# davxy/ark-vrf

Measured on AMD Instinct MI355X. Metric: thin_vrf_batch_verifications_per_sec, higher is better.
Workload: dtype u32x8 (256-bit prime-field Montgomery, integer)

## Files before the change

ark_vrf_amd/csrc/capi.hip:

```cpp
#include "capi_internal.h"
#include "host_sha512.h"
#include "host_shake128.h"
#include "host_sha256.h"
#include "host_sha512_mb.h"
#include <condition_variable>
#include <deque>
#include <mutex>
#include <thread>
#include "proto_dev.h"
#include "vrf_batch.h"
#include "suite_dispatch.h"
#include <chrono>
#include <optional>
#include <stdlib.h>
#include <string.h>

using namespace avrf;

namespace avrf {
double now_us() {
  return std::chrono::duration<double, std::micro>(std::chrono::steady_clock::now().time_since_epoch()).count();
}
}

static inline bool ctx_busy(const avrf_ctx *c) { return c->run_phase != 0; }

static int ensure_fixed(avrf_ctx *c) {
  if (c->fixed_ready) return AVRF_OK;
  if (c->d_fixed.ensure((size_t)2 * 32 * 256 * sizeof(te_pre_raw)) != hipSuccess) return AVRF_ERR_NO_DEVICE;
  AVRF_SINGLE(c->suite, fixed_table(c->d_fixed.as<te_pre_raw>(), c->stream));
  c->fixed_ready = true;
  return AVRF_OK;
}

static BatchDev batch_of(avrf_ctx *c) {
  BatchDev b;
  b.pks_xy = c->d_pks.as<uint8_t>(); b.ios_xy = c->d_ios.as<uint8_t>(); b.io_off = c->d_io_off.as<uint32_t>();
  b.ads = c->d_ads.as<uint8_t>(); b.ad_off = c->d_ad_off.as<uint32_t>(); b.proofs = c->d_proofs.as<uint8_t>();
  b.sks = c->d_sks.as<uint8_t>(); b.n = (uint32_t)c->n;
  b.fixed = (const te_pre *)c->d_fixed.p;
  b.tabs = (te_ext *)c->d_tabs.p; b.first = 0;
  b.weights = nullptr; b.records = nullptr;
  return b;
}

static constexpr size_t ITEM_CHUNK = 131072;
template <class F> static int per_item_chunks(avrf_ctx *c, bool with_pks, F launch) {
  if (int fs = ensure_fixed(c)) return fs;
  const size_t chunk = c->n < ITEM_CHUNK ? c->n : ITEM_CHUNK;
  if (c->d_tabs.ensure(chunk * (size_t)ITEM_TAB_SLOTS * sizeof(te_ext_raw)) != hipSuccess) return AVRF_ERR_NO_DEVICE;
  BatchDev b = batch_of(c);
  if (!with_pks) b.pks_xy = nullptr;
  for (size_t i = 0; i < c->n; i += chunk) {
    b.first = (uint32_t)i; b.n = (uint32_t)(c->n - i < chunk ? c->n : i + chunk);
    launch(b);
  }
  return AVRF_OK;
}

static void validate_staged(avrf_ctx *c, int kind, int32_t *d_rec_status) {
  if (c->validate <= 0 || !c->n) return;
  uint32_t *fl = c->d_flags.as<uint32_t>();
  const uint32_t n = (uint32_t)c->n;
  const KindFacts &k = kind_facts(kind);
  if (k.pk && c->d_pks.p) AVRF_SINGLE(c->suite, validate_xy(c->d_pks.as<uint8_t>(), 64, 1, n, c->validate, fl, d_rec_status, c->stream));
  if (k.points) AVRF_SINGLE(c->suite, validate_xy(c->d_proofs.as<uint8_t>(), (uint32_t)k.xy_proof(), (uint32_t)k.points, n, c->validate, fl, d_rec_status, c->stream));
  if (c->tot_io) {
    if (!d_rec_status) AVRF_SINGLE(c->suite, validate_xy(c->d_ios.as<uint8_t>(), 128, 2, (uint32_t)c->tot_io, c->validate, fl, nullptr, c->stream));
    else {
      const uint32_t *io_off = c->h_io.as<uint32_t>();
      bool uniform = c->tot_io == c->n;
      for (size_t j = 0; uniform && j < c->n; j++) uniform = io_off[j] == j;
      if (uniform) AVRF_SINGLE(c->suite, validate_xy(c->d_ios.as<uint8_t>(), 128, 2, n, c->validate, fl, d_rec_status, c->stream));
      else AVRF_SINGLE(c->suite, validate_xy(c->d_ios.as<uint8_t>(), 128, 2, (uint32_t)c->tot_io, c->validate, fl, d_rec_status, c->stream,
                                             c->d_io_off.as<uint32_t>(), n));
    }
  }
}

namespace avrf {
int ctx_create(int suite, int device, bool lane_owner, avrf_ctx **out) {
  if (!out || suite < 0 || suite >= AVRF_N_SUITES) return AVRF_ERR_BAD_ARG;
  *out = nullptr;
  int n = 0;
  if (hipGetDeviceCount(&n) != hipSuccess || n <= 0 || device < 0 || device >= n) return AVRF_ERR_NO_DEVICE;
  HIP_TRY(hipSetDevice(device));
  avrf_ctx *c = new avrf_ctx();
  c->suite = suite; c->device = device; c->lane_owner = lane_owner;
  if (lane_owner) {
    if (hipStreamCreateWithFlags(&c->own.stream, hipStreamNonBlocking) != hipSuccess) { delete c; return AVRF_ERR_NO_DEVICE; }
    c->stream = c->own.stream;
  }
  if (c->d_flags.ensure(64) != hipSuccess || c->h_flags.ensure(64) != hipSuccess) { avrf_ctx_destroy(c); return AVRF_ERR_NO_DEVICE; }
  *out = c;
  return AVRF_OK;
}
}

extern "C" {

int avrf_ctx_set_validation(avrf_ctx *c, int level) {
  if (!c || level < 0 || level > 2) return AVRF_ERR_BAD_ARG;
  c->validate = level;
  return AVRF_OK;
}

hipStream_t avrf_ctx_stream_(avrf_ctx *c) { return c->stream; }
int avrf_ctx_suite_(avrf_ctx *c) { return c->suite; }
int avrf_ctx_device_(avrf_ctx *c) { return c->device; }
int avrf_ctx_busy_(avrf_ctx *c) { return c && ctx_busy(c); }

const char *avrf_version(void) { return "avrf 0.3 (gfx950; tiny/thin/pedersen/ring VRF over Bandersnatch, Baby-JubJub, JubJub; device pairing)"; }

int avrf_device_count(void) {
  int n = 0;
  if (hipGetDeviceCount(&n) != hipSuccess) return 0;
  return n;
}

int avrf_device_set_blocking_sync(int device, int on) {
  int prev = 0;
  if (hipGetDevice(&prev) != hipSuccess || hipSetDevice(device) != hipSuccess) { (void)hipGetLastError(); return AVRF_ERR_NO_DEVICE; }
  const hipError_t e = hipSetDeviceFlags(on ? hipDeviceScheduleBlockingSync : hipDeviceScheduleAuto);
  (void)hipSetDevice(prev);
  if (e != hipSuccess) (void)hipGetLastError();
  return e == hipSuccess ? AVRF_OK : AVRF_ERR_NO_DEVICE;
}

int avrf_ctx_create(int suite, int device, avrf_ctx **out) { return ctx_create(suite, device, true, out); }

void avrf_ctx_destroy(avrf_ctx *c) {
  if (!c) return;
  delete c;
}

static int lane_msm(avrf_ctx *c, size_t n, HostExt *r) {
  return guarded([&] { return msm_te_device(c->suite, c->L->d_pre.as<te_pre_raw>(), c->L->d_scalars.as<uint32_t>(), n, c->L->ws, c->stream, r) ? (int)AVRF_ERR_BAD_ARG : 0; });
}
static int lane_msm_vectors(avrf_ctx *c, size_t n, size_t nv, HostExt *r) {
  return guarded([&] { return msm_te_small_vectors(c->suite, c->L->d_pre.as<te_pre_raw>(), c->L->d_scalars.as<uint32_t>(), n, nv, c->L->ws, c->stream, r) ? (int)AVRF_ERR_BAD_ARG : 0; });
}

static int finish_point(avrf_ctx *c, const HostExt &r, uint8_t out_xy[64]) {
  with_suite(c->suite, [&](auto tag) { using S = typename decltype(tag)::type; HostTe<S>::to_affine_bytes(r, out_xy); });
  return AVRF_OK;
}
static bool point_is_identity(avrf_ctx *c, const HostExt &r) {
  return with_suite(c->suite, [&](auto tag) { using S = typename decltype(tag)::type; return HostTe<S>::is_identity(r); });
}
static bool scalar_in_range(int suite, const uint8_t *s) {
  H256 v; memcpy(v.l, s, 32);
  return with_suite(suite, [&](auto tag) { using S = typename decltype(tag)::type; return !HostField<typename S::Fr>::geq_p(v); });
}

static int upload_bases_and_scalars(avrf_ctx *c, size_t n, const uint8_t *bases_xy, const uint8_t *scalars, size_t scalar_bytes) {
  HIP_TRY(c->d_misc.ensure(n * 64)); HIP_TRY(c->L->d_scalars.ensure(scalar_bytes)); HIP_TRY(c->L->d_pre.ensure(n * sizeof(te_pre_raw)));
  HIP_TRY(hipMemcpyAsync(c->d_misc.p, bases_xy, n * 64, hipMemcpyHostToDevice, c->stream));
  HIP_TRY(hipMemcpyAsync(c->L->d_scalars.p, scalars, scalar_bytes, hipMemcpyHostToDevice, c->stream));
  HIP_TRY(hipMemsetAsync(c->d_flags.p, 0, 4, c->stream));
  return AVRF_OK;
}

static int msm_te_call(avrf_ctx *c, size_t n, const uint8_t *bases_xy, const uint8_t *scalars, uint8_t out_xy[64], bool mont) {
  if (!c || !out_xy || (n && (!bases_xy || !scalars))) return AVRF_ERR_BAD_ARG;
  if (ctx_busy(c)) return AVRF_ERR_BAD_ARG;
  HIP_TRY(hipSetDevice(c->device));
  for (size_t i = 0; !mont && i < n; i++) if (!scalar_in_range(c->suite, scalars + 32 * i)) return AVRF_INVALID_DATA;
  HostExt r;
  if (n) {
    if (int e = upload_bases_and_scalars(c, n, bases_xy, scalars, n * 32)) return e;
    launch_pre_from_affine(c->suite, c->d_misc.as<uint8_t>(), n, c->L->d_pre.as<te_pre_raw>(), c->d_flags.as<uint32_t>(), 0, c->stream, mont);
    if (mont) launch_scalars_from_mont(c->suite, c->L->d_scalars.as<uint32_t>(), n, c->d_flags.as<uint32_t>(), c->stream);
    HIP_TRY(hipMemcpyAsync(c->h_flags.p, c->d_flags.p, 4, hipMemcpyDeviceToHost, c->stream));
  }
  c->staged_kind = 0;
  if (int e = lane_msm(c, n, &r)) return e;
  if (n && *c->h_flags.as<uint32_t>()) return AVRF_INVALID_DATA;
  finish_point(c, r, out_xy);
  if (mont) with_suite(c->suite, [&](auto tag) { using S = typename decltype(tag)::type; using Fq = HostField<typename S::Fq>;
    Fq::store_le(out_xy, Fq::to_mont(Fq::load_le(out_xy))); Fq::store_le(out_xy + 32, Fq::to_mont(Fq::load_le(out_xy + 32))); });
  return AVRF_OK;
}
int avrf_msm_te(avrf_ctx *c, size_t n, const uint8_t *bases_xy, const uint8_t *scalars, uint8_t out_xy[64]) { return msm_te_call(c, n, bases_xy, scalars, out_xy, false); }
int avrf_msm_te_mont(avrf_ctx *c, size_t n, const uint8_t *bases_mont_xy, const uint8_t *scalars_mont, uint8_t out_mont_xy[64]) { return msm_te_call(c, n, bases_mont_xy, scalars_mont, out_mont_xy, true); }

int avrf_g1_msm(avrf_ctx *c, size_t n, const uint8_t *bases_xy, const uint8_t *scalars, uint8_t *out_xy) {
  if (!c || !out_xy || (n && (!bases_xy || !scalars))) return AVRF_ERR_BAD_ARG;
  if (ctx_busy(c)) return AVRF_ERR_BAD_ARG;
  HIP_TRY(hipSetDevice(c->device));
  const int curve = pairing_curve_of(c->suite);
  const size_t fqb = curve == 0 ? 48 : 32;
  for (size_t i = 0; i < n; i++) {
    H256 v; memcpy(v.l, scalars + 32 * i, 32);
    bool ok = curve == 0 ? !HostField<FqBandersnatch>::geq_p(v) : !HostField<FqBabyJubJub>::geq_p(v);
    if (!ok) return AVRF_INVALID_DATA;
// ... 77 lines not shown
    for (size_t j = 0; j < n; j++) memcpy(&c->h_resp[rsz * j], resp + stride * j, rsz);
  }
  c->n_terms = n_terms(kind, n, c->tot_io);
  HIP_TRY(c->d_c.ensure(n * 16)); HIP_TRY(c->h_c.ensure(n * 16));
  HIP_TRY(c->d_z.ensure(z_bytes(kind, n, c->tot_io)));
  return c->lane_owner ? ensure_terms(c) : (int)AVRF_OK;
}

int ctx_stage(avrf_ctx *c, int kind, size_t n, const uint8_t *sks, const uint8_t *pks_xy, const uint8_t *ios_xy,
              const uint32_t *io_counts, const uint8_t *ads, const uint32_t *ad_lens, const uint8_t *proofs, bool wait) {
  if (int e = stage_open(c, kind, n, true, ios_xy, true, io_counts, ads, ad_lens)) return e;
  if (n == 0) return AVRF_OK;
  const size_t psz = kind_facts(kind).xy_proof();
  if (pks_xy) { HIP_TRY(c->d_pks.ensure(n * 64)); HIP_TRY(hipMemcpyAsync(c->d_pks.p, pks_xy, n * 64, hipMemcpyHostToDevice, c->stream)); }
  if (sks) { HIP_TRY(c->d_sks.ensure(n * 32)); HIP_TRY(hipMemcpyAsync(c->d_sks.p, sks, n * 32, hipMemcpyHostToDevice, c->stream)); }
  if (proofs) {
    HIP_TRY(c->d_proofs.ensure(n * psz)); HIP_TRY(hipMemcpyAsync(c->d_proofs.p, proofs, n * psz, hipMemcpyHostToDevice, c->stream));
    if (kind == Tiny) { HIP_TRY(hipStreamSynchronize(c->stream)); c->staged_kind = kind; return AVRF_OK; }
    if (int e = stage_verifier(c, kind, proofs + kind_facts(kind).resp_at_xy(), psz)) return e;
  }
  if (wait) HIP_TRY(hipStreamSynchronize(c->stream));
  c->staged_kind = kind;
  return AVRF_OK;
}
int ctx_stage_wire(avrf_ctx *c, int kind, size_t n, const uint8_t *pks, const uint8_t *ios, const uint32_t *io_counts, const uint8_t *ads,
                   const uint32_t *ad_lens, const uint8_t *proofs, int validate, bool wait) {
  const bool args_ok = (kind == Thin || kind == Pedersen) && (!n || (proofs && (kind != Thin || pks)));
  if (int e = stage_open(c, kind, n, args_ok, ios, false, io_counts, ads, ad_lens)) return e;
  if (n == 0) return AVRF_OK;
  const KindFacts &k = kind_facts(kind);
  const size_t L = (size_t)point_len_of(c->suite), a = c->tot_io, ppts = k.points, plen = k.wire_proof(L), psz = k.xy_proof();
  const size_t w_pks = k.pk ? n * L : 0, w_ios = 2 * a * L, w_pr = n * plen;
  HIP_TRY(c->d_proofs.ensure(n * psz));
  if (k.pk) HIP_TRY(c->d_pks.ensure(n * 64));
  HIP_TRY(c->d_misc.ensure(w_pks + w_ios + w_pr + 64)); HIP_TRY(c->d_status.ensure(64));
  uint8_t *dw = c->d_misc.as<uint8_t>();
  if (w_pks) HIP_TRY(hipMemcpyAsync(dw, pks, w_pks, hipMemcpyHostToDevice, c->stream));
  if (w_ios) HIP_TRY(hipMemcpyAsync(dw + w_pks, ios, w_ios, hipMemcpyHostToDevice, c->stream));
  HIP_TRY(hipMemcpyAsync(dw + w_pks + w_ios, proofs, w_pr, hipMemcpyHostToDevice, c->stream));
  uint32_t *d_flag = c->d_status.as<uint32_t>(), *h_flag = c->h_flags.as<uint32_t>() + 2;
  HIP_TRY(hipMemsetAsync(d_flag, 0, 4, c->stream));
  if (k.pk) AVRF_SINGLE(c->suite, decompress_strided(dw, (uint32_t)L, (uint32_t)n, c->d_pks.as<uint8_t>(), 64, validate, d_flag, c->stream));
  AVRF_SINGLE(c->suite, decompress_strided(dw + w_pks, (uint32_t)L, (uint32_t)(2 * a), c->d_ios.as<uint8_t>(), 64, validate, d_flag, c->stream));
  const uint8_t *dpr = dw + w_pks + w_ios;
  for (size_t p = 0; p < ppts; p++)
    AVRF_SINGLE(c->suite, decompress_strided(dpr + L * p, (uint32_t)plen, (uint32_t)n, c->d_proofs.as<uint8_t>() + 64 * p, (uint32_t)psz, validate, d_flag, c->stream));
  HIP_TRY(hipMemcpy2DAsync(c->d_proofs.as<uint8_t>() + 64 * ppts, psz, dpr + L * ppts, plen, k.tail, n, hipMemcpyDeviceToDevice, c->stream));
  HIP_TRY(hipMemcpyAsync(h_flag, d_flag, 4, hipMemcpyDeviceToHost, c->stream));
  if (int e = stage_verifier(c, kind, proofs + k.resp_at_wire(L), plen)) return e;
  if (!wait) { c->wire_pending = true; c->staged_kind = kind; return AVRF_OK; }
  HIP_TRY(hipStreamSynchronize(c->stream)); HIP_TRY(hipGetLastError());
  if (*h_flag) return AVRF_INVALID_DATA;
  c->staged_kind = kind;
  return AVRF_OK;
}
}
extern "C" {
int avrf_thin_batch_stage_wire(avrf_ctx *c, size_t n, const uint8_t *pks, const uint8_t *ios, const uint32_t *io_counts, const uint8_t *ads,
                               const uint32_t *ad_lens, const uint8_t *proofs, int validate) {
  if (!c || ctx_busy(c)) return AVRF_ERR_BAD_ARG;
  return avrf::ctx_stage_wire(c, Thin, n, pks, ios, io_counts, ads, ad_lens, proofs, validate, true);
}
int avrf_pedersen_batch_stage_wire(avrf_ctx *c, size_t n, const uint8_t *ios, const uint32_t *io_counts, const uint8_t *ads,
                                   const uint32_t *ad_lens, const uint8_t *proofs, int validate) {
  if (!c || ctx_busy(c)) return AVRF_ERR_BAD_ARG;
  return avrf::ctx_stage_wire(c, Pedersen, n, nullptr, ios, io_counts, ads, ad_lens, proofs, validate, true);
}

int avrf_thin_batch_stage(avrf_ctx *c, size_t n, const uint8_t *pks_xy, const uint8_t *ios_xy, const uint32_t *io_counts,
                          const uint8_t *ads, const uint32_t *ad_lens, const uint8_t *proofs) {
  if (n && (!pks_xy || !proofs)) return AVRF_ERR_BAD_ARG;
  return ctx_stage(c, Thin, n, nullptr, pks_xy, ios_xy, io_counts, ads, ad_lens, proofs, true);
}
int avrf_pedersen_batch_stage(avrf_ctx *c, size_t n, const uint8_t *ios_xy, const uint32_t *io_counts,
                              const uint8_t *ads, const uint32_t *ad_lens, const uint8_t *proofs) {
  if (n && !proofs) return AVRF_ERR_BAD_ARG;
  return ctx_stage(c, Pedersen, n, nullptr, nullptr, ios_xy, io_counts, ads, ad_lens, proofs, true);
}

namespace {
class WeightHashService {
 public:
  static WeightHashService &get() { static WeightHashService s; return s; }
  bool enabled() const { return !workers_.empty(); }
  void run(WeightJob &job) {
    Item it{&job, false};
    std::unique_lock<std::mutex> lk(m_);
    q_.push_back(&it);
    cv_work_.notify_one();
    cv_done_.wait(lk, [&] { return it.done; });
  }
 private:
  struct Item { WeightJob *job; bool done; };
  WeightHashService() {
    int n = 0;
    if (const char *e = getenv("AVRF_HASH_THREADS")) n = atoi(e);
    if (n < 0) n = 0; if (n > 16) n = 16;
    if (!sha512_mb_available()) n = 0;
    for (int i = 0; i < n; i++) workers_.emplace_back([this] { loop(); });
  }
  ~WeightHashService() {
    { std::lock_guard<std::mutex> lk(m_); stop_ = true; }
    cv_work_.notify_all();
    for (auto &t : workers_) t.join();
  }
  void loop() {
    for (;;) {
      Item *take[8]; int cnt = 0;
      {
        std::unique_lock<std::mutex> lk(m_);
        cv_work_.wait(lk, [&] { return stop_ || !q_.empty(); });
        if (stop_) return;
        if (q_.size() == 1) cv_work_.wait_for(lk, std::chrono::microseconds(40), [&] { return stop_ || q_.size() >= 2; });
        if (stop_) return;
        while (cnt < 8 && !q_.empty()) { take[cnt++] = q_.front(); q_.pop_front(); }
      }
      WeightJob *jobs[8];
      for (int i = 0; i < cnt; i++) jobs[i] = take[i]->job;
      sha512_many(jobs, cnt);
      { std::lock_guard<std::mutex> lk(m_); for (int i = 0; i < cnt; i++) take[i]->done = true; }
      cv_done_.notify_all();
    }
  }
  std::mutex m_; std::condition_variable cv_work_, cv_done_; std::deque<Item *> q_; std::vector<std::thread> workers_; bool stop_ = false;
};
}

}
namespace avrf {
static Seed64 seed_of(const uint8_t digest[64]) {
  Seed64 seed;
  for (int i = 0; i < 8; i++) { uint64_t v; memcpy(&v, digest + 8 * i, 8); seed.w[i] = __builtin_bswap64(v); }
  return seed;
}
static void launch_prepare(avrf_ctx *c, int kind, const BatchDev &b) {
  if (kind == Thin) AVRF_BATCH(c->suite, thin_prepare(b, c->d_c.as<uint32_t>(), c->d_z.as<uint32_t>(), c->d_flags.as<uint32_t>(), c->stream));
  else AVRF_BATCH(c->suite, ped_prepare(b, c->d_c.as<uint32_t>(), c->d_z.as<uint8_t>(), c->d_flags.as<uint32_t>(), c->stream));
}
static void launch_terms(avrf_ctx *c, int kind, const BatchDev &b, const Seed64 &seed, uint64_t first, uint32_t *d_scalars) {
  if (kind == Thin) AVRF_BATCH(c->suite, thin_terms(b, seed, first, c->d_c.as<uint32_t>(), c->d_z.as<uint32_t>(), d_scalars,
                                                    c->L->d_pre.as<te_pre_raw>(), c->L->d_gpart.as<uint32_t>(), (uint32_t)c->n_terms, c->stream));
  else AVRF_BATCH(c->suite, ped_terms(b, seed, first, c->d_c.as<uint32_t>(), c->d_z.as<uint8_t>(), d_scalars,
                                      c->L->d_pre.as<te_pre_raw>(), c->L->d_gpart.as<uint32_t>(), (uint32_t)c->n_terms, c->stream));
}

int batch_begin(avrf_ctx *c, int kind) {
  if (!c || c->staged_kind != kind || c->run_phase != 0) return AVRF_ERR_BAD_ARG;
  if (c->n == 0) { c->run_phase = 1; return AVRF_OK; }
  if (!c->n_terms) return AVRF_ERR_BAD_ARG;
  HIP_TRY(hipSetDevice(c->device));
  c->run_t0 = now_us();
  const size_t n = c->n;
  BatchDev b = batch_of(c);
  HIP_TRY(hipMemsetAsync(c->d_flags.p, 0, 4, c->stream));
  validate_staged(c, kind, nullptr);
  const bool host_weights = suite_host_weights(c->suite);
  const size_t recsz = kind_facts(kind).record();
  uint8_t prefix[64]; const size_t pl = batch_prefix(c->suite, prefix);
  if (!host_weights) {
    HIP_TRY(c->d_rec.ensure(n * recsz)); HIP_TRY(c->h_msg.ensure(pl + n * recsz));
    b.records = c->d_rec.as<uint8_t>();
  }
  launch_prepare(c, kind, b);
  if (!host_weights) {
    memcpy(c->h_msg.p, prefix, pl);
    HIP_TRY(hipMemcpyAsync(c->h_msg.as<uint8_t>() + pl, c->d_rec.p, n * recsz, hipMemcpyDeviceToHost, c->stream));
    c->h_msg_len = pl + n * recsz;
  } else HIP_TRY(hipMemcpyAsync(c->h_c.p, c->d_c.p, n * 16, hipMemcpyDeviceToHost, c->stream));
  HIP_TRY(hipMemcpyAsync(c->h_flags.p, c->d_flags.p, 4, hipMemcpyDeviceToHost, c->stream));
  c->run_begin_us = now_us() - c->run_t0;
  c->run_phase = 1;
  return AVRF_OK;
}

int batch_collect(avrf_ctx *c, int kind) {
  if (!c || c->staged_kind != kind || c->run_phase != 1) return AVRF_ERR_BAD_ARG;
  if (c->n && *c->h_flags.as<uint32_t>()) { c->run_phase = 0; return AVRF_INVALID_DATA; }
  if (c->wire_pending) {
    c->wire_pending = false;
    if (c->n && c->h_flags.as<uint32_t>()[2]) { c->run_phase = 0; c->staged_kind = 0; return AVRF_INVALID_DATA; }
  }
  return AVRF_OK;
}

int batch_seed(avrf_ctx *c, int kind, uint8_t digest[64]) {
  const size_t n = c->n;
  memset(digest, 0, 64);
  if (!n) return AVRF_OK;
  if (suite_host_weights(c->suite)) {
    const KindFacts &k = kind_facts(kind);
    uint8_t prefix[64]; const size_t pl = batch_prefix(c->suite, prefix);
    c->h_weights.resize(n * k.weight);
    with_suite(c->suite, [&](auto tag_) {
      using S = typename decltype(tag_)::type;
      std::conditional_t<S::XOF_SHAKE, HostShake128, HostSha256> h;
      absorb_weight_message(h, prefix, pl, n, c->h_c.as<uint8_t>(), c->h_resp.data(), k.resp);
      h.squeeze_copy(c->h_weights.data(), n * k.weight);
    });
    return AVRF_OK;
  }
  WeightJob job = WeightJob::whole(c->h_msg.as<uint8_t>(), c->h_msg_len);
  WeightHashService &svc = WeightHashService::get();
  if (svc.enabled()) svc.run(job); else weight_digest_scalar(job);
  memcpy(digest, job.digest, 64);
  return AVRF_OK;
}

int batch_launch(avrf_ctx *c, int kind, const uint8_t digest[64]) {
  if (!c || c->staged_kind != kind || c->run_phase != 1) return AVRF_ERR_BAD_ARG;
  if (c->n == 0) { c->run_phase = 2; return AVRF_OK; }
  c->run_phase = 0;
  HIP_TRY(hipSetDevice(c->device));
  const size_t n = c->n;
  BatchDev b = batch_of(c);
  if (c->unit_weights) {
    c->h_weights.assign(n * 16, 0);
    for (size_t j = 0; j < n; j++) c->h_weights[16 * j] = 1;
  }
  if (c->unit_weights || suite_host_weights(c->suite)) {
    const size_t wbytes = n * kind_facts(kind).weight;
    HIP_TRY(c->d_weights.ensure(wbytes));
    HIP_TRY(hipMemcpyAsync(c->d_weights.p, c->h_weights.data(), wbytes, hipMemcpyHostToDevice, c->stream));
    b.weights = c->d_weights.as<uint8_t>();
  } else b.records = c->d_rec.as<uint8_t>();
  if (int e = ensure_terms(c)) return e;
  const double t2 = now_us();
  launch_terms(c, kind, b, seed_of(digest), 0, c->L->d_scalars.as<uint32_t>());
  const double t3 = now_us();
  if (int e = guarded([&] { return msm_te_enqueue(c->suite, c->L->d_pre.as<te_pre_raw>(), c->L->d_scalars.as<uint32_t>(), c->n_terms, c->L->ws, c->chain(), c->stream) ? (int)AVRF_ERR_BAD_ARG : 0; })) return e;
  c->timing[3] = t3 - t2;
  c->run_msm_us = now_us() - t3;
  c->run_phase = 2;
  return AVRF_OK;
}

int batch_end(avrf_ctx *c, int kind) {
  if (!c || c->staged_kind != kind || c->run_phase != 2) return AVRF_ERR_BAD_ARG;
  c->run_phase = 0;
  if (c->n == 0) return AVRF_OK;
  HIP_TRY(hipSetDevice(c->device));
  const double t3 = now_us();
  HostExt r;
  if (int e = guarded([&] { return msm_te_finish(c->suite, c->L->ws, c->chain(), c->stream, &r) ? (int)AVRF_ERR_BAD_ARG : 0; })) return e;
  double t4 = now_us();
  int st = point_is_identity(c, r) ? AVRF_OK : AVRF_VERIFICATION_FAILURE;
  double t5 = now_us();
  c->timing[4] = c->run_msm_us + (t4 - t3); c->timing[5] = t5 - t4;
  c->timing[0] = c->timing[1] + c->timing[2] + c->timing[3] + c->timing[4] + c->timing[5];
  return st;
}
}
extern "C" {

static int batch_hash(avrf_ctx *c, int kind) {
  if (!c || c->staged_kind != kind || c->run_phase != 1) return AVRF_ERR_BAD_ARG;
  if (c->n == 0) { c->run_phase = 2; return AVRF_OK; }
  HIP_TRY(hipSetDevice(c->device));
  const double tw = now_us();
  if (hipStreamSynchronize(c->stream) != hipSuccess) { c->run_phase = 0; (void)hipGetLastError(); return AVRF_ERR_NO_DEVICE; }
  const double t1 = now_us();
  if (int e = batch_collect(c, kind)) return e;
  uint8_t digest[64];
  if (int e = batch_seed(c, kind, digest)) { c->run_phase = 0; return e; }
  const double t2 = now_us();
  c->timing[1] = c->run_begin_us + (t1 - tw); c->timing[2] = t2 - t1;
  return batch_launch(c, kind, digest);
}

static int batch_run(avrf_ctx *c, int kind) {
  if (int e = batch_begin(c, kind)) return e;
  if (int e = batch_hash(c, kind)) return e;
  return batch_end(c, kind);
}

int avrf_thin_batch_run(avrf_ctx *c) { return batch_run(c, Thin); }
int avrf_pedersen_batch_run(avrf_ctx *c) { return batch_run(c, Pedersen); }
static int run_call(avrf_ctx *c, int (*phase)(avrf_ctx *, int)) {
  if (!c) return AVRF_ERR_BAD_ARG;
  if (!c->staged_kind) {
    if (c->run_phase) { (void)hipSetDevice(c->device); (void)hipStreamSynchronize(c->stream); c->run_phase = 0; c->chain().disarm(); }
    return AVRF_ERR_BAD_ARG;
  }
  return phase(c, c->staged_kind);
}
int avrf_batch_run_begin(avrf_ctx *c) { return run_call(c, batch_begin); }
int avrf_batch_run_hash(avrf_ctx *c) { return run_call(c, batch_hash); }
int avrf_batch_run_end(avrf_ctx *c) { return run_call(c, batch_end); }

int avrf_thin_batch_verify(avrf_ctx *c, size_t n, const uint8_t *pks_xy, const uint8_t *ios_xy, const uint32_t *io_counts,
                           const uint8_t *ads, const uint32_t *ad_lens, const uint8_t *proofs) {
  int st = avrf_thin_batch_stage(c, n, pks_xy, ios_xy, io_counts, ads, ad_lens, proofs);
  return st ? st : avrf_thin_batch_run(c);
}
int avrf_pedersen_batch_verify(avrf_ctx *c, size_t n, const uint8_t *ios_xy, const uint32_t *io_counts,
                               const uint8_t *ads, const uint32_t *ad_lens, const uint8_t *proofs) {
  int st = avrf_pedersen_batch_stage(c, n, ios_xy, io_counts, ads, ad_lens, proofs);
  return st ? st : avrf_pedersen_batch_run(c);
}


int avrf_batch_weight_seed(int suite, int pedersen, size_t n, const uint8_t *c16, const uint8_t *resp, uint8_t seed_out[64]) {
  if (suite < 0 || suite >= AVRF_N_SUITES || !seed_out || (n && (!c16 || !resp))) return AVRF_ERR_BAD_ARG;
  if (suite_host_weights(suite)) return AVRF_ERR_BAD_ARG;
  uint8_t prefix[64]; const size_t pl = batch_prefix(suite, prefix);
  HostSha512 h;
  absorb_weight_message(h, prefix, pl, n, c16, resp, kind_facts(pedersen ? Pedersen : Thin).resp);
  h.final(seed_out);
  return AVRF_OK;
}

int avrf_batch_weight_seeds_x8(int suite, int pedersen, int count, const size_t *n, const uint8_t *const *c16, const uint8_t *const *resp, uint8_t *seeds_out) {
  if (suite < 0 || suite >= AVRF_N_SUITES || count < 1 || count > 8 || !n || !c16 || !resp || !seeds_out) return AVRF_ERR_BAD_ARG;
  if (suite_host_weights(suite)) return AVRF_ERR_BAD_ARG;
  if (!sha512_mb_available()) return AVRF_ERR_NO_DEVICE;
  uint8_t prefix[64]; const size_t pl = batch_prefix(suite, prefix);
  WeightJob jobs[8]; WeightJob *pj[8];
  for (int i = 0; i < count; i++) {
    if (n[i] && (!c16[i] || !resp[i])) return AVRF_ERR_BAD_ARG;
    jobs[i].prefix = prefix; jobs[i].prefix_len = pl; jobs[i].c16 = c16[i]; jobs[i].resp = resp[i]; jobs[i].n = n[i]; jobs[i].rsz = kind_facts(pedersen ? Pedersen : Thin).resp; pj[i] = &jobs[i];
  }
  sha512_weights_x8(pj, count);
  for (int i = 0; i < count; i++) memcpy(seeds_out + 64 * i, jobs[i].digest, 64);
  return AVRF_OK;
}

static int sha512_messages(int count, int lanes, bool available, void (*many)(WeightJob *const *, int), const uint8_t *const *msgs, const size_t *lens, uint8_t *digests_out) {
  if (count < 1 || count > lanes || !msgs || !lens || !digests_out) return AVRF_ERR_BAD_ARG;
  if (!available) return AVRF_ERR_NO_DEVICE;
  static const uint8_t empty = 0;
  WeightJob jobs[16]; WeightJob *pj[16];
// ... 18 lines not shown
  if (c->n == 0) return AVRF_OK;
  HIP_TRY(hipSetDevice(c->device));
  HIP_TRY(hipMemsetAsync(c->d_flags.p, 0, 4, c->stream));
  validate_staged(c, kind, nullptr);
  launch_prepare(c, kind, batch_of(c));
  HIP_TRY(hipMemcpyAsync(c_out, c->d_c.p, c->n * 16, hipMemcpyDeviceToHost, c->stream));
  HIP_TRY(hipMemcpyAsync(c->h_flags.p, c->d_flags.p, 4, hipMemcpyDeviceToHost, c->stream));
  HIP_TRY(hipStreamSynchronize(c->stream));
  if (*c->h_flags.as<uint32_t>()) return AVRF_INVALID_DATA;
  c->chal_gen = c->stage_gen;
  return AVRF_OK;
}
static int batch_partial(avrf_ctx *c, int kind, const uint8_t seed64[64], uint64_t first_index, uint8_t out_xy[64]) {
  if (!c || c->staged_kind != kind || !seed64 || !out_xy) return AVRF_ERR_BAD_ARG;
  if (ctx_busy(c)) return AVRF_ERR_BAD_ARG;
  if (suite_host_weights(c->suite)) return AVRF_ERR_BAD_ARG;
  if (c->n && c->chal_gen != c->stage_gen) return AVRF_ERR_BAD_ARG;
  HIP_TRY(hipSetDevice(c->device));
  HostExt r;
  if (c->n == 0) { r = with_suite(c->suite, [&](auto tag) { using S = typename decltype(tag)::type; return HostTe<S>::identity(); }); return finish_point(c, r, out_xy); }
  launch_terms(c, kind, batch_of(c), seed_of(seed64), first_index, c->L->d_scalars.as<uint32_t>());
  if (int e = lane_msm(c, c->n_terms, &r)) return e;
  return finish_point(c, r, out_xy);
}
int avrf_thin_batch_challenges(avrf_ctx *c, uint8_t *c_out) { return batch_challenges(c, Thin, c_out); }
int avrf_thin_batch_partial(avrf_ctx *c, const uint8_t seed64[64], uint64_t first_index, uint8_t out_xy[64]) { return batch_partial(c, Thin, seed64, first_index, out_xy); }
int avrf_pedersen_batch_challenges(avrf_ctx *c, uint8_t *c_out) { return batch_challenges(c, Pedersen, c_out); }
int avrf_pedersen_batch_partial(avrf_ctx *c, const uint8_t seed64[64], uint64_t first_index, uint8_t out_xy[64]) { return batch_partial(c, Pedersen, seed64, first_index, out_xy); }

int avrf_points_sum(int suite, size_t k, const uint8_t *points_xy, uint8_t out_xy[64]) {
  if (suite < 0 || suite >= AVRF_N_SUITES || !out_xy || (k && !points_xy)) return AVRF_ERR_BAD_ARG;
  bool bad = false;
  with_suite(suite, [&](auto tag) { using S = typename decltype(tag)::type; using T = HostTe<S>;
    HostExt acc = T::identity(), p;
    for (size_t i = 0; i < k && !bad; i++) { if (!T::from_affine_bytes(points_xy + 64 * i, &p)) bad = true; else acc = T::add(acc, p); }
    if (!bad) T::to_affine_bytes(acc, out_xy); });
  if (bad) return AVRF_INVALID_DATA;
  return AVRF_OK;
}

size_t avrf_batch_last_terms(avrf_ctx *c, uint8_t *bases_xy, uint8_t *scalars) {
  if (!c || !c->staged_kind || !c->n_terms || ctx_busy(c)) return 0;
  if (hipSetDevice(c->device) != hipSuccess) return 0;
  size_t k = c->n_terms;
  if (scalars) { if (hipMemcpy(scalars, c->L->d_scalars.p, k * 32, hipMemcpyDeviceToHost) != hipSuccess) return 0; }
  if (bases_xy) {
    std::vector<te_pre_raw> pre(k);
    if (hipMemcpy(pre.data(), c->L->d_pre.p, k * sizeof(te_pre_raw), hipMemcpyDeviceToHost) != hipSuccess) return 0;
    for (size_t i = 0; i < k; i++) {
      H256 x, y; memcpy(x.l, pre[i].w, 32); memcpy(y.l, pre[i].w + 8, 32);
      with_suite(c->suite, [&](auto tag) { using S = typename decltype(tag)::type; x = HostField<typename S::Fq>::from_mont(x); y = HostField<typename S::Fq>::from_mont(y); });
      memcpy(bases_xy + 64 * i, x.l, 32); memcpy(bases_xy + 64 * i + 32, y.l, 32);
    }
  }
  return k;
}

void avrf_last_timing(avrf_ctx *c, double out[8]) {
  if (!c || !out) return;
  for (int i = 0; i < 8; i++) out[i] = c->timing[i];
}

int avrf_kernel_stats(avrf_ctx *c, int reset, double *accum_ms_total, uint64_t *accum_launches, int32_t plan[4]) {
  if (!c) return AVRF_ERR_BAD_ARG;
  if (accum_ms_total) *accum_ms_total = c->L->ws.accum_ms_total;
  if (accum_launches) *accum_launches = c->L->ws.accum_launches;
  if (plan) { plan[0] = c->L->ws.last_plan.c; plan[1] = c->L->ws.last_plan.nwin; plan[2] = c->L->ws.last_plan.nb; plan[3] = c->L->ws.last_plan.lpb; }
  if (reset) { c->L->ws.accum_ms_total = 0; c->L->ws.accum_launches = 0; }
  return AVRF_OK;
}

}

static int read_flags(avrf_ctx *c) {
  if (hipMemcpyAsync(c->h_flags.p, c->d_flags.p, 4, hipMemcpyDeviceToHost, c->stream) != hipSuccess) return AVRF_ERR_NO_DEVICE;
  if (hipStreamSynchronize(c->stream) != hipSuccess || hipGetLastError() != hipSuccess) return AVRF_ERR_NO_DEVICE;
  static const bool trace = getenv("AVRF_TRACE_FLAGS") != nullptr;
  if (trace && *c->h_flags.as<uint32_t>()) fprintf(stderr, "avrf: input flags 0x%x (suite %d)\n", *c->h_flags.as<uint32_t>(), c->suite);
  return *c->h_flags.as<uint32_t>() ? AVRF_INVALID_DATA : AVRF_OK;
}

static int sync_stream(avrf_ctx *c) {
  HIP_TRY(hipStreamSynchronize(c->stream)); HIP_TRY(hipGetLastError());
  return AVRF_OK;
}

static bool wave_shape(const avrf_ctx *c, size_t n, const uint32_t *io_counts) {
  if (!n || n > (size_t)AVRF_WAVE_ITEMS_MAX || c->tot_io != n) return false;
  static const bool off = getenv("AVRF_NO_WAVE_ITEMS") != nullptr;
  if (off) return false;
  for (size_t j = 0; j < n; j++) if (io_counts[j] != 1) return false;
  return true;
}

using Route = std::optional<int>;
static bool one_as_msm() { static const bool on = getenv("AVRF_NO_ONE_AS_MSM") == nullptr; return on; }

static Route prove_one_as_msm(avrf_ctx *c, bool have_pk, bool tiny, uint8_t *proofs_out) {
  if (c->tot_io >= 1000) return {};
  const size_t nt = 1 + c->tot_io, plen = kind_facts(tiny ? Tiny : Thin).xy_proof(), sb = AVRF_SINGLE(c->suite, prove_state_bytes());
  HIP_TRY(c->h_c.ensure(64));
  if (!have_pk) { if (int fs = ensure_fixed(c)) return fs; }
  HIP_TRY(c->L->d_scalars.ensure(nt * 32)); HIP_TRY(c->L->d_pre.ensure(nt * sizeof(te_pre_raw))); HIP_TRY(c->d_misc.ensure(sb + 64)); HIP_TRY(c->d_out.ensure(plen));
  BatchDev b = batch_of(c);
  if (!have_pk) b.pks_xy = nullptr;
  uint8_t *d_state = c->d_misc.as<uint8_t>();
  AVRF_SINGLE(c->suite, thin_prove_begin(b, c->L->d_scalars.as<uint32_t>(), c->L->d_pre.as<te_pre_raw>(), d_state, c->stream, tiny));
  HostExt r;
  if (int e = lane_msm(c, nt, &r)) return e;
  uint8_t *rxy = c->h_c.as<uint8_t>();
  finish_point(c, r, rxy);
  HIP_TRY(hipMemcpyAsync(d_state + sb, rxy, 64, hipMemcpyHostToDevice, c->stream));
  AVRF_SINGLE(c->suite, thin_prove_end(b, d_state, d_state + sb, c->d_out.as<uint8_t>(), c->d_flags.as<uint32_t>(), c->stream, tiny));
  HIP_TRY(hipMemcpyAsync(proofs_out, c->d_out.p, plen, hipMemcpyDeviceToHost, c->stream));
  return read_flags(c);
}

static Route prove_ped_one_as_msm(avrf_ctx *c, bool have_pk, uint8_t *proofs_out, uint8_t *blindings_out) {
  if (c->tot_io > 1000) return {};
  if (!have_pk) { if (int fs = ensure_fixed(c)) return fs; }
  const size_t m = c->tot_io, nt = 2 + m, sb = AVRF_SINGLE(c->suite, ped_state_bytes()), wb = (m * 32 + 63) / 64 * 64 + 64;
  HIP_TRY(c->L->d_scalars.ensure(2 * nt * 32)); HIP_TRY(c->L->d_pre.ensure(nt * sizeof(te_pre_raw)));
  HIP_TRY(c->d_misc.ensure(sb + wb + 192 + 32)); HIP_TRY(c->d_out.ensure(kind_facts(Pedersen).xy_proof())); HIP_TRY(c->h_c.ensure(192));
  BatchDev b = batch_of(c);
  if (!have_pk) b.pks_xy = nullptr;
  uint8_t *d_state = c->d_misc.as<uint8_t>(), *d_pts = d_state + sb + wb, *d_blind = d_pts + 192;
  uint32_t *d_wts = reinterpret_cast<uint32_t *>(d_state + sb);
  uint32_t *d_sc = c->L->d_scalars.as<uint32_t>(); te_pre_raw *d_pre = c->L->d_pre.as<te_pre_raw>();
  AVRF_SINGLE(c->suite, ped_prove_begin(b, d_sc, d_pre, d_state, d_wts, c->stream));
  HostExt r[2];
  if (int e = lane_msm(c, 2, &r[0])) return e;
  uint8_t *pts = c->h_c.as<uint8_t>();
  finish_point(c, r[0], pts);
  HIP_TRY(hipMemcpyAsync(d_pts, pts, 64, hipMemcpyHostToDevice, c->stream));
  AVRF_SINGLE(c->suite, ped_prove_mid(b, d_sc, d_pre, d_state, d_wts, d_pts, c->stream));
  if (int e = lane_msm_vectors(c, nt, 2, r)) return e;
  finish_point(c, r[0], pts + 64); finish_point(c, r[1], pts + 128);
  HIP_TRY(hipMemcpyAsync(d_pts + 64, pts + 64, 128, hipMemcpyHostToDevice, c->stream));
  AVRF_SINGLE(c->suite, ped_prove_end(b, d_state, d_pts, c->d_out.as<uint8_t>(), blindings_out ? d_blind : nullptr, c->d_flags.as<uint32_t>(), c->stream));
  HIP_TRY(hipMemcpyAsync(proofs_out, c->d_out.p, kind_facts(Pedersen).xy_proof(), hipMemcpyDeviceToHost, c->stream));
  if (blindings_out) HIP_TRY(hipMemcpyAsync(blindings_out, d_blind, 32, hipMemcpyDeviceToHost, c->stream));
  return read_flags(c);
}

static Route verify_one_as_msm(avrf_ctx *c, int32_t *status_out) {
  if (!c->n_terms || c->n_terms > 2048) return {};
  uint8_t zero[64] = {0};
  c->unit_weights = true;
  int st = batch_begin(c, Thin);
  if (st == AVRF_OK) st = batch_launch(c, Thin, zero);
  if (st == AVRF_OK) st = batch_end(c, Thin);
  c->unit_weights = false;
  if (st != AVRF_OK && st != AVRF_VERIFICATION_FAILURE) { c->run_phase = 0; return st; }
  status_out[0] = *c->h_flags.as<uint32_t>() ? AVRF_INVALID_DATA : st;
  return AVRF_OK;
}

static Route verify_ped_one_as_msm(avrf_ctx *c, int32_t *status_out) {
  if (!c->n_terms || c->n_terms > 2048) return {};
  int st = batch_begin(c, Pedersen);
  c->run_phase = 0;
  if (st != AVRF_OK) return st;
  const size_t nt = c->n_terms;
  HIP_TRY(c->L->d_scalars.ensure(2 * nt * 32)); HIP_TRY(c->L->d_pre.ensure(nt * sizeof(te_pre_raw))); HIP_TRY(c->L->d_gpart.ensure(2 * 64 + 64));
  c->h_weights.assign(64, 0); c->h_weights[0] = 1; c->h_weights[32 + 16] = 1;
  HIP_TRY(c->d_weights.ensure(64));
  HIP_TRY(hipMemcpyAsync(c->d_weights.p, c->h_weights.data(), 64, hipMemcpyHostToDevice, c->stream));
  BatchDev b = batch_of(c);
  const uint8_t zero[64] = {0};
  for (int v = 0; v < 2; v++) {
    b.weights = c->d_weights.as<uint8_t>() + 32 * v;
    launch_terms(c, Pedersen, b, seed_of(zero), 0, c->L->d_scalars.as<uint32_t>() + (size_t)v * nt * 8);
  }
  HostExt r[2];
  if (int e = lane_msm_vectors(c, nt, 2, r)) return e;
  status_out[0] = *c->h_flags.as<uint32_t>() ? AVRF_INVALID_DATA : (point_is_identity(c, r[0]) && point_is_identity(c, r[1])) ? AVRF_OK : AVRF_VERIFICATION_FAILURE;
  return AVRF_OK;
}

struct ItemCall {
  int kind;
  bool prover;
  uint8_t *proofs_out;
  uint8_t *blindings_out;
  int32_t *status_out;
};

template <class One, class Wave, class Lane>
static int item_call(avrf_ctx *c, const ItemCall &k, size_t n, const uint8_t *sks, const uint8_t *pks_xy, const uint8_t *ios_xy,
                     const uint32_t *io_counts, const uint8_t *ads, const uint32_t *ad_lens, const uint8_t *proofs, One one, Wave wave, Lane lane) {
  int st = ctx_stage(c, k.kind, n, sks, pks_xy, ios_xy, io_counts, ads, ad_lens, proofs, k.kind == Tiny);
  if (st || !n) return st;
  const size_t psz = kind_facts(k.kind).xy_proof();
  if (k.prover) {
    c->staged_kind = 0;
    HIP_TRY(c->d_out.ensure(n * psz));
    if (k.kind == Pedersen) HIP_TRY(c->d_misc.ensure(n * 32));
  } else HIP_TRY(c->d_status.ensure(n * 4));
  if (k.prover || k.kind == Tiny) HIP_TRY(hipMemsetAsync(c->d_flags.p, 0, 4, c->stream));
  auto finish = [&](bool wave_statuses) -> int {
    if (!k.prover) {
      validate_staged(c, k.kind, c->d_status.as<int32_t>());
      HIP_TRY(hipMemcpyAsync(k.status_out, c->d_status.p, n * 4, hipMemcpyDeviceToHost, c->stream));
      return sync_stream(c);
    }
    HIP_TRY(hipMemcpyAsync(k.proofs_out, c->d_out.p, n * psz, hipMemcpyDeviceToHost, c->stream));
    if (k.blindings_out) HIP_TRY(hipMemcpyAsync(k.blindings_out, c->d_misc.p, n * 32, hipMemcpyDeviceToHost, c->stream));
    if (wave_statuses) HIP_TRY(hipMemcpyAsync(c->h_c.p, c->d_status.p, n * 4, hipMemcpyDeviceToHost, c->stream));
    return read_flags(c);
  };
  auto routes = [&]() -> int {
    if (n == 1 && one_as_msm()) { if (Route r = one()) return *r; }
    if ((!k.prover || pks_xy) && wave_shape(c, n, io_counts)) {
      if (k.prover && k.kind == Pedersen) { if (int fs = ensure_fixed(c)) return fs; }
      if (k.prover) { HIP_TRY(c->d_status.ensure(n * 4)); HIP_TRY(c->h_c.ensure(n * 4)); }
      if (wave(batch_of(c))) {
        const int ws = finish(true);
        if (ws < 0) return ws;
        const int32_t *h_status = k.prover ? c->h_c.as<int32_t>() : k.status_out;
        bool fallback = false;
        for (size_t j = 0; j < n; j++) fallback |= h_status[j] == AVRF_WAVE_FALLBACK;
        if (!fallback) return ws;
        if (k.prover) HIP_TRY(hipMemsetAsync(c->d_flags.p, 0, 4, c->stream));
      }
    }
    if (int e = per_item_chunks(c, !k.prover || pks_xy, lane)) return e;
    return finish(false);
  };
  const double t0 = now_us();
  st = routes();
  c->timing[0] = now_us() - t0;
  if (k.kind == Tiny && st == AVRF_OK) c->staged_kind = 0;
  return st;
}

template <class F> static int pointwise(avrf_ctx *c, size_t n, bool args_ok, F body) {
  if (!c || (n && !args_ok) || ctx_busy(c)) return AVRF_ERR_BAD_ARG;
  if (!n) return AVRF_OK;
  if (n > 0x7fffffffULL) return AVRF_ERR_BAD_ARG;
  HIP_TRY(hipSetDevice(c->device));
  c->staged_kind = 0;
  return body();
}
extern "C" {

static int thin_or_tiny_prove(avrf_ctx *c, bool tiny, size_t n, const uint8_t *sks, const uint8_t *pks_xy, const uint8_t *ios_xy,
                              const uint32_t *io_counts, const uint8_t *ads, const uint32_t *ad_lens, uint8_t *proofs_out) {
  if (n && (!sks || !proofs_out)) return AVRF_ERR_BAD_ARG;
  return item_call(c, {tiny ? Tiny : Thin, true, proofs_out, nullptr, nullptr}, n, sks, pks_xy, ios_xy, io_counts, ads, ad_lens, nullptr,
      [&] { return prove_one_as_msm(c, pks_xy != nullptr, tiny, proofs_out); },
      [&](const BatchDev &b) { return AVRF_SINGLE(c->suite, thin_prove_wave(b, c->d_out.as<uint8_t>(), c->d_flags.as<uint32_t>(), c->d_status.as<int32_t>(), c->stream, tiny)); },
      [&](const BatchDev &b) { AVRF_SINGLE(c->suite, thin_prove(b, c->d_out.as<uint8_t>(), c->d_flags.as<uint32_t>(), c->stream, tiny)); });
}

int avrf_thin_prove(avrf_ctx *c, size_t n, const uint8_t *sks, const uint8_t *pks_xy, const uint8_t *ios_xy, const uint32_t *io_counts,
                    const uint8_t *ads, const uint32_t *ad_lens, uint8_t *proofs_out) {
  return thin_or_tiny_prove(c, false, n, sks, pks_xy, ios_xy, io_counts, ads, ad_lens, proofs_out);
}

int avrf_thin_verify(avrf_ctx *c, size_t n, const uint8_t *pks_xy, const uint8_t *ios_xy, const uint32_t *io_counts,
                     const uint8_t *ads, const uint32_t *ad_lens, const uint8_t *proofs, int32_t *status_out) {
  if (n && (!pks_xy || !proofs || !status_out)) return AVRF_ERR_BAD_ARG;
  return item_call(c, {Thin, false, nullptr, nullptr, status_out}, n, nullptr, pks_xy, ios_xy, io_counts, ads, ad_lens, proofs,
      [&] { return verify_one_as_msm(c, status_out); },
      [&](const BatchDev &b) { return AVRF_SINGLE(c->suite, thin_verify_wave(b, c->d_status.as<int32_t>(), c->stream)); },
      [&](const BatchDev &b) { AVRF_SINGLE(c->suite, thin_verify(b, c->d_status.as<int32_t>(), c->stream)); });
}

int avrf_tiny_prove(avrf_ctx *c, size_t n, const uint8_t *sks, const uint8_t *pks_xy, const uint8_t *ios_xy, const uint32_t *io_counts,
                    const uint8_t *ads, const uint32_t *ad_lens, uint8_t *proofs_out) {
  return thin_or_tiny_prove(c, true, n, sks, pks_xy, ios_xy, io_counts, ads, ad_lens, proofs_out);
}
int avrf_tiny_verify(avrf_ctx *c, size_t n, const uint8_t *pks_xy, const uint8_t *ios_xy, const uint32_t *io_counts,
                     const uint8_t *ads, const uint32_t *ad_lens, const uint8_t *proofs, int32_t *status_out) {
  if (n && (!pks_xy || !proofs || !status_out)) return AVRF_ERR_BAD_ARG;
  return item_call(c, {Tiny, false, nullptr, nullptr, status_out}, n, nullptr, pks_xy, ios_xy, io_counts, ads, ad_lens, proofs,
      [] { return Route(); },
      [&](const BatchDev &b) { return AVRF_SINGLE(c->suite, tiny_verify_wave(b, c->d_status.as<int32_t>(), c->stream)); },
      [&](const BatchDev &b) { AVRF_SINGLE(c->suite, tiny_verify(b, c->d_status.as<int32_t>(), c->stream)); });
}

int avrf_pedersen_prove(avrf_ctx *c, size_t n, const uint8_t *sks, const uint8_t *pks_xy, const uint8_t *ios_xy, const uint32_t *io_counts,
                        const uint8_t *ads, const uint32_t *ad_lens, uint8_t *proofs_out, uint8_t *blindings_out) {
  if (n && (!sks || !proofs_out)) return AVRF_ERR_BAD_ARG;
  return item_call(c, {Pedersen, true, proofs_out, blindings_out, nullptr}, n, sks, pks_xy, ios_xy, io_counts, ads, ad_lens, nullptr,
      [&] { return prove_ped_one_as_msm(c, pks_xy != nullptr, proofs_out, blindings_out); },
      [&](const BatchDev &b) { return AVRF_SINGLE(c->suite, ped_prove_wave(b, c->d_out.as<uint8_t>(), c->d_misc.as<uint8_t>(), c->d_flags.as<uint32_t>(), c->d_status.as<int32_t>(), c->stream)); },
      [&](const BatchDev &b) { AVRF_SINGLE(c->suite, ped_prove(b, c->d_out.as<uint8_t>(), c->d_misc.as<uint8_t>(), c->d_flags.as<uint32_t>(), c->stream)); });
}

int avrf_pedersen_verify(avrf_ctx *c, size_t n, const uint8_t *ios_xy, const uint32_t *io_counts,
                         const uint8_t *ads, const uint32_t *ad_lens, const uint8_t *proofs, int32_t *status_out) {
  if (n && (!proofs || !status_out)) return AVRF_ERR_BAD_ARG;
  return item_call(c, {Pedersen, false, nullptr, nullptr, status_out}, n, nullptr, nullptr, ios_xy, io_counts, ads, ad_lens, proofs,
      [&] { return verify_ped_one_as_msm(c, status_out); },
      [&](const BatchDev &b) { return AVRF_SINGLE(c->suite, ped_verify_wave(b, c->d_status.as<int32_t>(), c->stream)); },
      [&](const BatchDev &b) { AVRF_SINGLE(c->suite, ped_verify(b, c->d_status.as<int32_t>(), c->stream)); });
}

static int smul_common(avrf_ctx *c, size_t n, const uint8_t *scalars, const uint8_t *points_xy, uint8_t *out_xy) {
  return pointwise(c, n, scalars && out_xy, [&]() -> int {
    if (points_xy && n <= 32 && one_as_msm()) {
      for (size_t i = 0; i < n; i++) if (!scalar_in_range(c->suite, scalars + 32 * i)) return AVRF_INVALID_DATA;
      std::vector<uint8_t> diag(n * n * 32, 0);
      for (size_t i = 0; i < n; i++) memcpy(&diag[(i * n + i) * 32], scalars + 32 * i, 32);
      if (int e = upload_bases_and_scalars(c, n, points_xy, diag.data(), diag.size())) return e;
      launch_pre_from_affine(c->suite, c->d_misc.as<uint8_t>(), n, c->L->d_pre.as<te_pre_raw>(), c->d_flags.as<uint32_t>(), 0, c->stream);
      HIP_TRY(hipMemcpyAsync(c->h_flags.p, c->d_flags.p, 4, hipMemcpyDeviceToHost, c->stream));
      HostExt r[32];
      if (int e = lane_msm_vectors(c, n, n, r)) return e;
      if (*c->h_flags.as<uint32_t>()) return AVRF_INVALID_DATA;
      for (size_t i = 0; i < n; i++) finish_point(c, r[i], out_xy + 64 * i);
      return AVRF_OK;
    }
    HIP_TRY(c->d_sks.ensure(n * 32)); HIP_TRY(c->d_out.ensure(n * 64));
    HIP_TRY(hipMemcpyAsync(c->d_sks.p, scalars, n * 32, hipMemcpyHostToDevice, c->stream));
    if (points_xy) { HIP_TRY(c->d_misc.ensure(n * 64)); HIP_TRY(hipMemcpyAsync(c->d_misc.p, points_xy, n * 64, hipMemcpyHostToDevice, c->stream)); }
    HIP_TRY(hipMemsetAsync(c->d_flags.p, 0, 4, c->stream));
    if (!points_xy) { if (int fs = ensure_fixed(c)) return fs; }
    AVRF_SINGLE(c->suite, smul(c->d_sks.as<uint8_t>(), points_xy ? c->d_misc.as<uint8_t>() : nullptr, (uint32_t)n, c->d_out.as<uint8_t>(),
                               c->d_flags.as<uint32_t>(), c->d_fixed.as<te_pre_raw>(), c->stream));
    HIP_TRY(hipMemcpyAsync(out_xy, c->d_out.p, n * 64, hipMemcpyDeviceToHost, c->stream));
    return read_flags(c);
  });
}
int avrf_scalar_mul_base(avrf_ctx *c, size_t n, const uint8_t *sks, uint8_t *out_xy) { return smul_common(c, n, sks, nullptr, out_xy); }
int avrf_scalar_mul(avrf_ctx *c, size_t n, const uint8_t *scalars, const uint8_t *points_xy, uint8_t *out_xy) {
  if (n && !points_xy) return AVRF_ERR_BAD_ARG;
  return smul_common(c, n, scalars, points_xy, out_xy);
// ... 70 lines not shown
```

ark_vrf_amd/csrc/capi_internal.h:

```cpp
#pragma once
#include "../../include/avrf.h"
#include "host_te.h"
#include "msm.h"
#include "proof_kind.h"
#include <hip/hip_runtime.h>
#include <stdio.h>
#include <new>
#include <vector>

#define HIP_TRY(x) do { hipError_t e_ = (x); if (e_ != hipSuccess) { fprintf(stderr, "avrf: HIP error %s at %s:%d\n", hipGetErrorString(e_), __FILE__, __LINE__); return AVRF_ERR_NO_DEVICE; } } while (0)

namespace avrf {

template <bool PINNED> struct StageBuf : OwnedMem<PINNED> {
  hipError_t ensure(size_t bytes) {
    if (bytes <= this->cap && this->p) return hipSuccess;
    return this->reset(PINNED ? bytes + 256 : bytes + bytes / 8 + 256);
  }
};
using DevBuf = StageBuf<false>;
using PinBuf = StageBuf<true>;

template <class F> int guarded(F f) {
  try { return f(); }
  catch (const avrf::HipFailure &e) { fprintf(stderr, "avrf: HIP error %s at %s:%d\n", hipGetErrorString(e.err), e.file, e.line); return AVRF_ERR_NO_DEVICE; }
  catch (const std::bad_alloc &) { return AVRF_ERR_NO_DEVICE; }
}

struct LaneStream {
  hipStream_t stream = nullptr;
  LaneStream() = default;
  LaneStream(const LaneStream &) = delete;
  LaneStream &operator=(const LaneStream &) = delete;
  ~LaneStream() { if (stream) (void)hipStreamDestroy(stream); }
};
struct Lane : LaneStream {
  int queued = 0;
  MsmWorkspace ws;
  DevBuf d_scalars, d_pre, d_gpart;
};

}

struct avrf_ctx {
  int suite = 0, device = 0;
  hipStream_t stream = nullptr;
  avrf::Lane own; avrf::Lane *L = &own;
  avrf::MsmChain *pend = nullptr;
  avrf::MsmChain &chain() const { return pend ? *pend : L->ws.own; }
  bool lane_owner = true;
  int validate = 0;
  bool wire_pending = false;
  uint64_t stage_gen = 0, chal_gen = 0;
  int staged_kind = 0;
  size_t n = 0, tot_io = 0, n_terms = 0;
  avrf::DevBuf d_pks, d_ios, d_io_off, d_ads, d_ad_off, d_proofs, d_sks;
  std::vector<uint8_t> h_resp;
  avrf::DevBuf d_rec; avrf::PinBuf h_msg;
  size_t h_msg_len = 0;
  std::vector<uint8_t> h_weights; avrf::DevBuf d_weights;
  avrf::DevBuf d_c, d_z, d_flags, d_misc, d_out, d_status;
  avrf::DevBuf d_tabs;
  avrf::DevBuf d_fixed; bool fixed_ready = false;
  avrf::PinBuf h_c, h_flags, h_io;
  double timing[8] = {0, 0, 0, 0, 0, 0, 0, 0};
  int run_phase = 0;
  bool unit_weights = false;
  double run_t0 = 0, run_begin_us = 0, run_msm_us = 0;
  ~avrf_ctx() { (void)hipSetDevice(device); if (own.stream) (void)hipStreamSynchronize(own.stream); }
};

namespace avrf {
struct WeightJob;
int ctx_create(int suite, int device, bool lane_owner, avrf_ctx **out);
int ctx_stage(avrf_ctx *c, int kind, size_t n, const uint8_t *sks, const uint8_t *pks_xy, const uint8_t *ios_xy, const uint32_t *io_counts,
              const uint8_t *ads, const uint32_t *ad_lens, const uint8_t *proofs, bool wait);
int ctx_stage_wire(avrf_ctx *c, int kind, size_t n, const uint8_t *pks, const uint8_t *ios, const uint32_t *io_counts, const uint8_t *ads,
                   const uint32_t *ad_lens, const uint8_t *proofs, int validate, bool wait);
int batch_begin(avrf_ctx *c, int kind);
int batch_collect(avrf_ctx *c, int kind);
bool suite_host_weights(int suite);
int batch_seed(avrf_ctx *c, int kind, uint8_t digest[64]);
void sha512_many(WeightJob *const *jobs, int k);
int batch_launch(avrf_ctx *c, int kind, const uint8_t digest[64]);
int batch_end(avrf_ctx *c, int kind);
double now_us();
}
```

ark_vrf_amd/csrc/msm.h:

```cpp
#pragma once
#include <hip/hip_runtime.h>
#include <stddef.h>
#include <stdint.h>
#include "host_te.h"

namespace avrf {

struct te_pre_raw { uint32_t w[24]; };
struct te_ext_raw { uint32_t w[32]; };

struct HipFailure { hipError_t err; const char *file; int line; };

template <bool PINNED> struct OwnedMem {
  void *p = nullptr; size_t cap = 0;
  OwnedMem() = default;
  explicit OwnedMem(size_t bytes) { ensure(bytes); }
  OwnedMem(const OwnedMem &) = delete;
  OwnedMem &operator=(const OwnedMem &) = delete;
  OwnedMem(OwnedMem &&o) noexcept : p(o.p), cap(o.cap) { o.p = nullptr; o.cap = 0; }
  OwnedMem &operator=(OwnedMem &&o) noexcept { if (this != &o) { (void)release(); p = o.p; cap = o.cap; o.p = nullptr; o.cap = 0; } return *this; }
  ~OwnedMem() { (void)release(); }
  hipError_t reset(size_t bytes) {
    if (hipError_t e = release()) return e;
    if (hipError_t e = PINNED ? hipHostMalloc(&p, bytes) : hipMalloc(&p, bytes)) { p = nullptr; return e; }
    cap = bytes;
    return hipSuccess;
  }
  void ensure(size_t bytes) { if (bytes > cap) if (hipError_t e = reset(bytes)) throw HipFailure{e, __FILE__, __LINE__}; }
  hipError_t release() { hipError_t e = !p ? hipSuccess : PINNED ? hipHostFree(p) : hipFree(p); p = nullptr; cap = 0; return e; }
  template <class T = uint32_t> T *as() const { return (T *)p; }
  explicit operator bool() const { return p != nullptr; }
};
using DevMem = OwnedMem<false>;
using PinMem = OwnedMem<true>;
struct DevEvent {
  hipEvent_t e = nullptr;
  DevEvent() = default;
  DevEvent(const DevEvent &) = delete;
  DevEvent &operator=(const DevEvent &) = delete;
  DevEvent(DevEvent &&o) noexcept : e(o.e) { o.e = nullptr; }
  DevEvent &operator=(DevEvent &&o) noexcept { if (this != &o) { destroy(); e = o.e; o.e = nullptr; } return *this; }
  ~DevEvent() { destroy(); }
  hipError_t create(unsigned flags = hipEventDefault) { destroy(); return hipEventCreateWithFlags(&e, flags); }
  void destroy() { if (e) (void)hipEventDestroy(e); e = nullptr; }
  operator hipEvent_t() const { return e; }
};

struct MsmPlan {
  int c;
  int nwin;
  int nb;
  int lpb;
};
MsmPlan msm_plan(size_t n, int scalar_bits);

struct MsmChain {
  PinMem bits_host, plan_host;
  DevEvent ev0, ev1;
  MsmPlan plan = {0, 0, 0, 0}; int ret = 0;
  int wsum_lg = 4;
  size_t n = 0;
  bool armed = false;
  void ensure(size_t bytes);
  void disarm() { armed = false; }
  void release() { *this = MsmChain(); }
};

struct MsmWorkspace {
  DevMem keys;
  DevMem sorted;
  DevMem hist;
  DevMem cnts;
  DevMem offsets;
  DevMem win_tot;
  DevMem lane_base;
  DevMem heavy;
  DevMem plan_dev;
  DevMem buckets;
  DevMem rc;
  DevMem part;
  DevMem bits;
  MsmChain own;
  bool owns(const MsmChain &rec) const { return &rec == &own; }
  double accum_ms_total = 0; uint64_t accum_launches = 0; float accum_ms_last = 0;
  MsmPlan last_plan = {0, 0, 0, 0};
  void ensure(size_t n, const MsmPlan &p, size_t acc_bytes, size_t batch, size_t lanes_max, size_t part_bytes = 0);
  void release() { *this = MsmWorkspace(); }
};

int msm_te_device(int suite, const te_pre_raw *d_pre, const uint32_t *d_scalars, size_t n,
                  MsmWorkspace &ws, hipStream_t stream, HostExt *out);
int msm_te_enqueue(int suite, const te_pre_raw *d_pre, const uint32_t *d_scalars, size_t n, MsmWorkspace &ws, MsmChain &rec, hipStream_t stream);
int msm_te_finish(int suite, MsmWorkspace &ws, MsmChain &rec, hipStream_t stream, HostExt *out);
int msm_te_small_vectors(int suite, const te_pre_raw *d_pre, const uint32_t *d_scalars, size_t n, size_t n_vectors, MsmWorkspace &ws, hipStream_t stream,
                         HostExt *out);
bool msm_te_pending_supported(int suite);

int msm_g1_device(int curve, const uint32_t *d_bases, const uint32_t *d_scalars, size_t n, MsmWorkspace &ws, hipStream_t stream, uint8_t *out_xy,
                  size_t batch = 1, size_t scalar_stride = 0);
void build_g1_table(int curve, const uint32_t *d_bases, size_t n, int c, int nwin, uint32_t *d_table, hipStream_t stream);
int msm_g1_fixed_device(int curve, const uint32_t *d_table, int table_c, size_t table_stride, const uint32_t *d_scalars, size_t n,
                        size_t scalar_stride, MsmWorkspace &ws, hipStream_t stream, uint8_t *out_xy, size_t batch,
                        const uint32_t *d_base_idx = nullptr, int scalars_mont = 0);
struct G1DirectTable {
  uint32_t *d = nullptr;
  int curve = 0, c = 0, rows = 0;
  size_t n = 0;
  uint64_t off[32] = {};
  uint32_t mult[32] = {};
  uint64_t points = 0, bytes = 0;
};
size_t g1_direct_table_shape(int curve, size_t n, int c, G1DirectTable *t);
void build_g1_direct_table(int curve, const uint32_t *d_bases, size_t n, int c, G1DirectTable *t, hipStream_t stream);
void free_g1_direct_table(G1DirectTable *t);
int msm_g1_direct_device(const G1DirectTable &t, const uint32_t *d_scalars, size_t n, size_t scalar_stride, MsmWorkspace &ws, hipStream_t stream,
                         uint8_t *out_xy, size_t batch, int scalars_mont = 0, const uint32_t *d_base_idx = nullptr);
void launch_g1_decompress(int curve, const uint8_t *d_comp, size_t n, uint8_t *d_out_xy, uint8_t *d_ok, hipStream_t stream);
void launch_g1_bases(int curve, const uint8_t *d_xy, size_t n, uint32_t *d_out, uint32_t *d_flag, hipStream_t stream);
void launch_g1_subgroup_check(int curve, const uint32_t *d_bases, size_t n, uint32_t *d_flag, hipStream_t stream, int32_t *d_rec_status = nullptr,
                              uint32_t ppr = 1);
void launch_g1_lincomb(int curve, const uint32_t *d_bases, const uint32_t *d_scalars, size_t n_items, uint32_t tpi, uint32_t split, uint32_t *d_out,
                       hipStream_t stream, bool glv_split_scalars = false);
void g1_glv_split_bls(uint64_t k[4]);

void launch_pre_from_affine(int suite, const uint8_t *d_xy, size_t n, te_pre_raw *d_pre, uint32_t *d_flag,
                            int check_curve, hipStream_t stream, int mont_in = 0);
void launch_scalars_from_mont(int suite, uint32_t *d_scalars, size_t n, uint32_t *d_flag, hipStream_t stream);

}
```

ark_vrf_amd/csrc/msm.hip:

```cpp
#include "msm.h"
#include "host_pool.h"
#include "curves.h"
#include "suite_dispatch.h"
#include "te_quad.h"
#include "host_g1.h"
#include <stdio.h>
#include <stdlib.h>
#include <string.h>
#include <mutex>
#include <vector>

namespace avrf {

#define HIP_CHECK(x) do { hipError_t e_ = (x); if (e_ != hipSuccess) throw HipFailure{e_, __FILE__, __LINE__}; } while (0)


template <class S>
__global__ void __launch_bounds__(256) k_pre_from_affine(const uint8_t *__restrict__ xy, uint32_t n, te_pre *__restrict__ out,
                                  uint32_t *__restrict__ flag, int check_curve, int mont_in) {
  using Fq = typename S::Fq;
  uint32_t i = blockIdx.x * blockDim.x + threadIdx.x;
  if (i >= n) return;
  fp x = fp_load_le(xy + 64 * (size_t)i), y = fp_load_le(xy + 64 * (size_t)i + 32);
  uint32_t f = 0;
// ... 5 lines not shown
}

void launch_pre_from_affine(int suite, const uint8_t *d_xy, size_t n, te_pre_raw *d_pre, uint32_t *d_flag,
                            int check_curve, hipStream_t stream, int mont_in) {
  if (!n) return;
  dim3 g((unsigned)((n + 255) / 256)), b(256);
  with_suite(suite, [&](auto tag) { using S = typename decltype(tag)::type;
    hipLaunchKernelGGL(k_pre_from_affine<S>, g, b, 0, stream, d_xy, (uint32_t)n, (te_pre *)d_pre, d_flag, check_curve, mont_in); });
}
template <class S>
__global__ void __launch_bounds__(256) k_scalars_from_mont(uint32_t *__restrict__ sc, uint32_t n, uint32_t *__restrict__ flag) {
  using Fr = typename S::Fr;
  uint32_t i = blockIdx.x * blockDim.x + threadIdx.x;
  if (i >= n) return;
  fp k = fp_load(sc + 8 * (size_t)i);
  if (ge_p<Fr>(k)) atomicOr(flag, 4u);
  fp_store(sc + 8 * (size_t)i, fp_from_mont<Fr>(k));
}
void launch_scalars_from_mont(int suite, uint32_t *d_scalars, size_t n, uint32_t *d_flag, hipStream_t stream) {
  if (!n) return;
  with_suite(suite, [&](auto tag) { using S = typename decltype(tag)::type;
    hipLaunchKernelGGL(k_scalars_from_mont<S>, dim3((unsigned)((n + 255) / 256)), dim3(256), 0, stream, d_scalars, (uint32_t)n, d_flag); });
}


__global__ void __launch_bounds__(256) k_digits(const uint32_t *__restrict__ scalars, uint32_t n, uint32_t stride, int c, int nwin, uint16_t *__restrict__ keys, int mont) {
  uint32_t i = blockIdx.x * blockDim.x + threadIdx.x;
  if (i >= n) return;
  const uint32_t bat = blockIdx.y;
  keys += (size_t)bat * nwin * n;
  uint32_t s[9];
  const uint4 *p = reinterpret_cast<const uint4 *>(scalars + 8 * ((size_t)bat * stride + i));
  uint4 a = p[0], b = p[1];
  s[0] = a.x; s[1] = a.y; s[2] = a.z; s[3] = a.w; s[4] = b.x; s[5] = b.y; s[6] = b.z; s[7] = b.w; s[8] = 0;
  if (mont) {
    fp v;
#pragma unroll
    for (int k = 0; k < 8; k++) v.v[k] = s[k];
    v = mont == 1 ? fp_from_mont<FqBandersnatch>(v) : fp_from_mont<FqBabyJubJub>(v);
#pragma unroll
    for (int k = 0; k < 8; k++) s[k] = v.v[k];
  }
  const uint32_t nb = 1u << (c - 1), mask = (1u << c) - 1;
  uint32_t carry = 0;
  for (int w = 0; w < nwin; w++) {
    int bit = w * c;
    uint32_t v = 0;
    if (bit < 256) {
      int li = bit >> 5, sh = bit & 31;
      uint64_t two = (uint64_t)s[li] | ((uint64_t)s[li + 1] << 32);
      v = (uint32_t)(two >> sh) & mask;
    }
    v += carry;
    uint32_t key;
    if (v > nb) { key = ((1u << c) - v) | 0x8000u; carry = 1; }
    else { key = v; carry = 0; }
    keys[(size_t)w * n + i] = (uint16_t)key;
  }
}


__global__ void __launch_bounds__(256)
k_hist(const uint16_t *__restrict__ keys, uint32_t n, uint32_t tile_len, int c, uint32_t *__restrict__ H) {
  extern __shared__ uint32_t lds[];
  const uint32_t nb = 1u << (c - 1), tile = blockIdx.x, w = blockIdx.y, ntiles = gridDim.x;
  for (uint32_t b = threadIdx.x; b < nb; b += blockDim.x) lds[b] = 0;
  __syncthreads();
  uint32_t lo = tile * tile_len, hi = lo + tile_len; if (hi > n) hi = n;
  const uint16_t *kw = keys + (size_t)w * n;
  for (uint32_t i = lo + threadIdx.x; i < hi; i += blockDim.x) {
    uint32_t b = kw[i] & 0x7fffu;
    if (b) atomicAdd(&lds[b - 1], 1u);
  }
  __syncthreads();
  uint32_t *out = H + ((size_t)w * ntiles + tile) * nb;
  for (uint32_t b = threadIdx.x; b < nb; b += blockDim.x) out[b] = lds[b];
}

__global__ void __launch_bounds__(256)
k_scan_tiles(uint32_t *__restrict__ H, uint32_t ntiles, int c, uint32_t *__restrict__ cnts) {
  const uint32_t nb = 1u << (c - 1), w = blockIdx.y, b = blockIdx.x * 256 + threadIdx.x;
  if (b >= nb) return;
  uint32_t *Hb = H + (size_t)w * ntiles * nb + b;
  uint32_t run = 0, k = 0;
  for (; k + 8 <= ntiles; k += 8) {
    uint32_t v[8];
#pragma unroll
    for (int j = 0; j < 8; j++) v[j] = Hb[(size_t)(k + j) * nb];
#pragma unroll
    for (int j = 0; j < 8; j++) { Hb[(size_t)(k + j) * nb] = run; run += v[j]; }
  }
  for (; k < ntiles; k++) { const uint32_t v = Hb[(size_t)k * nb]; Hb[(size_t)k * nb] = run; run += v; }
  cnts[(size_t)w * nb + b] = run;
}
__global__ void __launch_bounds__(1024)
k_scan_offs(const uint32_t *__restrict__ cnts, uint32_t n, int c, uint32_t *__restrict__ offs, uint32_t *__restrict__ win_tot) {
  __shared__ uint32_t part[1024];
  const uint32_t nb = 1u << (c - 1), w = blockIdx.x, t = threadIdx.x;
  const uint32_t bpt = (nb + 1023) / 1024;
  uint32_t b0 = t * bpt, b1 = b0 + bpt; if (b1 > nb) b1 = nb; if (b0 > nb) b0 = nb;
  uint32_t sum = 0;
  for (uint32_t b = b0; b < b1; b++) sum += cnts[(size_t)w * nb + b];
  part[t] = sum;
  __syncthreads();
  for (uint32_t off = 1; off < 1024; off <<= 1) {
    uint32_t v = (t >= off) ? part[t - off] : 0;
    __syncthreads();
    part[t] += v;
    __syncthreads();
  }
  if (t == 1023) win_tot[w] = part[1023];
  uint32_t run = part[t] - sum + w * n;
  for (uint32_t b = b0; b < b1; b++) { offs[(size_t)w * nb + b] = run; run += cnts[(size_t)w * nb + b]; }
}

__global__ void __launch_bounds__(1024)
k_plan(const uint32_t *__restrict__ win_tot, uint32_t vwin, uint32_t lanes_target, uint32_t per_min, uint32_t *__restrict__ lane_base,
       uint32_t *__restrict__ plan) {
  __shared__ uint64_t red[1024];
  __shared__ uint32_t sc[1024];
  __shared__ uint32_t carry_s;
  const uint32_t t = threadIdx.x;
  uint64_t s = 0;
  for (uint32_t v = t; v < vwin; v += 1024) s += win_tot[v];
  red[t] = s;
  __syncthreads();
  for (uint32_t off = 512; off >= 1; off >>= 1) { if (t < off) red[t] += red[t + off]; __syncthreads(); }
  const uint64_t total = red[0];
  if (lanes_target > 8 * vwin) lanes_target -= vwin;
  uint64_t per64 = (total + lanes_target - 1) / lanes_target;
  if (per64 < per_min) per64 = per_min;
  const uint32_t per = (uint32_t)per64;
  if (t == 0) carry_s = 0;
  __syncthreads();
  for (uint32_t base = 0; base < vwin; base += 1024) {
    const uint32_t v = base + t;
    const uint32_t mine = v < vwin ? (win_tot[v] + per - 1) / per : 0;
    sc[t] = mine;
    __syncthreads();
    for (uint32_t off = 1; off < 1024; off <<= 1) {
      uint32_t x = (t >= off) ? sc[t - off] : 0;
      __syncthreads();
      sc[t] += x;
      __syncthreads();
    }
    if (v < vwin) lane_base[v] = carry_s + sc[t] - mine;
    __syncthreads();
    if (t == 1023) carry_s += sc[1023];
    __syncthreads();
  }
  if (t == 0) { lane_base[vwin] = carry_s; plan[0] = per; plan[1] = carry_s; plan[2] = 0; }
}

__global__ void __launch_bounds__(256)
k_scatter(const uint16_t *__restrict__ keys, uint32_t n, uint32_t tile_len, int c, const uint32_t *__restrict__ H,
          const uint32_t *__restrict__ offs, uint32_t *__restrict__ sorted, uint32_t remap_n, uint32_t remap_stride,
          const uint32_t *__restrict__ bidx, uint32_t ntiles, uint32_t vwin) {
  extern __shared__ uint32_t lds[];
  const uint32_t nb = 1u << (c - 1);
  const uint32_t xcd = blockIdx.x & 7u, k = blockIdx.x >> 3, tile = k % ntiles, w = xcd + 8u * (k / ntiles);
  if (w >= vwin) return;
  const uint32_t *Hin = H + ((size_t)w * ntiles + tile) * nb;
  for (uint32_t b = threadIdx.x; b < nb; b += blockDim.x) lds[b] = offs[(size_t)w * nb + b] + Hin[b];
  __syncthreads();
  uint32_t lo = tile * tile_len, hi = lo + tile_len; if (hi > n) hi = n;
  const uint16_t *kw = keys + (size_t)w * n;
  for (uint32_t i = lo + threadIdx.x; i < hi; i += blockDim.x) {
    uint32_t key = kw[i], b = key & 0x7fffu;
    if (b) {
      uint32_t pos = atomicAdd(&lds[b - 1], 1u);
      uint32_t idx = i;
      if (remap_n) {
        uint32_t j = i % remap_n;
        idx = (i / remap_n) * remap_stride + (bidx ? bidx[(size_t)w * remap_n + j] : j);
      }
      sorted[pos] = idx | ((key & 0x8000u) << 16);
    }
  }
}

template <class CV> __device__ __noinline__ void cv_add_nf(typename CV::acc_t *r, const typename CV::acc_t *a, const typename CV::acc_t *b) { *r = CV::add(*a, *b); }
template <class CV> __device__ __noinline__ void cv_dbl_nf(typename CV::acc_t *r, const typename CV::acc_t *a) { *r = CV::dbl(*a); }
template <class CV> AVRF_DI typename CV::acc_t cv_add(const typename CV::acc_t &a, const typename CV::acc_t &b) {
  if constexpr (CV::INLINE_REDUCE_OPS) return CV::add(a, b);
  else { typename CV::acc_t r; cv_add_nf<CV>(&r, &a, &b); return r; }
}
template <class CV> AVRF_DI typename CV::acc_t cv_dbl(const typename CV::acc_t &a) {
  if constexpr (CV::INLINE_REDUCE_OPS) return CV::dbl(a);
  else { typename CV::acc_t r; cv_dbl_nf<CV>(&r, &a); return r; }
}



template <class CV>
__global__ void __launch_bounds__(256, CV::MIN_WAVES)
k_accumulate(const uint32_t *__restrict__ bases, const uint32_t *__restrict__ sorted,
             const uint32_t *__restrict__ offs, const uint32_t *__restrict__ win_tot, const uint32_t *__restrict__ lane_base,
             const uint32_t *__restrict__ plan, uint32_t vwin, uint32_t nb, uint32_t n, uint32_t *__restrict__ part) {
  using AC = typename CV::accum;
  using acc_t = typename AC::acc_t; using base_t = typename CV::base_t;
  const uint32_t t = blockIdx.x * blockDim.x + threadIdx.x;
  const uint32_t per = plan[0];
  if (t >= plan[1]) return;
  uint32_t lo = 0, hi = vwin;
  while (hi - lo > 1) { uint32_t mid = (lo + hi) >> 1; if (lane_base[mid] <= t) lo = mid; else hi = mid; }
  const uint32_t v = lo;
  const uint32_t wbeg = v * n, wend = wbeg + win_tot[v];
  const uint32_t e0 = wbeg + (t - lane_base[v]) * per;
  uint32_t e1 = e0 + per; if (e1 > wend) e1 = wend;
  const uint32_t *ow = offs + (size_t)v * nb;
  lo = 0; hi = nb;
  while (hi - lo > 1) { uint32_t mid = (lo + hi) >> 1; if (ow[mid] <= e0) lo = mid; else hi = mid; }
  uint32_t b = lo;
  uint32_t nxt = (b + 1 < nb) ? ow[b + 1] : 0xffffffffu;
  const size_t slot0 = (size_t)t + (size_t)v * nb;
  acc_t acc;
  {
    extern __shared__ uint32_t acc_lds[];
    constexpr int BW = CV::BASE_WORDS, CH = BW / 4;
    uint32_t *wbuf = acc_lds + (threadIdx.x >> 6) * (2 * BW * 64);
    const uint32_t lane = threadIdx.x & 63;
    auto issue = [&](uint32_t ix, uint32_t slot) {
      const uint32_t *src = bases + (size_t)(ix & 0x7fffffffu) * BW;
#pragma unroll
      for (int c = 0; c < CH; c++)
        __builtin_amdgcn_global_load_lds((const __attribute__((address_space(1))) void *)(src + 4 * c),
                                         (__attribute__((address_space(3))) void *)(wbuf + slot * (BW * 64) + c * 256), 16, 0, 0);
    };
    auto fetch = [&](uint32_t slot) {
      uint32_t w[BW];
#pragma unroll
      for (int c = 0; c < CH; c++) {
        const uint4 v = *reinterpret_cast<const uint4 *>(wbuf + slot * (BW * 64) + c * 256 + lane * 4);
        w[4 * c] = v.x; w[4 * c + 1] = v.y; w[4 * c + 2] = v.z; w[4 * c + 3] = v.w;
      }
      return CV::base_from_words(w);
    };
    const uint32_t cnt = e1 - e0;
    if constexpr (!CV::PREFETCH) acc = AC::identity();
    uint32_t idx = cnt ? sorted[e0] : 0u;
    uint32_t idx1 = cnt > 1 ? sorted[e0 + 1] : 0u;
    if (cnt) issue(idx, 0);
    for (uint32_t k = 0; k < cnt; k++) {
      const uint32_t i = e0 + k, cidx = idx;
      asm volatile("s_waitcnt vmcnt(0) lgkmcnt(0)" ::: "memory");
      const base_t cur = fetch(k & 1);
      idx = idx1;
      if (k + 1 < cnt) issue(idx, (k + 1) & 1);
      if (k + 2 < cnt) idx1 = sorted[i + 2];
      if constexpr (CV::PREFETCH) {
        if (k == 0) { acc = AC::from_base(cur, (cidx & 0x80000000u) != 0); continue; }
      }
      if (i >= nxt) {
        AC::store_part(part + (slot0 + b) * AC::PART_WORDS, acc);
        acc = AC::identity();
        do { b++; nxt = (b + 1 < nb) ? ow[b + 1] : 0xffffffffu; } while (i >= nxt);
      }
      acc = AC::madd(acc, cur, (cidx & 0x80000000u) != 0);
    }
  }
  AC::store_part(part + (slot0 + b) * AC::PART_WORDS, acc);
}

template <class T> struct type_tag { using type = T; };
template <class CV> AVRF_DI typename CV::acc_t wave_sum(typename CV::acc_t acc);

constexpr uint32_t HEAVY_PARTIALS = 12;
template <class CV>
__global__ void __launch_bounds__(256, CV::RED_WAVES)
k_bucket_sum(const uint32_t *__restrict__ offs, const uint32_t *__restrict__ cnts, const uint32_t *__restrict__ lane_base,
             uint32_t *__restrict__ plan, uint32_t nslots, uint32_t nb, uint32_t n, const uint32_t *__restrict__ part,
             uint32_t *__restrict__ buckets, uint32_t *__restrict__ heavy) {
  using acc_t = typename CV::acc_t;
  const uint32_t slot = blockIdx.x * blockDim.x + threadIdx.x;
  if (slot >= nslots) return;
  const uint32_t per = plan[0];
  const uint32_t cnt = cnts[slot];
  if (!cnt) { if (!CV::ZERO_IS_IDENTITY) CV::store_acc(buckets + (size_t)slot * CV::ACC_WORDS, CV::identity()); return; }
  const uint32_t v = slot / nb, rel = offs[slot] - v * n;
  const uint32_t lf = rel / per, ll = (rel + cnt - 1) / per, np = ll - lf + 1;
  if (np > HEAVY_PARTIALS) { heavy[atomicAdd(&plan[2], 1u)] = slot; return; }
  const size_t p0 = (size_t)lane_base[v] + lf + slot;
  using AC = typename CV::accum;
  acc_t acc = AC::load_part(part + p0 * AC::PART_WORDS);
#pragma unroll 1
  for (uint32_t k = 1; k < np; k++) acc = cv_add<CV>(acc, AC::load_part(part + (p0 + k) * AC::PART_WORDS));
  CV::store_acc(buckets + (size_t)slot * CV::ACC_WORDS, acc);
}

template <class CV>
__global__ void __launch_bounds__(256, CV::RED_WAVES)
k_heavy_sum(const uint32_t *__restrict__ offs, const uint32_t *__restrict__ cnts, const uint32_t *__restrict__ lane_base,
            const uint32_t *__restrict__ plan, uint32_t nb, uint32_t n, const uint32_t *__restrict__ part,
            uint32_t *__restrict__ buckets, const uint32_t *__restrict__ heavy) {
  using acc_t = typename CV::acc_t;
  extern __shared__ uint32_t lds[];
  const uint32_t per = plan[0], nheavy = plan[2], t = threadIdx.x, lane = t & 63, wv = t >> 6;
  for (uint32_t h = blockIdx.x; h < nheavy; h += gridDim.x) {
    const uint32_t slot = heavy[h], cnt = cnts[slot];
    const uint32_t v = slot / nb, rel = offs[slot] - v * n;
    const uint32_t lf = rel / per, ll = (rel + cnt - 1) / per, np = ll - lf + 1;
    const size_t p0 = (size_t)lane_base[v] + lf + slot;
    if constexpr (CV::QUAD) { q_heavy_sum<typename CV::suite>(part, p0, np, buckets + (size_t)slot * CV::ACC_WORDS, lds); continue; }
    acc_t a = CV::identity();
#pragma unroll 1
    for (uint32_t k = t; k < np; k += 256) a = cv_add<CV>(a, CV::accum::load_part(part + (p0 + k) * CV::accum::PART_WORDS));
    a = wave_sum<CV>(a);
    if (lane == 0) CV::store_acc(lds + wv * CV::ACC_WORDS, a);
    __syncthreads();
    if (t == 0) {
#pragma unroll 1
      for (uint32_t w = 1; w < 4; w++) a = cv_add<CV>(a, CV::load_acc(lds + w * CV::ACC_WORDS));
      CV::store_acc(buckets + (size_t)slot * CV::ACC_WORDS, a);
    }
    __syncthreads();
  }
}


template <class CV> AVRF_DI typename CV::acc_t wave_sum(typename CV::acc_t acc) {
#pragma unroll 1
  for (int off = 32; off >= 1; off >>= 1) acc = cv_add<CV>(acc, CV::shfl_down(acc, off));
  return acc;
}

template <class CV>
__global__ void __launch_bounds__(256)
k_rowcol(const uint32_t *__restrict__ buckets, int c, int h, uint32_t total_waves, uint32_t *__restrict__ rc) {
  const uint32_t nb = 1u << (c - 1), NC = 1u << h, NR = nb >> h;
  const uint32_t gw = (blockIdx.x * blockDim.x + threadIdx.x) >> 6, lane = threadIdx.x & 63;
  if (gw >= total_waves) return;
  const uint32_t tasks = NR + NC, w = gw / tasks, task = gw - w * tasks;
  const uint32_t *B = buckets + (size_t)w * nb * CV::ACC_WORDS;
  typename CV::acc_t acc = CV::identity();
  if (task < NR) {
    for (uint32_t lo = lane; lo < NC; lo += 64) { uint32_t b = task * NC + lo; if (b >= 1) acc = CV::add(acc, CV::load_acc(B + (size_t)(b - 1) * CV::ACC_WORDS)); }
  } else {
    uint32_t lo = task - NR;
    for (uint32_t hi = lane; hi < NR; hi += 64) { uint32_t b = hi * NC + lo; if (b >= 1) acc = CV::add(acc, CV::load_acc(B + (size_t)(b - 1) * CV::ACC_WORDS)); }
  }
  acc = wave_sum<CV>(acc);
  if (lane == 0) CV::store_acc(rc + (size_t)gw * CV::ACC_WORDS, acc);
}

template <class CV>
__global__ void __launch_bounds__(256)
k_bits(const uint32_t *__restrict__ buckets, const uint32_t *__restrict__ rc, int c, int h, uint32_t total_waves, uint32_t *__restrict__ out) {
  const uint32_t nb = 1u << (c - 1), NC = 1u << h, NR = nb >> h;
  const uint32_t gw = (blockIdx.x * blockDim.x + threadIdx.x) >> 6, lane = threadIdx.x & 63;
  if (gw >= total_waves) return;
  const uint32_t w = gw / c, k = gw - w * c;
  const uint32_t *RC = rc + (size_t)w * (NR + NC) * CV::ACC_WORDS;
  typename CV::acc_t acc = CV::identity();
  if ((int)k == c - 1) { if (lane == 0) acc = CV::load_acc(buckets + ((size_t)w * nb + (nb - 1)) * CV::ACC_WORDS); }
  else if ((int)k < h) { for (uint32_t lo = lane; lo < NC; lo += 64) if ((lo >> k) & 1) acc = CV::add(acc, CV::load_acc(RC + (size_t)(NR + lo) * CV::ACC_WORDS)); }
  else { uint32_t kk = k - h; for (uint32_t hi = lane; hi < NR; hi += 64) if ((hi >> kk) & 1) acc = CV::add(acc, CV::load_acc(RC + (size_t)hi * CV::ACC_WORDS)); }
  acc = wave_sum<CV>(acc);
  if (lane == 0) CV::store_acc(out + (size_t)gw * CV::ACC_WORDS, acc);
}

template <class CV>
__global__ void __launch_bounds__(128)
k_bits_direct(const uint32_t *__restrict__ buckets, int c, uint32_t total, uint32_t *__restrict__ out) {
  const uint32_t t = blockIdx.x * blockDim.x + threadIdx.x;
  if (t >= total) return;
  const uint32_t nb = 1u << (c - 1), w = t / c, k = t - w * c;
  const uint32_t *B = buckets + (size_t)w * nb * CV::ACC_WORDS;
  typename CV::acc_t acc = CV::identity();
  if ((int)k == c - 1) acc = CV::load_acc(B + (size_t)(nb - 1) * CV::ACC_WORDS);
  else for (uint32_t m = 0; m < (nb >> 1); m++) {
    uint32_t b = ((m >> k) << (k + 1)) | (1u << k) | (m & ((1u << k) - 1));
    acc = CV::add(acc, CV::load_acc(B + (size_t)(b - 1) * CV::ACC_WORDS));
  }
  CV::store_acc(out + (size_t)t * CV::ACC_WORDS, acc);
}

template <class CV>
__global__ void __launch_bounds__(64)
k_horner(const uint32_t *__restrict__ bits, uint32_t nbits, uint32_t batch, uint32_t *__restrict__ out) {
  uint32_t b = blockIdx.x * blockDim.x + threadIdx.x;
  if (b >= batch) return;
  const uint32_t *T = bits + (size_t)b * nbits * CV::ACC_WORDS;
  typename CV::acc_t acc = CV::identity();
  for (int i = (int)nbits - 1; i >= 0; i--) {
    acc = CV::dbl(acc);
    acc = CV::add(acc, CV::load_acc(T + (size_t)i * CV::ACC_WORDS));
  }
  CV::store_acc(out + (size_t)b * CV::ACC_WORDS, acc);
}

template <class CV>
__global__ void __launch_bounds__(256, CV::RED_WAVES)
k_wsum(const uint32_t *__restrict__ buckets, uint32_t nb, uint32_t nsets, uint32_t lps_log, uint32_t *__restrict__ out) {
  using acc_t = typename CV::acc_t;
  const uint32_t t = blockIdx.x * blockDim.x + threadIdx.x;
  const uint32_t lps = 1u << lps_log, set = t >> lps_log, g = t & (lps - 1), m = nb >> lps_log;
  const bool live = set < nsets;
  acc_t S = CV::identity(), W = CV::identity();
  if (live) {
    const uint32_t *B = buckets + (size_t)set * nb * CV::ACC_WORDS;
    const uint32_t lo = g * m + 1;
#pragma unroll 1
    for (uint32_t b = lo + m - 1; b >= lo; b--) {
      S = CV::add(S, CV::load_acc(B + (size_t)(b - 1) * CV::ACC_WORDS));
      W = CV::add(W, S);
    }
  }
  acc_t A = S;
#pragma unroll 1
  for (uint32_t off = 1; off < lps; off <<= 1) {
    acc_t o = CV::shfl_down(A, off);
    if (g + off < lps) A = cv_add<CV>(A, o);
  }
  acc_t Z = g ? A : CV::identity();
#pragma unroll 1
  for (uint32_t k = m; k > 1; k >>= 1) Z = cv_dbl<CV>(Z);
  acc_t V = cv_add<CV>(W, Z);
#pragma unroll 1
  for (uint32_t off = lps >> 1; off >= 1; off >>= 1) {
    acc_t o = CV::shfl_down(V, off);
    if (g + off < lps) V = cv_add<CV>(V, o);
  }
  if (live && g == 0) CV::store_out(out + (size_t)set * CV::OUT_WORDS, V);
}

template <class CV>
__global__ void __launch_bounds__(256, CV::RED_WAVES)
k_wsum_blk(const uint32_t *__restrict__ buckets, uint32_t nb, uint32_t *__restrict__ out) {
  using acc_t = typename CV::acc_t;
  extern __shared__ uint32_t lds[];
  const uint32_t set = blockIdx.x, t = threadIdx.x, lane = t & 63, wv = t >> 6, wps = blockDim.x >> 6;
  const uint32_t m = nb / blockDim.x;
  const uint32_t *B = buckets + (size_t)set * nb * CV::ACC_WORDS;
  acc_t S = CV::identity(), W = CV::identity();
  {
    const uint32_t lo = t * m + 1;
#pragma unroll 1
    for (uint32_t b = lo + m - 1; b >= lo; b--) {
      S = CV::add(S, CV::load_acc(B + (size_t)(b - 1) * CV::ACC_WORDS));
      W = CV::add(W, S);
    }
  }
  acc_t A = S;
#pragma unroll 1
  for (uint32_t off = 1; off < 64; off <<= 1) {
    acc_t o = CV::shfl_down(A, off);
    if (lane + off < 64) A = cv_add<CV>(A, o);
  }
  acc_t Z = lane ? A : CV::identity();
#pragma unroll 1
  for (uint32_t k = m; k > 1; k >>= 1) Z = cv_dbl<CV>(Z);
  acc_t V = cv_add<CV>(W, Z);
#pragma unroll 1
  for (uint32_t off = 32; off >= 1; off >>= 1) {
    acc_t o = CV::shfl_down(V, off);
    if (lane + off < 64) V = cv_add<CV>(V, o);
  }
  if (lane == 0) { CV::store_acc(lds + (2 * wv) * CV::ACC_WORDS, V); CV::store_acc(lds + (2 * wv + 1) * CV::ACC_WORDS, A); }
  __syncthreads();
  if (t == 0) {
    acc_t r = V, suf = CV::identity(), q = CV::identity();
#pragma unroll 1
    for (uint32_t w = wps - 1; w >= 1; w--) {
      suf = cv_add<CV>(suf, CV::load_acc(lds + (2 * w + 1) * CV::ACC_WORDS));
      q = cv_add<CV>(q, suf);
      r = cv_add<CV>(r, CV::load_acc(lds + (2 * w) * CV::ACC_WORDS));
    }
#pragma unroll 1
    for (uint32_t k = 64 * m; k > 1; k >>= 1) q = cv_dbl<CV>(q);
    CV::store_out(out + (size_t)set * CV::OUT_WORDS, cv_add<CV>(r, q));
  }
}


struct MsmEnv {
  int c = 0, per_min = 8, wsum_wps = 0, occ = 0, tile = 0; bool window_sums = true, tiny = true;
  size_t wsum_blk_max = 64;
  MsmEnv() {
    if (const char *e = getenv("AVRF_MSM_C")) { int v = atoi(e); if (v >= 3 && v <= 15) c = v; }
    if (const char *e = getenv("AVRF_MSM_OCC")) { int v = atoi(e); if (v >= 1 && v <= 8) occ = v; }
    if (const char *e = getenv("AVRF_MSM_TILE")) { int v = atoi(e); if (v >= 1024 && v <= (1 << 22)) tile = v; }
    if (const char *e = getenv("AVRF_MSM_PER_MIN")) { int v = atoi(e); if (v >= 1 && v <= 4096) per_min = v; }
    if (const char *e = getenv("AVRF_TE_WSUM_WPS")) { int v = atoi(e); if (v == 1 || v == 2 || v == 4 || v == 8 || v == 16) wsum_wps = v; }
    if (const char *e = getenv("AVRF_TE_WINDOW_SUMS")) window_sums = atoi(e) != 0;
    if (const char *e = getenv("AVRF_G1_WSUM_BLK_MAX")) { int v = atoi(e); if (v >= 0 && v <= 65536) wsum_blk_max = (size_t)v; }
    if (const char *e = getenv("AVRF_MSM_TINY")) tiny = atoi(e) != 0;
  }
};
static const MsmEnv &msm_env() { static const MsmEnv e; return e; }
static uint32_t tile_len_for(size_t n, size_t vwin) { return vwin >= 64 && msm_env().tile ? (uint32_t)msm_env().tile : 8192u; }

MsmPlan msm_plan(size_t n, int scalar_bits) {
  MsmPlan p;
  int lg = 0; while (((size_t)1 << (lg + 1)) <= n) lg++;
  int c = lg >= 16 ? lg - 5 : lg - 3;
  if (c < 4) c = 4; if (c > 15) c = 15;
  p.c = msm_env().c ? msm_env().c : c; p.lpb = 0;
  p.nb = 1 << (p.c - 1);
  p.nwin = (scalar_bits + 1 + p.c - 1) / p.c;
  return p;
}


struct AccShape { size_t lanes; unsigned lds; };
template <class CV> static AccShape accumulate_shape() {
  static AccShape cache[64] = {};
  static std::mutex mu;
  int dev = 0; HIP_CHECK(hipGetDevice(&dev));
  if (dev < 0 || dev >= 64) dev = 0;
  std::lock_guard<std::mutex> lk(mu);
  if (!cache[dev].lanes) {
    int cus = 0, blocks = 0, lds_cu = 0, lds_blk = 0;
    HIP_CHECK(hipDeviceGetAttribute(&cus, hipDeviceAttributeMultiprocessorCount, dev));
    HIP_CHECK(hipOccupancyMaxActiveBlocksPerMultiprocessor(&blocks, k_accumulate<CV>, 256, 0));
    if (blocks < 1) blocks = 1;
    if (hipDeviceGetAttribute(&lds_cu, hipDeviceAttributeMaxSharedMemoryPerMultiprocessor, dev) != hipSuccess || lds_cu <= 0) { (void)hipGetLastError(); lds_cu = 0; }
    if (hipDeviceGetAttribute(&lds_blk, hipDeviceAttributeMaxSharedMemoryPerBlock, dev) != hipSuccess || lds_blk <= 0) { (void)hipGetLastError(); lds_blk = 64 * 1024; }
    {
      hipDeviceProp_t prop;
      if (hipGetDeviceProperties(&prop, dev) == hipSuccess && !strncmp(prop.gcnArchName, "gfx950", 6)) {
        if (lds_cu < 160 * 1024) lds_cu = 160 * 1024;
        if (lds_blk < 160 * 1024) lds_blk = 160 * 1024;
      } else (void)hipGetLastError();
    }
    int cap = CV::MAX_WAVES;
    if (msm_env().occ) cap = msm_env().occ;
    unsigned lds = 0;
    if (cap >= 1 && cap < blocks && lds_cu > 0) {
      const unsigned slice = (unsigned)(lds_cu / (cap + 1) + 1024);
      if ((size_t)slice * cap <= (size_t)lds_cu && slice <= (unsigned)lds_blk) {
        blocks = cap; lds = slice;
        if (lds > 48 * 1024) HIP_CHECK(hipFuncSetAttribute((const void *)k_accumulate<CV>, hipFuncAttributeMaxDynamicSharedMemorySize, (int)lds));
      }
    }
    {
      const unsigned need = 4u * 2u * CV::BASE_WORDS * 64u * 4u;
      if (lds < need) lds = need;
      if (lds > 48 * 1024) HIP_CHECK(hipFuncSetAttribute((const void *)k_accumulate<CV>, hipFuncAttributeMaxDynamicSharedMemorySize, (int)lds));
      int blk2 = 0;
      HIP_CHECK(hipOccupancyMaxActiveBlocksPerMultiprocessor(&blk2, k_accumulate<CV>, 256, lds));
      if (blk2 >= 1 && blk2 < blocks) blocks = blk2;
    }
    cache[dev] = AccShape{(size_t)cus * blocks * 256, lds};
  }
  return cache[dev];
}
template <class CV> static size_t accumulate_lanes() { return accumulate_shape<CV>().lanes; }

static bool msm_poison() { static const bool on = getenv("AVRF_MSM_POISON") != nullptr; return on; }
static void poison(void *p, size_t bytes, int which) {
  if (!msm_poison() || !p) return;
  if (const char *e = getenv("AVRF_MSM_POISON_SKIP")) { if (atoi(e) == which) return; }
  HIP_CHECK(hipMemset(p, 0xA5, bytes)); if (!getenv("AVRF_MSM_POISON_NOSYNC")) HIP_CHECK(hipDeviceSynchronize());
}
static void ws_buf(DevMem &m, size_t bytes, int which) {
  if (bytes <= m.cap) return;
  m.ensure(bytes);
  poison(m.p, bytes, which);
}

void MsmWorkspace::ensure(size_t n, const MsmPlan &p, size_t acc_bytes, size_t batch, size_t lanes_max, size_t part_bytes) {
  const size_t vwin = (size_t)p.nwin * batch;
  const size_t nbk = vwin * p.nb, nbits = vwin * p.c;
  const size_t need_n = vwin * n;
  const size_t ntiles = (n + tile_len_for(n, vwin) - 1) / tile_len_for(n, vwin);
  ws_buf(keys, need_n * 2 + 16, 1); ws_buf(sorted, need_n * 4 + 16, 2);
  ws_buf(hist, nbk * ntiles * 4 + 64, 3);
  ws_buf(cnts, nbk * 4, 4); ws_buf(offsets, nbk * 4, 5); ws_buf(heavy, nbk * 4, 6);
  ws_buf(win_tot, (vwin + 64) * 4, 7); ws_buf(lane_base, (vwin + 64) * 4, 8);
  plan_dev.ensure(64);
  ws_buf(buckets, nbk * acc_bytes, 9); ws_buf(rc, nbk * acc_bytes, 10);
  ws_buf(part, (lanes_max + nbk + 64) * (part_bytes ? part_bytes : acc_bytes) + 64, 11);
  ws_buf(bits, nbits * acc_bytes, 12); own.ensure(nbits * acc_bytes);
}

void MsmChain::ensure(size_t bytes) {
  if (!plan_host) { plan_host.ensure(64); plan_host.as()[0] = plan_host.as()[1] = 0; }
  if (!ev0) { HIP_CHECK(ev0.create()); HIP_CHECK(ev1.create()); }
  bits_host.ensure(bytes);
}

static void msm_collect(MsmWorkspace &ws, MsmChain &rec, hipStream_t stream) {
  if (ws.owns(rec)) { HIP_CHECK(hipStreamSynchronize(stream)); HIP_CHECK(hipGetLastError()); }
  HIP_CHECK(hipEventElapsedTime(&ws.accum_ms_last, rec.ev0, rec.ev1));
  rec.plan.lpb = (int)rec.plan_host.as()[0];
  ws.accum_ms_total += ws.accum_ms_last; ws.accum_launches++; ws.last_plan = rec.plan;
}

constexpr size_t MSM_TINY_TERMS = 2048, MSM_TINY_VECTORS = 32;
template <class CV>
__global__ void __launch_bounds__(256)
k_msm_tiny_bits(const uint32_t *__restrict__ bases, const uint32_t *__restrict__ scalars, uint32_t n, uint32_t stride, uint32_t *__restrict__ out) {
  extern __shared__ uint32_t lds[];
  const uint32_t p = blockIdx.x, v = blockIdx.y, t = threadIdx.x, T = blockDim.x, lane = t & 63, wv = t >> 6, nw = T >> 6;
  typename CV::acc_t acc = CV::identity();
  bool first = true;
#pragma unroll 1
  for (uint32_t k = t; k < n; k += T) {
    if (!((scalars[8 * ((size_t)v * stride + k) + (p >> 5)] >> (p & 31)) & 1u)) continue;
    const typename CV::base_t q = CV::load_base(bases + (size_t)k * CV::BASE_WORDS);
    acc = first ? CV::from_base(q, false) : CV::madd(acc, q, false);
    first = false;
  }
  uint32_t span = 1; while (span < n && span < 64) span <<= 1;
#pragma unroll 1
  for (uint32_t off = span >> 1; off >= 1; off >>= 1) acc = cv_add<CV>(acc, CV::shfl_down(acc, (int)off));
  if (nw > 1) {
    if (lane == 0) CV::store_acc(lds + wv * CV::ACC_WORDS, acc);
    __syncthreads();
    if (wv == 0) {
      acc = lane < nw ? CV::load_acc(lds + lane * CV::ACC_WORDS) : CV::identity();
#pragma unroll 1
      for (uint32_t off = nw >> 1; off >= 1; off >>= 1) acc = cv_add<CV>(acc, CV::shfl_down(acc, (int)off));
    }
  }
  if (t == 0) CV::store_acc(out + ((size_t)v * gridDim.x + p) * CV::ACC_WORDS, acc);
}

struct MsmLaunch {
  size_t batch = 1;
  int table_c = 0; size_t table_stride = 0;
  size_t scalar_stride = 0;
  const uint32_t *d_base_idx = nullptr;
  bool defer = false;
  int scalars_mont = 0;
};

template <class CV>
static int msm_device(const uint32_t *d_bases, const uint32_t *d_scalars, size_t n_in, int scalar_bits, MsmWorkspace &ws, MsmChain &rec, hipStream_t stream,
                      const MsmLaunch &o = MsmLaunch()) {
  const size_t batch = o.batch, scalar_stride = o.scalar_stride ? o.scalar_stride : n_in;
  const int table_c = o.table_c, scalars_mont = o.scalars_mont;
  const uint32_t *const d_base_idx = o.d_base_idx;
  MsmPlan p = msm_plan(n_in, scalar_bits);
  auto finish = [&]() { if (!o.defer) msm_collect(ws, rec, stream); };
  if (n_in <= MSM_TINY_TERMS && batch <= (CV::FIXED_TABLE ? (size_t)7 : MSM_TINY_VECTORS) && !table_c && !d_base_idx && !scalars_mont && msm_env().tiny) {
    p.c = 1; p.nwin = scalar_bits; p.nb = 1; p.lpb = 0;
    const size_t acc_b = (size_t)CV::ACC_WORDS * 4, nbits = (size_t)scalar_bits;
    ws.ensure(n_in, p, acc_b, batch, 256);
    rec.ensure(batch * nbits * acc_b); rec.plan_host.as()[0] = 0; rec.plan = p;
    HIP_CHECK(hipEventRecord(rec.ev0, stream));
    unsigned threads = 64; while (threads < n_in && threads < 256) threads <<= 1;
    hipLaunchKernelGGL(k_msm_tiny_bits<CV>, dim3((unsigned)nbits, (unsigned)batch), dim3(threads), (threads / 64) * acc_b, stream, d_bases, d_scalars, (uint32_t)n_in,
                       (uint32_t)scalar_stride, ws.bits.as());
    HIP_CHECK(hipEventRecord(rec.ev1, stream));
    HIP_CHECK(hipMemcpyAsync(rec.bits_host.p, ws.bits.p, batch * nbits * acc_b, hipMemcpyDeviceToHost, stream));
    finish();
    return (int)nbits;
  }
  const size_t lanes_target = accumulate_lanes<CV>();
  size_t n = n_in;
  uint32_t remap_n = 0, remap_stride = 0;
  dim3 b256(256);
  int dig_nwin = p.nwin;
  if (table_c) {
    dig_nwin = (scalar_bits + 1 + table_c - 1) / table_c;
    p.c = table_c; p.nb = 1 << (table_c - 1); p.nwin = 1;
    n = n_in * (size_t)dig_nwin;
    remap_n = (uint32_t)n_in; remap_stride = (uint32_t)o.table_stride;
  }
  using RV = typename CV::red;
  const bool red = CV::FIXED_TABLE && table_c != 0;
  const size_t acc_bytes = (size_t)(red ? (int)RV::ACC_WORDS : (int)CV::ACC_WORDS) * 4;
  const uint32_t vwin = (uint32_t)(p.nwin * batch);
  const size_t lanes_max = lanes_target + vwin + 256;
  if ((size_t)vwin * n >= 0xffff0000ull) throw HipFailure{hipErrorInvalidValue, __FILE__, __LINE__};
  ws.ensure(n, p, acc_bytes, batch, lanes_max, (size_t)CV::accum::PART_WORDS * 4);
  const uint32_t nbk = vwin * p.nb;
  const uint32_t tile_len = tile_len_for(n, vwin), ntiles = (uint32_t)((n + tile_len - 1) / tile_len);
  const size_t lds_bytes = (size_t)p.nb * 4;
  hipLaunchKernelGGL(k_digits, dim3((unsigned)((n_in + 255) / 256), (unsigned)batch), b256, 0, stream, d_scalars, (uint32_t)n_in, (uint32_t)scalar_stride,
                     p.c, dig_nwin, ws.keys.as<uint16_t>(), scalars_mont);
  hipLaunchKernelGGL(k_hist, dim3(ntiles, vwin), b256, lds_bytes, stream, ws.keys.as<uint16_t>(), (uint32_t)n, tile_len, p.c, ws.hist.as());
  hipLaunchKernelGGL(k_scan_tiles, dim3((unsigned)((p.nb + 255) / 256), vwin), b256, 0, stream, ws.hist.as(), ntiles, p.c, ws.cnts.as());
  hipLaunchKernelGGL(k_scan_offs, dim3(vwin), dim3(1024), 0, stream, ws.cnts.as(), (uint32_t)n, p.c, ws.offsets.as(), ws.win_tot.as());
  hipLaunchKernelGGL(k_plan, dim3(1), dim3(1024), 0, stream, ws.win_tot.as(), vwin, (uint32_t)lanes_target, (uint32_t)msm_env().per_min,
                     ws.lane_base.as(), ws.plan_dev.as());
  hipLaunchKernelGGL(k_scatter, dim3(8u * ((vwin + 7u) / 8u) * ntiles), b256, lds_bytes, stream, ws.keys.as<uint16_t>(), (uint32_t)n, tile_len, p.c, ws.hist.as(),
                     ws.offsets.as(), ws.sorted.as(), remap_n, remap_stride, d_base_idx, ntiles, vwin);
  rec.ensure((size_t)vwin * 3 * acc_bytes);
  if (CV::ZERO_IS_IDENTITY) HIP_CHECK(hipMemsetAsync(ws.buckets.p, 0, (size_t)nbk * acc_bytes, stream));
  HIP_CHECK(hipEventRecord(rec.ev0, stream));
  hipLaunchKernelGGL(k_accumulate<CV>, dim3((unsigned)((lanes_max + 255) / 256)), b256, accumulate_shape<CV>().lds, stream, d_bases, ws.sorted.as(),
                     ws.offsets.as(), ws.win_tot.as(), ws.lane_base.as(), ws.plan_dev.as(), vwin, (uint32_t)p.nb, (uint32_t)n, ws.part.as());
  HIP_CHECK(hipEventRecord(rec.ev1, stream));
  auto bucket_sums = [&](auto tag) {
    using BV = typename decltype(tag)::type;
    hipLaunchKernelGGL(k_bucket_sum<BV>, dim3((nbk + 255) / 256), b256, 0, stream, ws.offsets.as(), ws.cnts.as(), ws.lane_base.as(), ws.plan_dev.as(), nbk,
                       (uint32_t)p.nb, (uint32_t)n, ws.part.as(), ws.buckets.as(), ws.heavy.as());
    hipLaunchKernelGGL(k_heavy_sum<BV>, dim3(nbk < 1024 ? nbk : 1024), b256, 4 * acc_bytes, stream, ws.offsets.as(), ws.cnts.as(), ws.lane_base.as(),
                       ws.plan_dev.as(), (uint32_t)p.nb, (uint32_t)n, ws.part.as(), ws.buckets.as(), ws.heavy.as());
  };
  if (red) bucket_sums(type_tag<RV>{}); else bucket_sums(type_tag<CV>{});
  HIP_CHECK(hipMemcpyAsync(rec.plan_host.p, ws.plan_dev.p, 8, hipMemcpyDeviceToHost, stream));
  rec.plan = p;
  if constexpr (CV::WINDOW_SUMS) if (batch == 1 && msm_env().window_sums) {
    const uint32_t nb = (uint32_t)p.nb;
    const uint32_t wpw = nb >= 256 ? 16u : 1u, m = nb >= 256 ? nb / 256 : (nb >= 16 ? nb / 16 : 1u);
    const uint32_t nwaves = vwin * wpw;
    hipLaunchKernelGGL(k_wsum_q1<typename CV::suite>, dim3((nwaves + 3) / 4), b256, 0, stream, ws.buckets.as(), nb, m, wpw, nwaves, ws.rc.as());
    hipLaunchKernelGGL(k_wsum_q2<typename CV::suite>, dim3(vwin), dim3(64), 0, stream, ws.rc.as(), wpw, ws.bits.as());
    HIP_CHECK(hipMemcpyAsync(rec.bits_host.p, ws.bits.p, (size_t)vwin * 3 * acc_bytes, hipMemcpyDeviceToHost, stream));
    rec.wsum_lg = 4; while ((1u << rec.wsum_lg) < 16 * m) rec.wsum_lg++;
    finish();
    return -(int)vwin;
  }
  if (!ws.owns(rec)) throw HipFailure{hipErrorInvalidValue, __FILE__, __LINE__};
  const int h = (p.c - 1) / 2;
  const uint32_t tasks = (1u << h) + ((uint32_t)p.nb >> h);
  const int nbits = (int)vwin * p.c;
  if constexpr (CV::FIXED_TABLE) if (table_c) {
    uint32_t wps = 1;
    const uint32_t wps_max = batch <= msm_env().wsum_blk_max ? 4 : 1;
    while (wps < wps_max && (uint32_t)p.nb >= 64 * wps * 2) wps *= 2;
    if (wps > 1) {
      hipLaunchKernelGGL(k_wsum_blk<RV>, dim3((unsigned)batch), dim3(64 * wps), (size_t)wps * 2 * acc_bytes, stream, ws.buckets.as(),
                         (uint32_t)p.nb, ws.rc.as());
    } else {
      uint32_t lps_log = 6;
      while (lps_log > 2 && (batch << (lps_log - 1)) >= 2048 * 64) lps_log--;
      while ((1u << lps_log) > (uint32_t)p.nb) lps_log--;
      hipLaunchKernelGGL(k_wsum<RV>, dim3((unsigned)(((batch << lps_log) + 255) / 256)), b256, 0, stream, ws.buckets.as(), (uint32_t)p.nb,
                         (uint32_t)batch, lps_log, ws.rc.as());
    }
    HIP_CHECK(hipMemcpyAsync(rec.bits_host.p, ws.rc.p, batch * (size_t)RV::OUT_WORDS * 4, hipMemcpyDeviceToHost, stream));
    finish();
    return p.c;
  }
  if (p.nb <= 256 && batch >= 8) {
    hipLaunchKernelGGL(k_bits_direct<CV>, dim3(((unsigned)nbits + 127) / 128), dim3(128), 0, stream, ws.buckets.as(), p.c, (uint32_t)nbits, ws.bits.as());
  } else {
    hipLaunchKernelGGL(k_rowcol<CV>, dim3(((size_t)vwin * tasks * 64 + 255) / 256), b256, 0, stream, ws.buckets.as(), p.c, h,
                       vwin * tasks, ws.rc.as());
    hipLaunchKernelGGL(k_bits<CV>, dim3(((size_t)nbits * 64 + 255) / 256), b256, 0, stream, ws.buckets.as(), ws.rc.as(),
                       p.c, h, (uint32_t)nbits, ws.bits.as());
  }
  if (batch >= 8) {
    hipLaunchKernelGGL(k_horner<CV>, dim3(((unsigned)batch + 63) / 64), dim3(64), 0, stream, ws.bits.as(), (uint32_t)(p.nwin * p.c),
                       (uint32_t)batch, ws.rc.as());
    HIP_CHECK(hipMemcpyAsync(rec.bits_host.p, ws.rc.p, batch * acc_bytes, hipMemcpyDeviceToHost, stream));
  } else {
    HIP_CHECK(hipMemcpyAsync(rec.bits_host.p, ws.bits.p, (size_t)nbits * acc_bytes, hipMemcpyDeviceToHost, stream));
  }
  finish();
  return p.nwin * p.c;
}

template <class S>
static int msm_te_enqueue_impl(const te_pre_raw *d_pre, const uint32_t *d_scalars, size_t n, MsmWorkspace &ws, MsmChain &rec, hipStream_t stream) {
  rec.n = n; rec.ret = 0; rec.armed = true;
  MsmLaunch o; o.defer = true;
  if (n) rec.ret = msm_device<TeCurve<S>>((const uint32_t *)d_pre, d_scalars, n, S::Fr::BITS, ws, rec, stream, o);
  return 0;
}
template <class S>
static int msm_te_finish_impl(MsmWorkspace &ws, MsmChain &rec, hipStream_t stream, HostExt *out) {
  using HT = HostTe<S>;
  *out = HT::identity();
  if (!rec.armed) return -1;
  rec.disarm();
  if (rec.n == 0) return 0;
  msm_collect(ws, rec, stream);
  const int nbits = rec.ret, c = rec.plan.c, lg = rec.wsum_lg; const uint32_t *bh = rec.bits_host.as();
  HostExt acc = HT::identity();
  if (nbits < 0) {
    for (int w = -nbits - 1; w >= 0; w--) {
      for (int k = 0; k < c - lg; k++) acc = HT::dbl(acc);
      acc = HT::add(acc, HT::from_raw32(bh + ((size_t)w * 3 + 2) * 32));
      for (int k = 0; k < lg - 4; k++) acc = HT::dbl(acc);
      acc = HT::add(acc, HT::from_raw32(bh + ((size_t)w * 3 + 1) * 32));
      for (int k = 0; k < 4; k++) acc = HT::dbl(acc);
      acc = HT::add(acc, HT::from_raw32(bh + (size_t)w * 3 * 32));
    }
  } else for (int i = nbits - 1; i >= 0; i--) {
    acc = HT::dbl(acc);
    acc = HT::add(acc, HT::from_raw32(bh + (size_t)i * 32));
  }
  *out = acc;
  return 0;
}

int msm_te_enqueue(int suite, const te_pre_raw *d_pre, const uint32_t *d_scalars, size_t n, MsmWorkspace &ws, MsmChain &rec, hipStream_t stream) {
  if (suite < 0 || suite >= AVRF_N_SUITES) return -1;
  return with_suite(suite, [&](auto tag) { using S = typename decltype(tag)::type; return msm_te_enqueue_impl<S>(d_pre, d_scalars, n, ws, rec, stream); });
}
int msm_te_finish(int suite, MsmWorkspace &ws, MsmChain &rec, hipStream_t stream, HostExt *out) {
  if (suite < 0 || suite >= AVRF_N_SUITES) return -1;
  return with_suite(suite, [&](auto tag) { using S = typename decltype(tag)::type; return msm_te_finish_impl<S>(ws, rec, stream, out); });
}
template <class S>
static int msm_te_small_vectors_impl(const te_pre_raw *d_pre, const uint32_t *d_scalars, size_t n, size_t nv, MsmWorkspace &ws, hipStream_t stream, HostExt *out) {
  using HT = HostTe<S>;
  if (!n || n > MSM_TINY_TERMS || !nv || nv > MSM_TINY_VECTORS || !msm_env().tiny) return -1;
  MsmLaunch o; o.batch = nv; o.scalar_stride = n;
  const int nbits = msm_device<TeCurve<S>>((const uint32_t *)d_pre, d_scalars, n, S::Fr::BITS, ws, ws.own, stream, o);
  ws.own.disarm();
  const uint32_t *bh = ws.own.bits_host.as();
  parallel_for(nv, [&](size_t v) {
    HostExt acc = HT::identity();
    for (int i = nbits - 1; i >= 0; i--) { acc = HT::dbl(acc); acc = HT::add(acc, HT::from_raw32(bh + ((size_t)v * nbits + i) * 32)); }
    out[v] = acc;
  });
  return 0;
}
int msm_te_small_vectors(int suite, const te_pre_raw *d_pre, const uint32_t *d_scalars, size_t n, size_t n_vectors, MsmWorkspace &ws, hipStream_t stream,
                         HostExt *out) {
  if (suite < 0 || suite >= AVRF_N_SUITES) return -1;
  return with_suite(suite, [&](auto tag) { using S = typename decltype(tag)::type; return msm_te_small_vectors_impl<S>(d_pre, d_scalars, n, n_vectors, ws, stream, out); });
}
bool msm_te_pending_supported(int suite) {
  if (suite < 0 || suite >= AVRF_N_SUITES || !msm_env().window_sums) return false;
  return with_suite(suite, [&](auto tag) { using S = typename decltype(tag)::type; return (bool)TeCurve<S>::WINDOW_SUMS; });
}
int msm_te_device(int suite, const te_pre_raw *d_pre, const uint32_t *d_scalars, size_t n,
                  MsmWorkspace &ws, hipStream_t stream, HostExt *out) {
  if (int e = msm_te_enqueue(suite, d_pre, d_scalars, n, ws, ws.own, stream)) return e;
  return msm_te_finish(suite, ws, ws.own, stream, out);
}


template <class C>
__global__ void __launch_bounds__(256) k_g1_bases(const uint8_t *__restrict__ xy, uint32_t n, uint32_t *__restrict__ out, uint32_t *__restrict__ flag) {
  using Fq = typename C::Fq; constexpr int N = Fq::N;
  uint32_t i = blockIdx.x * blockDim.x + threadIdx.x;
  if (i >= n) return;
  const uint32_t *src = reinterpret_cast<const uint32_t *>(xy + (size_t)i * N * 8);
  fpn<N> x = fp_load<N>(src), y = fp_load<N>(src + N);
  if (ge_p<Fq>(x) || ge_p<Fq>(y)) atomicOr(flag, 1u);
  fp_store<N>(out + (size_t)i * 2 * N, fp_to_mont<Fq>(x)); fp_store<N>(out + (size_t)i * 2 * N + N, fp_to_mont<Fq>(y));
}

template <class C>
__global__ void __launch_bounds__(64) k_g1_decompress(const uint8_t *__restrict__ comp, uint32_t n, uint8_t *__restrict__ out_xy, uint8_t *__restrict__ ok) {
  using Fq = typename C::Fq; constexpr int N = Fq::N, FQB = 4 * N;
  const uint32_t i = blockIdx.x * blockDim.x + threadIdx.x;
  if (i >= n) return;
  const uint8_t *b = comp + (size_t)i * FQB;
  uint8_t le[FQB]; bool big, inf;
  if (FQB == 48) {
    inf = b[0] & 0x40; big = b[0] & 0x20;
    if (!(b[0] & 0x80)) { ok[i] = 0; return; }
    for (int k = 0; k < FQB; k++) le[k] = b[FQB - 1 - k];
    le[FQB - 1] &= 0x1f;
  } else {
    inf = b[FQB - 1] & 0x40; big = b[FQB - 1] & 0x80;
    for (int k = 0; k < FQB; k++) le[k] = b[k];
    le[FQB - 1] &= 0x3f;
  }
  fpn<N> x;
  for (int k = 0; k < N; k++) x.v[k] = (uint32_t)le[4 * k] | ((uint32_t)le[4 * k + 1] << 8) | ((uint32_t)le[4 * k + 2] << 16) | ((uint32_t)le[4 * k + 3] << 24);
  uint32_t *o = reinterpret_cast<uint32_t *>(out_xy + (size_t)i * 2 * FQB);
  if (inf) {
    const bool good = !big && fp_is_zero(x);
    fp_store<N>(o, fp_zero<N>()); fp_store<N>(o + N, fp_zero<N>());
    ok[i] = good ? 2 : 0; return;
// ... 275 lines not shown
    const uint32_t *q = tmp + ((size_t)(m - m0) * lanes + lane) * 3 * N;
    const fpn<N> zz = fp_load<N>(q), zzz = fp_load<N>(q + N);
    if (fp_is_zero(zz)) { fp_store<N>(o, fp_zero<N>()); fp_store<N>(o + N, fp_zero<N>()); continue; }
    const fpn<N> dinv = fp_mul<Fq>(inv, fp_load<N>(q + 2 * N));
    inv = fp_mul<Fq>(inv, fp_mul<Fq>(zz, zzz));
    fp_store<N>(o, fp_mul<Fq>(fp_load<N>(o), fp_mul<Fq>(dinv, zzz)));
    fp_store<N>(o + N, fp_mul<Fq>(fp_load<N>(o + N), fp_mul<Fq>(dinv, zz)));
  }
}
template <class C> static void build_direct_impl(const uint32_t *d_bases, G1DirectTable *t, hipStream_t stream) {
  constexpr int N = C::Fq::N;
  const size_t n = t->n; const uint32_t rows = (uint32_t)t->rows;
  if (t->points >= 0x7fffffffull) throw HipFailure{hipErrorInvalidValue, __FILE__, __LINE__};
  HIP_CHECK(hipMalloc(&t->d, t->bytes));
  DevMem rowbase((size_t)rows * n * 2 * N * 4);
  build_g1_table(t->curve, d_bases, n, t->c, (int)rows, rowbase.as(), stream);
  const uint32_t lanes = (uint32_t)(rows * n), K = 128;
  DevMem tmp((size_t)K * lanes * 3 * N * 4);
  uint32_t mmax = 0; for (uint32_t w = 0; w < rows; w++) mmax = t->mult[w] > mmax ? t->mult[w] : mmax;
  for (uint32_t m0 = 0; m0 < mmax; m0 += K)
    hipLaunchKernelGGL(k_g1_multiples<C>, dim3((lanes + 63) / 64), dim3(64), 0, stream, (const uint32_t *)rowbase.as(), (uint32_t)n, rows, *t, m0, K, t->d, tmp.as(), lanes);
  HIP_CHECK(hipStreamSynchronize(stream));
  HIP_CHECK(hipGetLastError());
  HIP_CHECK(tmp.release()); HIP_CHECK(rowbase.release());
}
void build_g1_direct_table(int curve, const uint32_t *d_bases, size_t n, int c, G1DirectTable *t, hipStream_t stream) {
  free_g1_direct_table(t);
  g1_direct_table_shape(curve, n, c, t);
  if (curve == 0) build_direct_impl<G1Bls12381>(d_bases, t, stream); else build_direct_impl<G1Bn254>(d_bases, t, stream);
}
void free_g1_direct_table(G1DirectTable *t) { if (t->d) (void)hipFree(t->d); t->d = nullptr; }

constexpr uint32_t DIRECT_ZERO = 0xffffffffu;
__global__ void __launch_bounds__(256) k_direct_index(const uint32_t *__restrict__ scalars, uint32_t n, uint32_t stride, G1DirectTable t, uint32_t *__restrict__ idx, int mont,
                                                      const uint32_t *__restrict__ base_idx) {
  const uint32_t i = blockIdx.x * blockDim.x + threadIdx.x;
  if (i >= n) return;
  const uint32_t bat = blockIdx.y, rows = (uint32_t)t.rows, tn = (uint32_t)t.n;
  const int c = t.c;
  uint32_t s[9];
  const uint4 *p = reinterpret_cast<const uint4 *>(scalars + 8 * ((size_t)bat * stride + i));
  const uint4 a = p[0], b = p[1];
  s[0] = a.x; s[1] = a.y; s[2] = a.z; s[3] = a.w; s[4] = b.x; s[5] = b.y; s[6] = b.z; s[7] = b.w; s[8] = 0;
  if (mont) {
    fp v;
#pragma unroll
    for (int k = 0; k < 8; k++) v.v[k] = s[k];
    v = mont == 1 ? fp_from_mont<FqBandersnatch>(v) : fp_from_mont<FqBabyJubJub>(v);
#pragma unroll
    for (int k = 0; k < 8; k++) s[k] = v.v[k];
  }
  uint32_t *o = idx + ((size_t)bat * n + i) * rows;
  const uint32_t ib = base_idx ? base_idx[(size_t)bat * n + i] : i;
  const uint32_t nb = 1u << (c - 1), mask = (1u << c) - 1;
  uint32_t carry = 0;
  for (uint32_t w = 0; w < rows; w++) {
    const int bit = (int)w * c;
    uint32_t v = 0;
    if (bit < 256) {
      const int li = bit >> 5, sh = bit & 31;
      const uint64_t two = (uint64_t)s[li] | ((uint64_t)(li + 1 < 9 ? s[li + 1] : 0u) << 32);
      v = (uint32_t)(two >> sh) & mask;
    }
    v += carry;
    uint32_t m, sign = 0;
    if (v > nb) { m = (1u << c) - v; sign = 0x80000000u; carry = 1; } else { m = v; carry = 0; }
    o[w] = (m == 0 || m > t.mult[w] || ib >= tn) ? DIRECT_ZERO : (uint32_t)(t.off[w] + (uint64_t)(m - 1) * tn + ib) | sign;
  }
}

template <class CV>
__global__ void __launch_bounds__(256, CV::MIN_WAVES)
k_accumulate_direct(const uint32_t *__restrict__ table, const uint32_t *__restrict__ idx, uint32_t E, uint32_t lpv, uint32_t per, uint32_t batch,
                    uint32_t *__restrict__ part) {
  using AC = typename CV::accum; using acc_t = typename AC::acc_t; using base_t = typename CV::base_t;
  const uint32_t t = blockIdx.x * blockDim.x + threadIdx.x;
  const uint32_t vec = t / lpv, r = t - vec * lpv;
  extern __shared__ uint32_t acc_lds[];
  constexpr int BW = CV::BASE_WORDS, CH = BW / 4;
  uint32_t *wbuf = acc_lds + (threadIdx.x >> 6) * (2 * BW * 64);
  const uint32_t lane = threadIdx.x & 63;
  const bool live = vec < batch;
  const size_t v0 = (size_t)(live ? vec : 0) * E;
  uint32_t cnt = 0; size_t e0 = v0;
  if (live && (uint64_t)r * per < E) { e0 = v0 + (size_t)r * per; cnt = (uint64_t)r * per + per <= E ? per : (uint32_t)(E - (uint64_t)r * per); }
  auto issue = [&](uint32_t ix, uint32_t slot) {
    const uint32_t *src = table + (size_t)(ix == DIRECT_ZERO ? 0u : (ix & 0x7fffffffu)) * BW;
#pragma unroll
    for (int c = 0; c < CH; c++)
      __builtin_amdgcn_global_load_lds((const __attribute__((address_space(1))) void *)(src + 4 * c),
                                       (__attribute__((address_space(3))) void *)(wbuf + slot * (BW * 64) + c * 256), 16, 0, 0);
  };
  auto fetch = [&](uint32_t slot) {
    uint32_t w[BW];
#pragma unroll
    for (int c = 0; c < CH; c++) {
      const uint4 v = *reinterpret_cast<const uint4 *>(wbuf + slot * (BW * 64) + c * 256 + lane * 4);
      w[4 * c] = v.x; w[4 * c + 1] = v.y; w[4 * c + 2] = v.z; w[4 * c + 3] = v.w;
    }
    return CV::base_from_words(w);
  };
  acc_t acc = AC::identity();
  uint32_t ix = cnt ? idx[e0] : DIRECT_ZERO;
  uint32_t ix1 = cnt > 1 ? idx[e0 + 1] : DIRECT_ZERO;
  if (cnt) issue(ix, 0);
  for (uint32_t k = 0; k < cnt; k++) {
    const uint32_t cix = ix;
    asm volatile("s_waitcnt vmcnt(0) lgkmcnt(0)" ::: "memory");
    const base_t cur = fetch(k & 1);
    ix = ix1;
    if (k + 1 < cnt) issue(ix, (k + 1) & 1);
    if (k + 2 < cnt) ix1 = idx[e0 + k + 2];
    if (cix != DIRECT_ZERO) acc = AC::madd(acc, cur, (cix & 0x80000000u) != 0);
  }
  if (t < batch * lpv) AC::store_part(part + (size_t)t * AC::PART_WORDS, acc);
}
template <class RV>
__global__ void __launch_bounds__(64, RV::RED_WAVES)
k_direct_reduce(const uint32_t *__restrict__ part, uint32_t lpv, uint32_t *__restrict__ out) {
  using acc_t = typename RV::acc_t;
  const uint32_t vec = blockIdx.x, t = threadIdx.x;
  acc_t a = RV::identity();
#pragma unroll 1
  for (uint32_t k = t; k < lpv; k += 64) a = cv_add<RV>(a, RV::accum::load_part(part + ((size_t)vec * lpv + k) * RV::accum::PART_WORDS));
  a = wave_sum<RV>(a);
  if (t == 0) RV::store_out(out + (size_t)vec * RV::OUT_WORDS, a);
}
template <class C>
static int msm_g1_direct_impl(const G1DirectTable &t, const uint32_t *d_scalars, size_t n, size_t scalar_stride, MsmWorkspace &ws, hipStream_t stream,
                              uint8_t *out_xy, size_t batch, int scalars_mont, const uint32_t *d_base_idx) {
  using CV = G1Curve<C>; using RV = typename CV::red; using HG = HostG1<C>;
  if (!n || !batch) return -1;
  const size_t rows = (size_t)t.rows, E = n * rows;
  if (E * batch >= 0xffff0000ull || (!d_base_idx && n > t.n)) throw HipFailure{hipErrorInvalidValue, __FILE__, __LINE__};
  const AccShape shape = accumulate_shape<CV>();
  size_t lpv = shape.lanes / batch; if (lpv > 1024) lpv = 1024; if (lpv < 1) lpv = 1;
  const size_t per = (E + lpv - 1) / lpv, lanes = batch * lpv;
  MsmChain &rec = ws.own;
  MsmPlan p; p.c = t.c; p.nwin = 1; p.nb = 1; p.lpb = (int)per;
  ws.ensure(E, p, (size_t)RV::OUT_WORDS * 4 > (size_t)RV::ACC_WORDS * 4 ? (size_t)RV::OUT_WORDS * 4 : (size_t)RV::ACC_WORDS * 4, batch, lanes + 256,
            (size_t)CV::accum::PART_WORDS * 4);
  static std::once_flag once[2];
  std::call_once(once[t.curve ? 1 : 0], [&]() {
    if (shape.lds > 48 * 1024) HIP_CHECK(hipFuncSetAttribute((const void *)k_accumulate_direct<CV>, hipFuncAttributeMaxDynamicSharedMemorySize, (int)shape.lds));
  });
  hipLaunchKernelGGL(k_direct_index, dim3((unsigned)((n + 255) / 256), (unsigned)batch), dim3(256), 0, stream, d_scalars, (uint32_t)n, (uint32_t)(scalar_stride ? scalar_stride : n),
                     t, ws.sorted.as(), scalars_mont, d_base_idx);
  HIP_CHECK(hipEventRecord(rec.ev0, stream));
  hipLaunchKernelGGL(k_accumulate_direct<CV>, dim3((unsigned)((lanes + 255) / 256)), dim3(256), shape.lds, stream, (const uint32_t *)t.d, ws.sorted.as(),
                     (uint32_t)E, (uint32_t)lpv, (uint32_t)per, (uint32_t)batch, ws.part.as());
  HIP_CHECK(hipEventRecord(rec.ev1, stream));
  hipLaunchKernelGGL(k_direct_reduce<RV>, dim3((unsigned)batch), dim3(64), 0, stream, ws.part.as(), (uint32_t)lpv, ws.rc.as());
  HIP_CHECK(hipMemcpyAsync(rec.bits_host.p, ws.rc.p, batch * (size_t)RV::OUT_WORDS * 4, hipMemcpyDeviceToHost, stream));
  rec.plan_host.as()[0] = (uint32_t)per;
  rec.plan = p;
  msm_collect(ws, rec, stream);
  std::vector<typename HG::Pt> res(batch);
  for (size_t b = 0; b < batch; b++) res[b] = HG::from_raw32(rec.bits_host.as() + b * 4 * C::Fq::N);
  HG::to_affine_bytes_batch(res.data(), batch, out_xy);
  return 0;
}
int msm_g1_direct_device(const G1DirectTable &t, const uint32_t *d_scalars, size_t n, size_t scalar_stride, MsmWorkspace &ws, hipStream_t stream,
                         uint8_t *out_xy, size_t batch, int scalars_mont, const uint32_t *d_base_idx) {
  if (t.curve == 0) return msm_g1_direct_impl<G1Bls12381>(t, d_scalars, n, scalar_stride, ws, stream, out_xy, batch, scalars_mont, d_base_idx);
  return msm_g1_direct_impl<G1Bn254>(t, d_scalars, n, scalar_stride, ws, stream, out_xy, batch, scalars_mont, d_base_idx);
}

int msm_g1_fixed_device(int curve, const uint32_t *d_table, int table_c, size_t table_stride, const uint32_t *d_scalars, size_t n,
                        size_t scalar_stride, MsmWorkspace &ws, hipStream_t stream, uint8_t *out_xy, size_t batch, const uint32_t *d_base_idx,
                        int scalars_mont) {
  MsmLaunch o; o.batch = batch; o.table_c = table_c; o.table_stride = table_stride; o.scalar_stride = scalar_stride; o.d_base_idx = d_base_idx; o.scalars_mont = scalars_mont;
  if (curve == 0) return msm_g1_impl<G1Bls12381>(d_table, d_scalars, n, ws, stream, out_xy, o);
  if (curve == 1) return msm_g1_impl<G1Bn254>(d_table, d_scalars, n, ws, stream, out_xy, o);
  return -1;
}

}
```

ark_vrf_amd/csrc/proto_dev.h:

```cpp
#pragma once
#include "sha512_dev.h"
#include "shake_dev.h"
#include "sha256_dev.h"
#include "te.h"
#include <type_traits>

#define fp_mul fp_mul_nf
#define fp_sqr fp_sqr_nf
#define fp_inv fp_inv_nf
#define fp_to_mont fp_to_mont_nf
#define fp_from_mont fp_from_mont_nf
#define fp_is_negative_mont fp_is_negative_mont_nf
#define fp_from_wide_mont fp_from_wide_mont_nf
#define te_to_aff te_to_aff_nf
#define te_make_pre te_make_pre_nf
#include "sw_map.h"
#include "fpu_te.h"

namespace avrf {

enum : uint8_t {
  DS_TINY = 0x00, DS_THIN = 0x01, DS_PEDERSEN = 0x02, DS_NONCE_EXPAND = 0x10, DS_NONCE = 0x11, DS_PEDERSEN_BLINDING = 0x12,
  DS_POINT_TO_HASH = 0x20, DS_DELINEARIZE = 0x30, DS_CHALLENGE = 0x40, DS_BATCH_VERIFY = 0x50
};
enum { FLAG_RANGE = 1, FLAG_IDENTITY = 2, FLAG_SCALAR = 4, FLAG_CURVE = 8 };

struct BatchDev {
  const uint8_t *pks_xy;
  const uint8_t *ios_xy;
  const uint32_t *io_off;
  const uint8_t *ads;
  const uint32_t *ad_off;
  const uint8_t *proofs;
  const uint8_t *sks;
  uint32_t n;
  const te_pre *fixed;
  uint8_t *records;
  const uint8_t *weights;
  te_ext *tabs;
  uint32_t first;
};
struct Seed64 { uint64_t w[8]; };
template <class S> using suite_tr = std::conditional_t<S::XOF_SHAKE, Shake128, std::conditional_t<S::TR_SHA256, Sha256, Sha512>>;

template <class S, class T> AVRF_DI void absorb_point_xy(T &h, const fp &x, const fp &y) {
  using Fq = typename S::Fq;
  if constexpr (S::SW_CODEC) {
    absorb_sw_enc(h, sw_encode_te<S>(fp_to_mont<Fq>(x), fp_to_mont<Fq>(y)));
    return;
  }
  uint32_t sign = fp_is_negative_plain<Fq>(x) ? 0x80000000u : 0u;
#pragma unroll
  for (int i = 0; i < 8; i++) tr_u32le(h, y.v[i] | (i == 7 ? sign : 0u));
}
template <class T> AVRF_DI void absorb_sw_enc(T &h, const sw_enc &e) {
#pragma unroll
  for (int i = 0; i < 8; i++) tr_u32le(h, e.x.v[i]);
  tr_byte(h, e.flag);
}
template <class S, class T> AVRF_DI void absorb_generator(T &h) {
  for (int i = 0; i < S::POINT_LEN; i++) tr_byte(h, S::G_ENC[i]);
}
template <class T> AVRF_DI void absorb_fp_le(T &h, const fp &a) {
#pragma unroll
  for (int i = 0; i < 8; i++) tr_u32le(h, a.v[i]);
}
template <class S> AVRF_DI uint32_t point_flags(const fp &x, const fp &y) {
  using Fq = typename S::Fq;
  uint32_t f = 0;
  if (ge_p<Fq>(x) || ge_p<Fq>(y)) f |= FLAG_RANGE;
  fp one = fp_zero(); one.v[0] = 1;
  if constexpr (S::SW_NATIVE) { if (fp_is_zero(x) && fp_is_zero(y)) f |= FLAG_IDENTITY; }
  else if (fp_is_zero(x) && fp_eq(y, one)) f |= FLAG_IDENTITY;
  return f;
}

template <class S, class T> AVRF_DI void tr_base(T &h, uint8_t scheme, bool schnorr, const fp &pkx, const fp &pky,
                                        const uint8_t *ios_xy, uint32_t m, const uint8_t *ad, uint32_t adl, uint32_t *flags) {
  tr_init(h);
  for (int i = 0; i < S::SUITE_ID_LEN; i++) tr_byte(h, S::SUITE_ID[i]);
  tr_byte(h, scheme);
  tr_u64le(h, (uint64_t)m + (schnorr ? 1 : 0));
  uint32_t f = 0;
  if constexpr (S::SW_CODEC) if (m == 1) {
    fp xs[3], ys[3]; sw_enc enc[3];
    xs[0] = fp_load_le(ios_xy); ys[0] = fp_load_le(ios_xy + 32); xs[1] = fp_load_le(ios_xy + 64); ys[1] = fp_load_le(ios_xy + 96);
    if (schnorr) { xs[2] = pkx; ys[2] = pky; } else { xs[2] = xs[0]; ys[2] = ys[0]; }
    sw_encode_te_many<S, 3>(xs, ys, enc);
    if (schnorr) { absorb_generator<S>(h); f |= point_flags<S>(xs[2], ys[2]); absorb_sw_enc(h, enc[2]); }
    f |= point_flags<S>(xs[0], ys[0]) | point_flags<S>(xs[1], ys[1]);
    absorb_sw_enc(h, enc[0]); absorb_sw_enc(h, enc[1]);
    tr_u64le(h, (uint64_t)adl);
    tr_bytes(h, ad, adl);
    *flags |= f;
    return;
  }
  if (schnorr) {
    absorb_generator<S>(h);
    f |= point_flags<S>(pkx, pky);
    absorb_point_xy<S>(h, pkx, pky);
  }
  for (uint32_t i = 0; i < m; i++) {
    const uint8_t *p = ios_xy + 128 * (size_t)i;
    fp x = fp_load_le(p), y = fp_load_le(p + 32);
    f |= point_flags<S>(x, y); absorb_point_xy<S>(h, x, y);
    x = fp_load_le(p + 64); y = fp_load_le(p + 96);
    f |= point_flags<S>(x, y); absorb_point_xy<S>(h, x, y);
  }
  tr_u64le(h, (uint64_t)adl);
  tr_bytes(h, ad, adl);
  *flags |= f;
}
template <class S, class T> AVRF_DI void tr_base(T &h, uint8_t scheme, bool schnorr, const uint8_t *pk_xy,
                                        const uint8_t *ios_xy, uint32_t m, const uint8_t *ad, uint32_t adl, uint32_t *flags) {
  fp x = fp_zero(), y = fp_zero();
  if (schnorr) { x = fp_load_le(pk_xy); y = fp_load_le(pk_xy + 32); }
  tr_base<S>(h, scheme, schnorr, x, y, ios_xy, m, ad, adl, flags);
}
template <class T> AVRF_DI auto delin_seed(const T &h) {
  T hd = h; tr_byte(hd, DS_DELINEARIZE); return tr_reader(hd);
}
template <class R> AVRF_DI fp xof128(R &rd, uint32_t i) {
  uint32_t w[4]; rd_chunk16(rd, i, w);
  fp a = fp_zero(); a.v[0] = w[0]; a.v[1] = w[1]; a.v[2] = w[2]; a.v[3] = w[3]; return a;
}
template <class T> AVRF_DI fp challenge_finish(const T &h) {
  auto rd = tr_reader(h); return xof128(rd, 0);
}
template <class T> AVRF_DI void squeeze64(const T &h, fp &lo, fp &hi) {
  auto rd = tr_reader(h);
#pragma unroll
  for (int k = 0; k < 4; k++) {
    uint32_t w[4]; rd_chunk16(rd, (uint32_t)k, w);
    fp &dst = k < 2 ? lo : hi;
#pragma unroll
    for (int i = 0; i < 4; i++) dst.v[4 * (k & 1) + i] = w[i];
  }
}
template <class S, class T> AVRF_DN fp nonce(fp sk_plain, T t) {
  using Fr = typename S::Fr;
  T te = t; tr_byte(te, DS_NONCE_EXPAND); absorb_fp_le(te, sk_plain);
  fp lo, hi;
  squeeze64(te, lo, hi);
  T tn = t; tr_byte(tn, DS_NONCE);
  absorb_fp_le(tn, lo); absorb_fp_le(tn, hi);
  squeeze64(tn, lo, hi);
  static_assert((Fr::BITS + 128 + 7) / 8 == 48, "nonce length");
#pragma unroll
  for (int i = 4; i < 8; i++) hi.v[i] = 0;
  return fp_from_wide_mont<Fr>(lo, hi);
}


template <class S> AVRF_DI te_pre pre_from_xy(const uint8_t *xy) {
  using Fq = typename S::Fq;
  return te_make_pre<S>(fp_to_mont<Fq>(fp_load_le(xy)), fp_to_mont<Fq>(fp_load_le(xy + 32)));
}
template <class S> struct Chain {
#ifndef AVRF_NO_UNSAT_CHAINS
  static constexpr bool U = !S::SW_NATIVE && FuAsm<typename S::Fq>::value;
#else
  static constexpr bool U = false;
#endif
  struct sat_t { te_ext p; };
  using acc_t = std::conditional_t<U, teu4<S>, te_ext>;
  static AVRF_DI acc_t identity() { if constexpr (U) return teu4_identity<S>(); else return te_identity<S>(); }
  static AVRF_DI acc_t dbl(const acc_t &a) { if constexpr (U) return teu4_dbl<S>(a); else return te_dbl<S>(a); }
  template <int N> static AVRF_DI acc_t dbln(acc_t a) {
#pragma unroll 1
    for (int t = 0; t < N; t++) a = dbl(a);
    return a;
  }
  static AVRF_DI acc_t add(const acc_t &a, const te_ext &e) { if constexpr (U) return teu4_add_sat<S>(a, e); else return te_add<S>(a, e); }
  static AVRF_DI acc_t madd(const acc_t &a, const te_pre &q) { if constexpr (U) return teu4_madd_pre<S>(a, q); else return te_madd<S>(a, q); }
  static AVRF_DI te_ext finish(const acc_t &a) { if constexpr (U) return teu4_to_ext<S>(a); else return a; }
};
template <class S> AVRF_DN te_ext te_smul(te_pre p, fp k, int nbits) {
  te_ext tab[16];
  tab[0] = te_identity<S>(); tab[1] = te_from_pre<S>(p);
  for (int i = 2; i < 16; i++) tab[i] = te_madd<S>(tab[i - 1], p);
  using CH = Chain<S>;
  typename CH::acc_t acc = CH::identity();
  for (int w = (nbits + 3) / 4 - 1; w >= 0; w--) {
    acc = CH::template dbln<4>(acc);
    uint32_t d = (k.v[w >> 3] >> (4 * (w & 7))) & 15u;
    if (d) acc = CH::add(acc, tab[d]);
  }
  return CH::finish(acc);
}
enum { ITEM_TAB_SLOTS = 40 };
template <class S> AVRF_DN te_ext te_smul_ws(te_ext *tab, te_pre p, fp k, int nbits) {
  te_ext cur = te_from_pre<S>(p);
  store_ext(tab + 1, cur);
// ... 74 lines not shown
```

ark_vrf_amd/csrc/te_quad.h:

```cpp
#pragma once
#include "te.h"
#include "curves.h"

namespace avrf {

template <int P0, int P1, int P2, int P3> AVRF_DI fp qperm(const fp &a) {
  fp r;
#pragma unroll
  for (int i = 0; i < 8; i++) r.v[i] = (uint32_t)__builtin_amdgcn_mov_dpp((int)a.v[i], P0 | (P1 << 2) | (P2 << 4) | (P3 << 6), 0xf, 0xf, true);
  return r;
}
AVRF_DI fp fp_sel(bool c, const fp &a, const fp &b) {
  fp r;
#pragma unroll
  for (int i = 0; i < 8; i++) r.v[i] = c ? a.v[i] : b.v[i];
  return r;
}
template <class S> AVRF_DI fp q_identity(uint32_t j) { return (j & 1) ? fp_one<typename S::Fq>() : fp_zero(); }

template <class S> __device__ __noinline__ static fp q_add(fp a, fp b, uint32_t j) {
  using Fq = typename S::Fq;
  const fp m1 = fp_mul<Fq>(a, b);
  const fp sa = fp_add<Fq>(a, qperm<1, 0, 3, 2>(a)), sb = fp_add<Fq>(b, qperm<1, 0, 3, 2>(b));
  const bool l2 = j == 2;
// ... 55 lines not shown
    if (w) { acc = q_dbl<S>(acc, j); acc = q_dbl<S>(acc, j); acc = q_dbl<S>(acc, j); }
    fp e = tab[0];
#pragma unroll
    for (uint32_t i = 1; i < 8; i++) e = fp_sel(d == i, tab[i], e);
    acc = q_add<S>(acc, e, j);
  }
  return acc;
}

AVRF_DI fp fp_shfl_down(const fp &a, int delta) {
  fp r;
#pragma unroll
  for (int i = 0; i < 8; i++) r.v[i] = __shfl_down(a.v[i], delta);
  return r;
}
AVRF_DI fp fp_shfl_xor(const fp &a, int mask) {
  fp r;
#pragma unroll
  for (int i = 0; i < 8; i++) r.v[i] = __shfl_xor(a.v[i], mask);
  return r;
}

template <int P0, int P1, int P2, int P3, int L> AVRF_DI fu<L> fu_qperm(const fu<L> &a) {
  fu<L> r;
#pragma unroll
  for (int i = 0; i < L; i++) r.v[i] = __builtin_amdgcn_mov_dpp(a.v[i], P0 | (P1 << 2) | (P2 << 4) | (P3 << 6), 0xf, 0xf, true);
  return r;
}
template <int L> AVRF_DI fu<L> fu_sel(bool c, const fu<L> &a, const fu<L> &b) {
  fu<L> r;
#pragma unroll
  for (int i = 0; i < L; i++) r.v[i] = c ? a.v[i] : b.v[i];
  return r;
}
template <class S> __device__ __noinline__ static fuF<typename S::Fq> qu_add(fuF<typename S::Fq> a, fuF<typename S::Fq> b, uint32_t j) {
  using Fq = typename S::Fq;
  constexpr int L = UL<Fq>::L, SH = UL<Fq>::SH;
  const fu<L> m1 = fu_mul<Fq>(a, b);
  const fu<L> sa = fu_add<L>(a, fu_qperm<1, 0, 3, 2>(a)), sb = fu_carry<Fq>(fu_add<L>(b, fu_qperm<1, 0, 3, 2>(b)));
  const bool l2 = j == 2;
  const fu<L> m2 = fu_mul<Fq>(fu_sel<L>(l2, m1, sa), fu_sel<L>(l2, fu_slice<Fq, SH>(S::D), sb));
  const fu<L> A = fu_qperm<0, 0, 0, 0>(m1), B = fu_qperm<1, 1, 1, 1>(m1), D = fu_qperm<3, 3, 3, 3>(m1);
  const fu<L> C = fu_qperm<2, 2, 2, 2>(m2), Ep = fu_qperm<0, 0, 0, 0>(m2);
  fu<L> X, Y;
#pragma unroll
  for (int i = 0; i < L; i++) {
    X.v[i] = j == 0 ? Ep.v[i] : (j == 1 ? B.v[i] : D.v[i]);
    const int32_t y1 = S::A_KIND == 0 ? A.v[i] : -A.v[i];
    Y.v[i] = j == 0 ? A.v[i] + B.v[i] : (j == 1 ? y1 : (l2 ? -C.v[i] : C.v[i]));
  }
  fu<L> U = fu_carry<Fq>(fu_sub<L>(X, Y));
  if (S::A_KIND == 1) {
    uint32_t h[L - 1];
#pragma unroll
    for (int i = 0; i < L - 1; i++) h[i] = (uint32_t)B.v[i] + 5u * (uint32_t)A.v[i];
    U = fu_sel<L>(j == 1, fu_carry_u<Fq>(h, B.v[L - 1] + 5 * A.v[L - 1]), U);
  }
  return fu_mul<Fq>(fu_qperm<0, 1, 0, 3>(U), fu_qperm<3, 2, 1, 2>(U));
}

template <class S> struct QuadSat {
  using el = fp;
  static AVRF_DI el identity(uint32_t j) { return q_identity<S>(j); }
  static AVRF_DI el add(const el &a, const el &b, uint32_t j) { return q_add<S>(a, b, j); }
  static AVRF_DI el sel(bool c, const el &a, const el &b) { return fp_sel(c, a, b); }
  static AVRF_DI el shfl_down(const el &a, int d) { return fp_shfl_down(a, d); }
  static AVRF_DI el shfl_xor(const el &a, int m) { return fp_shfl_xor(a, m); }
  static AVRF_DI el load(const uint32_t *p) { return fp_load(p); }
  static AVRF_DI void store(uint32_t *p, const el &v) { fp_store(p, v); }
  static AVRF_DI el load_part(const uint32_t *part, size_t k, int j) {
    if constexpr (TeCurve<S>::accum::PART_WORDS == 32) return fp_load(part + k * 32 + j * 8);
    else return teu_load_part_coord<S>(part + k * TEU_PART_WORDS, j);
  }
};
template <class S> struct QuadUns {
  using Fq = typename S::Fq;
  static constexpr int L = UL<Fq>::L;
  using el = fu<L>;
  static AVRF_DI el identity(uint32_t j) { return (j & 1) ? fu_const<Fq>(UL<Fq>::ONE) : fu_zero<L>(); }
  static AVRF_DI el add(const el &a, const el &b, uint32_t j) { return qu_add<S>(a, b, j); }
  static AVRF_DI el sel(bool c, const el &a, const el &b) { return fu_sel<L>(c, a, b); }
  static AVRF_DI el shfl_down(const el &a, int d) { el r;
#pragma unroll
    for (int i = 0; i < L; i++) r.v[i] = __shfl_down(a.v[i], d);
    return r; }
  static AVRF_DI el shfl_xor(const el &a, int m) { el r;
#pragma unroll
    for (int i = 0; i < L; i++) r.v[i] = __shfl_xor(a.v[i], m);
    return r; }
  static AVRF_DI el load(const uint32_t *p) { const fp v = fp_load(p); return fu_slice<Fq, 0>(v.v); }
  static AVRF_DI void store(uint32_t *p, const el &v) { fp r; fu_to_packed<Fq>(r.v, v); fp_store(p, r); }
  static AVRF_DI el load_part(const uint32_t *part, size_t k, int j) { return teu_load_part_coord_raw<S>(part + k * TEU_PART_WORDS, j); }
};
#if !defined(AVRF_NO_UNSAT) && !defined(AVRF_NO_UNSAT_QUAD)
template <class S> using Quad = std::conditional_t<FuAsm<typename S::Fq>::value && !S::SW_NATIVE, QuadUns<S>, QuadSat<S>>;
#else
template <class S> using Quad = QuadSat<S>;
#endif

template <class S> AVRF_DI typename Quad<S>::el q_wave_sum(typename Quad<S>::el v, uint32_t q, uint32_t j) {
  using Q = Quad<S>;
#pragma unroll 1
  for (int off = 8; off >= 1; off >>= 1) {
    const typename Q::el o = Q::shfl_down(v, 4 * off);
    if ((int)q < off) v = Q::add(v, o, j);
  }
  return v;
}
template <class S> AVRF_DI typename Quad<S>::el q_wave_sum2(const typename Quad<S>::el &a, const typename Quad<S>::el &b, uint32_t q, uint32_t j) {
  using Q = Quad<S>;
  const bool lowq = q < 8;
  const typename Q::el send = Q::sel(lowq, b, a);
  const typename Q::el got = Q::shfl_xor(send, 32);
  typename Q::el v = Q::add(Q::sel(lowq, a, b), got, j);
#pragma unroll 1
  for (int off = 4; off >= 1; off >>= 1) {
    const typename Q::el o = Q::shfl_down(v, 4 * off);
    if ((int)(q & 7) < off) v = Q::add(v, o, j);
  }
  return v;
}
template <class S> AVRF_DI typename Quad<S>::el q_wave_suffix(typename Quad<S>::el v, uint32_t q, uint32_t j) {
  using Q = Quad<S>;
#pragma unroll 1
  for (int off = 1; off < 16; off <<= 1) {
    const typename Q::el o = Q::shfl_down(v, 4 * off);
    if ((int)q + off < 16) v = Q::add(v, o, j);
  }
  return v;
}

template <class S>
__global__ void __launch_bounds__(256)
k_wsum_q1(const uint32_t *__restrict__ buckets, uint32_t nb, uint32_t m, uint32_t wpw, uint32_t nwaves, uint32_t *__restrict__ out) {
  const uint32_t gw = (blockIdx.x * blockDim.x + threadIdx.x) >> 6, lane = threadIdx.x & 63, q = lane >> 2, j = lane & 3;
  if (gw >= nwaves) return;
  const uint32_t v = gw / wpw, wi = gw - v * wpw;
  using Q = Quad<S>; using el = typename Q::el;
  const uint32_t *B = buckets + (size_t)v * nb * 32;
  el Sx = Q::identity(j), J = Q::identity(j);
#pragma unroll 1
  for (int k = (int)m - 1; k >= 0; k--) {
    const uint32_t b0 = wi * 16 * m + q + 16 * (uint32_t)k;
    if (b0 < nb) Sx = Q::add(Sx, Q::load(B + (size_t)b0 * 32 + j * 8), j);
    if (k > 0) J = Q::add(J, Sx, j);
  }
  const el A = q_wave_suffix<S>(Sx, q, j);
  const el V = q_wave_sum2<S>(A, J, q, j);
  uint32_t *o = out + (size_t)gw * 3 * 32 + j * 8;
  if (q == 0) { Q::store(o, V); Q::store(o + 64, A); }
  if (q == 8) Q::store(o + 32, V);
}

template <class S>
__global__ void __launch_bounds__(64)
k_wsum_q2(const uint32_t *__restrict__ trip, uint32_t wpw, uint32_t *__restrict__ out) {
  const uint32_t v = blockIdx.x, lane = threadIdx.x & 63, q = lane >> 2, j = lane & 3;
  using Q = Quad<S>; using el = typename Q::el;
  el v1 = Q::identity(j), v2 = v1, y = v1;
  if (q < wpw) {
    const uint32_t *t = trip + ((size_t)v * wpw + q) * 3 * 32 + j * 8;
    v1 = Q::load(t); v2 = Q::load(t + 32); y = Q::load(t + 64);
  }
  const el P12 = q_wave_sum2<S>(v1, v2, q, j);
  el A = q_wave_suffix<S>(y, q, j);
  if (q == 0) A = Q::identity(j);
  const el P3 = q_wave_sum<S>(A, q, j);
  uint32_t *o = out + (size_t)v * 3 * 32 + j * 8;
  if (q == 0) { Q::store(o, P12); Q::store(o + 64, P3); }
  if (q == 8) Q::store(o + 32, P12);
}

template <class S> AVRF_DI void q_heavy_sum(const uint32_t *__restrict__ part, size_t p0, uint32_t np, uint32_t *__restrict__ dst, uint32_t *lds) {
  const uint32_t t = threadIdx.x, lane = t & 63, q = lane >> 2, j = lane & 3, gq = t >> 2, wv = t >> 6;
  using Q = Quad<S>; using el = typename Q::el;
  el a = Q::identity(j);
#pragma unroll 1
  for (uint32_t k = gq; k < np; k += 64) a = Q::add(a, Q::load_part(part, p0 + k, (int)j), j);
  a = q_wave_sum<S>(a, q, j);
  if (q == 0) Q::store(lds + wv * 32 + j * 8, a);
  __syncthreads();
  if (t < 4) {
#pragma unroll 1
    for (uint32_t w = 1; w < 4; w++) a = Q::add(a, Q::load(lds + w * 32 + j * 8), j);
    Q::store(dst + j * 8, a);
  }
  __syncthreads();
}

}
```

ark_vrf_amd/csrc/vrf_batch.hip:

```cpp
#include "vrf_batch.h"
#include "proto_dev.h"
#include "suite_dispatch.h"

#ifndef AVRF_TU_SUITE
#error "vrf_batch.hip is built once per suite: -DAVRF_TU_SUITE=<id> (csrc/Makefile)"
#endif
namespace avrf {

template <class S>
__global__ void __launch_bounds__(128)
k_thin_prepare(BatchDev b, uint32_t *__restrict__ c_out, uint32_t *__restrict__ z_out, uint32_t *__restrict__ flags) {
  using Fr = typename S::Fr;
  uint32_t j = blockIdx.x * blockDim.x + threadIdx.x;
  if (j >= b.n) return;
  uint32_t io0 = b.io_off[j], io1 = b.io_off[j + 1], m = io1 - io0;
  uint32_t ad0 = b.ad_off[j], adl = b.ad_off[j + 1] - ad0;
  uint32_t f = 0;
  suite_tr<S> h; tr_init(h);
  for (int i = 0; i < S::SUITE_ID_LEN; i++) tr_byte(h, S::SUITE_ID[i]);
  tr_byte(h, DS_THIN);
  tr_u64le(h, (uint64_t)m + 1);
  absorb_generator<S>(h);
  sw_enc enc[4]; bool have_enc = false;
  if constexpr (S::SW_CODEC) if (m == 1) {
    const uint8_t *p = b.ios_xy + 128 * (size_t)io0, *pr = b.proofs + 96 * (size_t)j, *pk = b.pks_xy + 64 * (size_t)j;
    const fp xs[4] = {fp_load_le(pk), fp_load_le(p), fp_load_le(p + 64), fp_load_le(pr)};
    const fp ys[4] = {fp_load_le(pk + 32), fp_load_le(p + 32), fp_load_le(p + 96), fp_load_le(pr + 32)};
    sw_encode_te_many<S, 4>(xs, ys, enc); have_enc = true;
  }
  {
    fp x = fp_load_le(b.pks_xy + 64 * (size_t)j), y = fp_load_le(b.pks_xy + 64 * (size_t)j + 32);
    f |= point_flags<S>(x, y);
    if (have_enc) absorb_sw_enc(h, enc[0]); else absorb_point_xy<S>(h, x, y);
  }
  for (uint32_t i = 0; i < m; i++) {
    const uint8_t *p = b.ios_xy + 128 * (size_t)(io0 + i);
    fp x = fp_load_le(p), y = fp_load_le(p + 32);
    f |= point_flags<S>(x, y); if (have_enc) absorb_sw_enc(h, enc[1]); else absorb_point_xy<S>(h, x, y);
    x = fp_load_le(p + 64); y = fp_load_le(p + 96);
    f |= point_flags<S>(x, y); if (have_enc) absorb_sw_enc(h, enc[2]); else absorb_point_xy<S>(h, x, y);
  }
  tr_u64le(h, (uint64_t)adl);
  tr_bytes(h, b.ads + ad0, adl);
  if (m) {
    auto rd = delin_seed(h);
    for (uint32_t i = 0; i < m; i++) {
      uint32_t w[4]; rd_chunk16(rd, i, w);
      uint4 *o = reinterpret_cast<uint4 *>(z_out + 4 * (size_t)(io0 + i));
      *o = make_uint4(w[0], w[1], w[2], w[3]);
    }
  }
  {
    const uint8_t *pr = b.proofs + 96 * (size_t)j;
    fp x = fp_load_le(pr), y = fp_load_le(pr + 32), s = fp_load_le(pr + 64);
    if (point_flags<S>(x, y) & FLAG_RANGE) f |= FLAG_RANGE;
    if (ge_p<Fr>(s)) f |= FLAG_SCALAR;
    tr_byte(h, DS_CHALLENGE);
    if (have_enc) absorb_sw_enc(h, enc[3]); else absorb_point_xy<S>(h, x, y);
    auto rd = tr_reader(h);
    uint32_t w[4]; rd_chunk16(rd, 0, w);
    uint4 *o = reinterpret_cast<uint4 *>(c_out + 4 * (size_t)j);
    *o = make_uint4(w[0], w[1], w[2], w[3]);
    if (b.records) {
      uint4 *r = reinterpret_cast<uint4 *>(b.records + 64 * (size_t)j);
      const uint4 *sp = reinterpret_cast<const uint4 *>(pr + 64);
      r[0] = make_uint4(w[0], w[1], w[2], w[3]); r[1] = make_uint4(0, 0, 0, 0); r[2] = sp[0]; r[3] = sp[1];
    }
  }
  if (f) atomicOr(flags, f);
}

AVRF_DI fp fp_from_u128(const uint32_t *w) {
  fp a = fp_zero(); uint4 v = *reinterpret_cast<const uint4 *>(w);
  a.v[0] = v.x; a.v[1] = v.y; a.v[2] = v.z; a.v[3] = v.w; return a;
}
template <class S> AVRF_DI void emit_term(uint32_t *scalars, te_pre *pre, uint32_t t, const fp &scalar_plain, const uint8_t *xy) {
  using Fq = typename S::Fq;
  fp_store(scalars + 8 * (size_t)t, scalar_plain);
  fp x = fp_to_mont<Fq>(fp_load_le(xy)), y = fp_to_mont<Fq>(fp_load_le(xy + 32));
  store_pre(pre + t, te_make_pre<S>(x, y));
}

template <class S>
__global__ void __launch_bounds__(128)
k_thin_terms(BatchDev b, Seed64 seed, uint64_t j0, const uint32_t *__restrict__ c_in, const uint32_t *__restrict__ z_in,
             uint32_t *__restrict__ scalars, te_pre *__restrict__ pre, uint32_t *__restrict__ gpart) {
  using Fr = typename S::Fr;
  __shared__ fp red[128];
  uint32_t j = blockIdx.x * blockDim.x + threadIdx.x;
  fp ws = fp_zero();
  if (j < b.n) {
    uint32_t io0 = b.io_off[j], m = b.io_off[j + 1] - io0;
    uint64_t gj = j0 + j;
    uint32_t ww[4];
    if (b.weights) { const uint4 v = *reinterpret_cast<const uint4 *>(b.weights + 16 * (size_t)j); ww[0] = v.x; ww[1] = v.y; ww[2] = v.z; ww[3] = v.w; }
    else { uint64_t blk[8]; sha512_xof_block(seed.w, gj >> 2, blk); digest_le128(blk, (int)(gj & 3), ww); }
    fp w_plain = fp_zero(); w_plain.v[0] = ww[0]; w_plain.v[1] = ww[1]; w_plain.v[2] = ww[2]; w_plain.v[3] = ww[3];
    fp w = fp_to_mont<Fr>(w_plain);
    fp c = fp_to_mont<Fr>(fp_from_u128(c_in + 4 * (size_t)j));
    const uint8_t *pr = b.proofs + 96 * (size_t)j;
    fp s = fp_to_mont<Fr>(fp_load_le(pr + 64));
    fp wc = fp_mul<Fr>(w, c);
    ws = fp_mul<Fr>(w, s);
    uint32_t t = 2 * j + 2 * io0;
    emit_term<S>(scalars, pre, t, w_plain, pr);
    emit_term<S>(scalars, pre, t + 1, fp_from_mont<Fr>(wc), b.pks_xy + 64 * (size_t)j);
    for (uint32_t i = 0; i < m; i++) {
      fp z = fp_to_mont<Fr>(fp_from_u128(z_in + 4 * (size_t)(io0 + i)));
      const uint8_t *p = b.ios_xy + 128 * (size_t)(io0 + i);
      emit_term<S>(scalars, pre, t + 2 + 2 * i, fp_from_mont<Fr>(fp_mul<Fr>(wc, z)), p + 64);
      emit_term<S>(scalars, pre, t + 3 + 2 * i, fp_from_mont<Fr>(fp_neg<Fr>(fp_mul<Fr>(ws, z))), p);
    }
  }
  red[threadIdx.x] = ws;
  __syncthreads();
  for (int s2 = 64; s2 >= 1; s2 >>= 1) {
    if ((int)threadIdx.x < s2) red[threadIdx.x] = fp_add<Fr>(red[threadIdx.x], red[threadIdx.x + s2]);
    __syncthreads();
  }
  if (threadIdx.x == 0) fp_store(gpart + 8 * (size_t)blockIdx.x, red[0]);
}

template <class S>
__global__ void __launch_bounds__(256)
k_g_final(const uint32_t *__restrict__ gpart, uint32_t nparts, uint32_t *__restrict__ scalars, te_pre *__restrict__ pre,
          uint32_t t_last, int which_base) {
  using Fr = typename S::Fr; using Fq = typename S::Fq;
  __shared__ fp red[256];
  fp acc = fp_zero();
  for (uint32_t i = threadIdx.x; i < nparts; i += 256) acc = fp_add<Fr>(acc, fp_load(gpart + 8 * (size_t)i));
  red[threadIdx.x] = acc;
  __syncthreads();
  for (int s2 = 128; s2 >= 1; s2 >>= 1) {
    if ((int)threadIdx.x < s2) red[threadIdx.x] = fp_add<Fr>(red[threadIdx.x], red[threadIdx.x + s2]);
    __syncthreads();
  }
  if (threadIdx.x == 0) {
    fp_store(scalars + 8 * (size_t)t_last, fp_from_mont<Fr>(fp_neg<Fr>(red[0])));
    te_pre g;
    if (which_base == 0) { g.x = fp_const<Fq>(S::G_X); g.y = fp_const<Fq>(S::G_Y); g.k = fp_const<Fq>(S::G_K); }
    else { g.x = fp_const<Fq>(S::B_X); g.y = fp_const<Fq>(S::B_Y); g.k = fp_const<Fq>(S::B_K); }
    store_pre(pre + t_last, g);
  }
}



template <class S>
__global__ void __launch_bounds__(128)
k_ped_prepare(BatchDev b, uint32_t *__restrict__ c_out, uint8_t *__restrict__ merged_xy, uint32_t *__restrict__ flags) {
  using Fr = typename S::Fr;
  uint32_t j = blockIdx.x * blockDim.x + threadIdx.x;
  if (j >= b.n) return;
  uint32_t io0 = b.io_off[j], m = b.io_off[j + 1] - io0, ad0 = b.ad_off[j], adl = b.ad_off[j + 1] - ad0;
  const uint8_t *ios = b.ios_xy + 128 * (size_t)io0, *pr = b.proofs + 256 * (size_t)j;
  suite_tr<S> t; uint32_t f = 0;
  tr_base<S>(t, DS_PEDERSEN, false, nullptr, ios, m, b.ads + ad0, adl, &f);
  uint8_t *mo = merged_xy + 128 * (size_t)j;
  if (m == 1) {
    const uint4 *src = reinterpret_cast<const uint4 *>(ios); uint4 *dst = reinterpret_cast<uint4 *>(mo);
#pragma unroll
    for (int i = 0; i < 8; i++) dst[i] = src[i];
  } else if (m == 0) {
    fp zero = fp_zero(), one = fp_zero(); one.v[0] = S::SW_NATIVE ? 0 : 1;
    fp_store_le(mo, zero); fp_store_le(mo + 32, one); fp_store_le(mo + 64, zero); fp_store_le(mo + 96, one);
  } else {
    auto dseed = delin_seed(t);
    te_ext im = te_identity<S>(), om = te_identity<S>();
    for (uint32_t i = 0; i < m; i++) {
      te_pre pi = pre_from_xy<S>(ios + 128 * (size_t)i), po = pre_from_xy<S>(ios + 128 * (size_t)i + 64);
      if (i == 0) { im = te_madd<S>(im, pi); om = te_madd<S>(om, po); }
      else { fp z = xof128(dseed, i - 1); im = te_add<S>(im, te_smul<S>(pi, z, 128)); om = te_add<S>(om, te_smul<S>(po, z, 128)); }
    }
    te_aff ia = te_to_aff<S>(im), oa = te_to_aff<S>(om);
    store_xy<S>(mo, ia); store_xy<S>(mo + 64, oa);
  }
  fp ybx = fp_load_le(pr), yby = fp_load_le(pr + 32), rx = fp_load_le(pr + 64), ry = fp_load_le(pr + 96);
  fp okx = fp_load_le(pr + 128), oky = fp_load_le(pr + 160);
  f |= point_flags<S>(ybx, yby);
  f |= (point_flags<S>(rx, ry) | point_flags<S>(okx, oky)) & FLAG_RANGE;
  if (ge_p<Fr>(fp_load_le(pr + 192)) || ge_p<Fr>(fp_load_le(pr + 224))) f |= FLAG_SCALAR;
  if constexpr (S::SW_CODEC) {
    const fp xs[3] = {ybx, rx, okx}, ys[3] = {yby, ry, oky};
    sw_enc enc[3]; sw_encode_te_many<S, 3>(xs, ys, enc);
    absorb_sw_enc(t, enc[0]); tr_byte(t, DS_CHALLENGE); absorb_sw_enc(t, enc[1]); absorb_sw_enc(t, enc[2]);
  } else {
    absorb_point_xy<S>(t, ybx, yby);
    tr_byte(t, DS_CHALLENGE); absorb_point_xy<S>(t, rx, ry); absorb_point_xy<S>(t, okx, oky);
  }
  fp c = challenge_finish(t);
  *reinterpret_cast<uint4 *>(c_out + 4 * (size_t)j) = make_uint4(c.v[0], c.v[1], c.v[2], c.v[3]);
  if (b.records) {
    uint4 *r = reinterpret_cast<uint4 *>(b.records + 96 * (size_t)j);
    const uint4 *sp = reinterpret_cast<const uint4 *>(pr + 192);
    r[0] = make_uint4(c.v[0], c.v[1], c.v[2], c.v[3]); r[1] = make_uint4(0, 0, 0, 0); r[2] = sp[0]; r[3] = sp[1]; r[4] = sp[2]; r[5] = sp[3];
  }
  if (f) atomicOr(flags, f);
}

template <class S>
__global__ void __launch_bounds__(128)
k_ped_terms(BatchDev b, Seed64 seed, uint64_t j0, const uint32_t *__restrict__ c_in, const uint8_t *__restrict__ merged_xy,
            uint32_t *__restrict__ scalars, te_pre *__restrict__ pre, uint32_t *__restrict__ gpart, uint32_t *__restrict__ bpart) {
  using Fr = typename S::Fr;
  __shared__ fp red[128];
  uint32_t j = blockIdx.x * blockDim.x + threadIdx.x;
  fp us = fp_zero(), usb = fp_zero();
  if (j < b.n) {
    fp t_plain, u_plain;
    if (b.weights) { t_plain = fp_from_u128(reinterpret_cast<const uint32_t *>(b.weights + 32 * (size_t)j)); u_plain = fp_from_u128(reinterpret_cast<const uint32_t *>(b.weights + 32 * (size_t)j + 16)); }
    else {
      ShaReader rd; for (int i = 0; i < 8; i++) rd.seed[i] = seed.w[i]; rd.have = 0;
      t_plain = xof128(rd, (uint32_t)(2 * (j0 + j))); u_plain = xof128(rd, (uint32_t)(2 * (j0 + j) + 1));
    }
    fp tt = fp_to_mont<Fr>(t_plain), uu = fp_to_mont<Fr>(u_plain);
    fp c = fp_to_mont<Fr>(fp_from_u128(c_in + 4 * (size_t)j));
    const uint8_t *pr = b.proofs + 256 * (size_t)j, *mo = merged_xy + 128 * (size_t)j;
    fp s = fp_to_mont<Fr>(fp_load_le(pr + 192)), sb = fp_to_mont<Fr>(fp_load_le(pr + 224));
    uint32_t k = 5 * j;
    emit_term<S>(scalars, pre, k, fp_from_mont<Fr>(fp_mul<Fr>(tt, c)), mo + 64);
    emit_term<S>(scalars, pre, k + 1, t_plain, pr + 128);
    emit_term<S>(scalars, pre, k + 2, fp_from_mont<Fr>(fp_neg<Fr>(fp_mul<Fr>(tt, s))), mo);
    emit_term<S>(scalars, pre, k + 3, fp_from_mont<Fr>(fp_mul<Fr>(uu, c)), pr);
    emit_term<S>(scalars, pre, k + 4, u_plain, pr + 64);
    us = fp_mul<Fr>(uu, s); usb = fp_mul<Fr>(uu, sb);
  }
  red[threadIdx.x] = us;
  __syncthreads();
  for (int s2 = 64; s2 >= 1; s2 >>= 1) {
    if ((int)threadIdx.x < s2) red[threadIdx.x] = fp_add<Fr>(red[threadIdx.x], red[threadIdx.x + s2]);
    __syncthreads();
  }
  if (threadIdx.x == 0) fp_store(gpart + 8 * (size_t)blockIdx.x, red[0]);
  __syncthreads();
  red[threadIdx.x] = usb;
  __syncthreads();
  for (int s2 = 64; s2 >= 1; s2 >>= 1) {
    if ((int)threadIdx.x < s2) red[threadIdx.x] = fp_add<Fr>(red[threadIdx.x], red[threadIdx.x + s2]);
    __syncthreads();
  }
  if (threadIdx.x == 0) fp_store(bpart + 8 * (size_t)blockIdx.x, red[0]);
}

template <class S> void BatchOps<S>::ped_prepare(const BatchDev &b, uint32_t *d_c, uint8_t *d_merged, uint32_t *d_flags, hipStream_t st) {
  if (!b.n) return;
  dim3 g((b.n + 127) / 128), blk(128);
  hipLaunchKernelGGL(k_ped_prepare<S>, g, blk, 0, st, b, d_c, d_merged, d_flags);
}
template <class S> void BatchOps<S>::ped_terms(const BatchDev &b, const Seed64 &seed, uint64_t j0, const uint32_t *d_c, const uint8_t *d_merged,
                                               uint32_t *d_scalars, te_pre_raw *d_pre, uint32_t *d_gpart, uint32_t n_terms, hipStream_t st) {
  if (!b.n) return;
  dim3 g((b.n + 127) / 128), blk(128);
  uint32_t *bp = d_gpart + 8 * (size_t)g.x;
  hipLaunchKernelGGL(k_ped_terms<S>, g, blk, 0, st, b, seed, j0, d_c, d_merged, d_scalars, (te_pre *)d_pre, d_gpart, bp);
  hipLaunchKernelGGL(k_g_final<S>, dim3(1), dim3(256), 0, st, d_gpart, g.x, d_scalars, (te_pre *)d_pre, n_terms - 2, 0);
  hipLaunchKernelGGL(k_g_final<S>, dim3(1), dim3(256), 0, st, bp, g.x, d_scalars, (te_pre *)d_pre, n_terms - 1, 1);
}
template <class S> void BatchOps<S>::thin_prepare(const BatchDev &b, uint32_t *d_c, uint32_t *d_z, uint32_t *d_flags, hipStream_t st) {
  if (!b.n) return;
  dim3 g((b.n + 127) / 128), blk(128);
  hipLaunchKernelGGL(k_thin_prepare<S>, g, blk, 0, st, b, d_c, d_z, d_flags);
}
template <class S> void BatchOps<S>::thin_terms(const BatchDev &b, const Seed64 &seed, uint64_t j0, const uint32_t *d_c, const uint32_t *d_z,
                                                uint32_t *d_scalars, te_pre_raw *d_pre, uint32_t *d_gpart, uint32_t n_terms, hipStream_t st) {
  if (!b.n) return;
  dim3 g((b.n + 127) / 128), blk(128);
  hipLaunchKernelGGL(k_thin_terms<S>, g, blk, 0, st, b, seed, j0, d_c, d_z, d_scalars, (te_pre *)d_pre, d_gpart);
  hipLaunchKernelGGL(k_g_final<S>, dim3(1), dim3(256), 0, st, d_gpart, g.x, d_scalars, (te_pre *)d_pre, n_terms - 1, 0);
}
template struct BatchOps<suite_by_id<AVRF_TU_SUITE>::type>;

}
```

Measured before the change: 136.0 million.

## Fold MSM plan into waves and piggyback batch flags on record copy

When validation is off, the prepare kernels write one flags word per block into the tail of the record buffer. This removes the separate flags memset and the small device-to-host copy, since the flags now ride the record download and are OR-reduced on the host. For single-vector window-sum MSMs, the k_plan kernel is dropped: each wave recomputes the lane plan with shuffles inside the accumulate kernel. The bucket-sum and heavy-sum kernels are merged into one launch, and the lanes-per-bucket value is written into the window-sums output so the separate plan copy is skipped. The aim is fewer launches and copies per batch, at the cost of redundant per-wave plan computation and extra block-level synchronisation in prepare.

Result: slower. 133.9 million (-1.5%).

```diff
diff --git a/ark_vrf_amd/csrc/capi.hip b/ark_vrf_amd/csrc/capi.hip
--- a/ark_vrf_amd/csrc/capi.hip
+++ b/ark_vrf_amd/csrc/capi.hip
@@ -40,7 +40,7 @@
   b.sks = c->d_sks.as<uint8_t>(); b.n = (uint32_t)c->n;
   b.fixed = (const te_pre *)c->d_fixed.p;
   b.tabs = (te_ext *)c->d_tabs.p; b.first = 0;
-  b.weights = nullptr; b.records = nullptr;
+  b.weights = nullptr; b.records = nullptr; b.flag_blk = nullptr;
   return b;
 }
 
@@ -424,30 +424,42 @@
   c->run_t0 = now_us();
   const size_t n = c->n;
   BatchDev b = batch_of(c);
-  HIP_TRY(hipMemsetAsync(c->d_flags.p, 0, 4, c->stream));
+  const bool host_weights = suite_host_weights(c->suite);
+  const uint32_t flag_words = (c->validate <= 0 && !c->wire_pending && !host_weights) ? (uint32_t)((n + 127) / 128) : 0;
+  c->flag_words = flag_words;
+  if (!flag_words) HIP_TRY(hipMemsetAsync(c->d_flags.p, 0, 4, c->stream));
   validate_staged(c, kind, nullptr);
-  const bool host_weights = suite_host_weights(c->suite);
   const size_t recsz = kind_facts(kind).record();
   uint8_t prefix[64]; const size_t pl = batch_prefix(c->suite, prefix);
   if (!host_weights) {
-    HIP_TRY(c->d_rec.ensure(n * recsz)); HIP_TRY(c->h_msg.ensure(pl + n * recsz));
+    HIP_TRY(c->d_rec.ensure(n * recsz + 4 * (size_t)flag_words)); HIP_TRY(c->h_msg.ensure(pl + n * recsz + 4 * (size_t)flag_words));
     b.records = c->d_rec.as<uint8_t>();
+    if (flag_words) b.flag_blk = (uint32_t *)(c->d_rec.as<uint8_t>() + n * recsz);
   }
   launch_prepare(c, kind, b);
   if (!host_weights) {
     memcpy(c->h_msg.p, prefix, pl);
-    HIP_TRY(hipMemcpyAsync(c->h_msg.as<uint8_t>() + pl, c->d_rec.p, n * recsz, hipMemcpyDeviceToHost, c->stream));
+    HIP_TRY(hipMemcpyAsync(c->h_msg.as<uint8_t>() + pl, c->d_rec.p, n * recsz + 4 * (size_t)flag_words, hipMemcpyDeviceToHost, c->stream));
     c->h_msg_len = pl + n * recsz;
   } else HIP_TRY(hipMemcpyAsync(c->h_c.p, c->d_c.p, n * 16, hipMemcpyDeviceToHost, c->stream));
-  HIP_TRY(hipMemcpyAsync(c->h_flags.p, c->d_flags.p, 4, hipMemcpyDeviceToHost, c->stream));
+  if (!flag_words) HIP_TRY(hipMemcpyAsync(c->h_flags.p, c->d_flags.p, 4, hipMemcpyDeviceToHost, c->stream));
   c->run_begin_us = now_us() - c->run_t0;
   c->run_phase = 1;
   return AVRF_OK;
 }
 
+static uint32_t batch_flags(const avrf_ctx *c) {
+  if (!c->n) return 0;
+  if (!c->flag_words) return *c->h_flags.as<uint32_t>();
+  uint32_t flags = 0;
+  const uint8_t *fw = c->h_msg.as<uint8_t>() + c->h_msg_len;
+  for (uint32_t i = 0; i < c->flag_words; i++) { uint32_t w; memcpy(&w, fw + 4 * (size_t)i, 4); flags |= w; }
+  return flags;
+}
+
 int batch_collect(avrf_ctx *c, int kind) {
   if (!c || c->staged_kind != kind || c->run_phase != 1) return AVRF_ERR_BAD_ARG;
-  if (c->n && *c->h_flags.as<uint32_t>()) { c->run_phase = 0; return AVRF_INVALID_DATA; }
+  if (batch_flags(c)) { c->run_phase = 0; return AVRF_INVALID_DATA; }
   if (c->wire_pending) {
     c->wire_pending = false;
     if (c->n && c->h_flags.as<uint32_t>()[2]) { c->run_phase = 0; c->staged_kind = 0; return AVRF_INVALID_DATA; }
@@ -772,7 +784,7 @@
   if (st == AVRF_OK) st = batch_end(c, Thin);
   c->unit_weights = false;
   if (st != AVRF_OK && st != AVRF_VERIFICATION_FAILURE) { c->run_phase = 0; return st; }
-  status_out[0] = *c->h_flags.as<uint32_t>() ? AVRF_INVALID_DATA : st;
+  status_out[0] = batch_flags(c) ? AVRF_INVALID_DATA : st;
   return AVRF_OK;
 }
 
@@ -794,7 +806,7 @@
   }
   HostExt r[2];
   if (int e = lane_msm_vectors(c, nt, 2, r)) return e;
-  status_out[0] = *c->h_flags.as<uint32_t>() ? AVRF_INVALID_DATA : (point_is_identity(c, r[0]) && point_is_identity(c, r[1])) ? AVRF_OK : AVRF_VERIFICATION_FAILURE;
+  status_out[0] = batch_flags(c) ? AVRF_INVALID_DATA : (point_is_identity(c, r[0]) && point_is_identity(c, r[1])) ? AVRF_OK : AVRF_VERIFICATION_FAILURE;
   return AVRF_OK;
 }
 
diff --git a/ark_vrf_amd/csrc/capi_internal.h b/ark_vrf_amd/csrc/capi_internal.h
--- a/ark_vrf_amd/csrc/capi_internal.h
+++ b/ark_vrf_amd/csrc/capi_internal.h
@@ -58,6 +58,7 @@
   std::vector<uint8_t> h_resp;
   avrf::DevBuf d_rec; avrf::PinBuf h_msg;
   size_t h_msg_len = 0;
+  uint32_t flag_words = 0;
   std::vector<uint8_t> h_weights; avrf::DevBuf d_weights;
   avrf::DevBuf d_c, d_z, d_flags, d_misc, d_out, d_status;
   avrf::DevBuf d_tabs;
diff --git a/ark_vrf_amd/csrc/msm.h b/ark_vrf_amd/csrc/msm.h
--- a/ark_vrf_amd/csrc/msm.h
+++ b/ark_vrf_amd/csrc/msm.h
@@ -59,6 +59,7 @@
   DevEvent ev0, ev1;
   MsmPlan plan = {0, 0, 0, 0}; int ret = 0;
   int wsum_lg = 4;
+  size_t lpb_word = 0;
   size_t n = 0;
   bool armed = false;
   void ensure(size_t bytes);
diff --git a/ark_vrf_amd/csrc/msm.hip b/ark_vrf_amd/csrc/msm.hip
--- a/ark_vrf_amd/csrc/msm.hip
+++ b/ark_vrf_amd/csrc/msm.hip
@@ -181,6 +181,26 @@
   if (t == 0) { lane_base[vwin] = carry_s; plan[0] = per; plan[1] = carry_s; plan[2] = 0; }
 }
 
+constexpr uint32_t PLAN_WAVE_WINDOWS = 64;
+struct PlanArgs { const uint32_t *win_tot; uint32_t vwin, lanes_target, per_min; };
+struct WavePlan { uint32_t per, lanes, tot, base; };
+AVRF_DI WavePlan wave_plan(const PlanArgs &a) {
+  const uint32_t l = threadIdx.x & 63;
+  const uint32_t tot = l < a.vwin ? a.win_tot[l] : 0;
+  uint32_t total = tot;
+#pragma unroll
+  for (int off = 32; off >= 1; off >>= 1) total += __shfl_xor(total, off);
+  uint32_t lt = a.lanes_target;
+  if (lt > 8 * a.vwin) lt -= a.vwin;
+  uint32_t per = total / lt + (total % lt != 0);
+  if (per < a.per_min) per = a.per_min;
+  const uint32_t mine = tot / per + (tot % per != 0);
+  uint32_t inc = mine;
+#pragma unroll
+  for (int off = 1; off < 64; off <<= 1) { const uint32_t x = __shfl_up(inc, off); if ((int)l >= off) inc += x; }
+  return WavePlan{per, (uint32_t)__shfl(inc, 63), tot, inc - mine};
+}
+
 __global__ void __launch_bounds__(256)
 k_scatter(const uint16_t *__restrict__ keys, uint32_t n, uint32_t tile_len, int c, const uint32_t *__restrict__ H,
           const uint32_t *__restrict__ offs, uint32_t *__restrict__ sorted, uint32_t remap_n, uint32_t remap_stride,
@@ -221,21 +241,33 @@
 
 
 
-template <class CV>
+template <class CV, bool WAVE_PLAN = false>
 __global__ void __launch_bounds__(256, CV::MIN_WAVES)
 k_accumulate(const uint32_t *__restrict__ bases, const uint32_t *__restrict__ sorted,
              const uint32_t *__restrict__ offs, const uint32_t *__restrict__ win_tot, const uint32_t *__restrict__ lane_base,
-             const uint32_t *__restrict__ plan, uint32_t vwin, uint32_t nb, uint32_t n, uint32_t *__restrict__ part) {
+             const uint32_t *__restrict__ plan, uint32_t vwin, uint32_t nb, uint32_t n, uint32_t *__restrict__ part,
+             uint32_t lanes_target, uint32_t per_min) {
   using AC = typename CV::accum;
   using acc_t = typename AC::acc_t; using base_t = typename CV::base_t;
   const uint32_t t = blockIdx.x * blockDim.x + threadIdx.x;
-  const uint32_t per = plan[0];
-  if (t >= plan[1]) return;
-  uint32_t lo = 0, hi = vwin;
-  while (hi - lo > 1) { uint32_t mid = (lo + hi) >> 1; if (lane_base[mid] <= t) lo = mid; else hi = mid; }
-  const uint32_t v = lo;
-  const uint32_t wbeg = v * n, wend = wbeg + win_tot[v];
-  const uint32_t e0 = wbeg + (t - lane_base[v]) * per;
+  uint32_t per, v, vbase, vtot, lo, hi;
+  if constexpr (WAVE_PLAN) {
+    const WavePlan wp = wave_plan(PlanArgs{win_tot, vwin, lanes_target, per_min});
+    per = wp.per; v = 0; vbase = 0; vtot = 0;
+    for (uint32_t k = 0; k < vwin; k++) {
+      const uint32_t bk = __builtin_amdgcn_readlane(wp.base, k), tk = __builtin_amdgcn_readlane(wp.tot, k);
+      if (bk <= t) { v = k; vbase = bk; vtot = tk; }
+    }
+    if (t >= wp.lanes) return;
+  } else {
+    per = plan[0];
+    if (t >= plan[1]) return;
+    lo = 0; hi = vwin;
+    while (hi - lo > 1) { uint32_t mid = (lo + hi) >> 1; if (lane_base[mid] <= t) lo = mid; else hi = mid; }
+    v = lo; vbase = lane_base[v]; vtot = win_tot[v];
+  }
+  const uint32_t wbeg = v * n, wend = wbeg + vtot;
+  const uint32_t e0 = wbeg + (t - vbase) * per;
   uint32_t e1 = e0 + per; if (e1 > wend) e1 = wend;
   const uint32_t *ow = offs + (size_t)v * nb;
   lo = 0; hi = nb;
@@ -346,6 +378,66 @@
   }
 }
 
+constexpr uint32_t HEAVY_BLOCKS = 256;
+template <class CV>
+__global__ void __launch_bounds__(256, CV::RED_WAVES)
+k_bucket_heavy_sum(const uint32_t *__restrict__ offs, const uint32_t *__restrict__ cnts, const uint32_t *__restrict__ win_tot, uint32_t vwin,
+                   uint32_t lanes_target, uint32_t per_min, uint32_t nslots, uint32_t nblk, uint32_t nb, uint32_t n,
+                   const uint32_t *__restrict__ part, uint32_t *__restrict__ buckets) {
+  static_assert(CV::QUAD && !CV::ZERO_IS_IDENTITY, "the merged reduction is the twisted-Edwards window-sum chain's");
+  using acc_t = typename CV::acc_t; using AC = typename CV::accum;
+  __shared__ uint32_t hv_slot[256], hv_p0[256], hv_np[256], hv_n, red[4 * 32];
+  const WavePlan wp = wave_plan(PlanArgs{win_tot, vwin, lanes_target, per_min});
+  const uint32_t per = wp.per, t = threadIdx.x;
+  if (blockIdx.x < nblk) {
+    const uint32_t slot = blockIdx.x * blockDim.x + t;
+    const uint32_t v = (slot < nslots ? slot : nslots - 1) / nb, vbase = __shfl(wp.base, v);
+    if (slot >= nslots) return;
+    const uint32_t cnt = cnts[slot];
+    if (!cnt) { CV::store_acc(buckets + (size_t)slot * CV::ACC_WORDS, CV::identity()); return; }
+    const uint32_t rel = offs[slot] - v * n;
+    const uint32_t lf = rel / per, ll = (rel + cnt - 1) / per, np = ll - lf + 1;
+    if (np > HEAVY_PARTIALS) return;
+    const size_t p0 = (size_t)vbase + lf + slot;
+    acc_t acc = AC::load_part(part + p0 * AC::PART_WORDS);
+#pragma unroll 1
+    for (uint32_t k = 1; k < np; k++) acc = cv_add<CV>(acc, AC::load_part(part + (p0 + k) * AC::PART_WORDS));
+    CV::store_acc(buckets + (size_t)slot * CV::ACC_WORDS, acc);
+    return;
+  }
+  const uint32_t h = blockIdx.x - nblk, H = gridDim.x - nblk;
+  for (uint32_t s0 = h; s0 < nslots; s0 += 256 * H) {
+    const uint32_t slot = s0 + t * H;
+    const uint32_t v = (slot < nslots ? slot : nslots - 1) / nb, vbase = __shfl(wp.base, v);
+    if (t == 0) hv_n = 0;
+    __syncthreads();
+    if (slot < nslots) {
+      const uint32_t cnt = cnts[slot];
+      if (cnt) {
+        const uint32_t rel = offs[slot] - v * n;
+        const uint32_t lf = rel / per, ll = (rel + cnt - 1) / per, np = ll - lf + 1;
+        if (np > HEAVY_PARTIALS) { const uint32_t k = atomicAdd(&hv_n, 1u); hv_slot[k] = slot; hv_p0[k] = vbase + lf + slot; hv_np[k] = np; }
+      }
+    }
+    __syncthreads();
+    const uint32_t nh = hv_n;
+    for (uint32_t i = 0; i < nh; i++)
+      q_heavy_sum<typename CV::suite>(part, hv_p0[i], hv_np[i], buckets + (size_t)hv_slot[i] * CV::ACC_WORDS, red);
+    __syncthreads();
+  }
+}
+
+template <class S>
+__global__ void __launch_bounds__(64)
+k_wsum_q2(const uint32_t *__restrict__ trip, uint32_t wpw, uint32_t *__restrict__ out, const uint32_t *__restrict__ plan,
+          const uint32_t *__restrict__ win_tot, uint32_t vwin, uint32_t lanes_target, uint32_t per_min) {
+  q_wsum_level2<S>(trip, wpw, out);
+  if (blockIdx.x == 0) {
+    const uint32_t per = plan ? plan[0] : wave_plan(PlanArgs{win_tot, vwin, lanes_target, per_min}).per;
+    if (threadIdx.x == 0) out[(size_t)gridDim.x * 3 * 32] = per;
+  }
+}
+
 
 template <class CV> AVRF_DI typename CV::acc_t wave_sum(typename CV::acc_t acc) {
 #pragma unroll 1
@@ -541,7 +633,16 @@
   if (!cache[dev].lanes) {
     int cus = 0, blocks = 0, lds_cu = 0, lds_blk = 0;
     HIP_CHECK(hipDeviceGetAttribute(&cus, hipDeviceAttributeMultiprocessorCount, dev));
-    HIP_CHECK(hipOccupancyMaxActiveBlocksPerMultiprocessor(&blocks, k_accumulate<CV>, 256, 0));
+    auto resident = [&](unsigned lds) {
+      int b = 0; HIP_CHECK(hipOccupancyMaxActiveBlocksPerMultiprocessor(&b, k_accumulate<CV>, 256, lds));
+      if constexpr (CV::WINDOW_SUMS) { int b2 = 0; HIP_CHECK(hipOccupancyMaxActiveBlocksPerMultiprocessor(&b2, k_accumulate<CV, true>, 256, lds)); if (b2 < b) b = b2; }
+      return b;
+    };
+    auto allow_lds = [&](unsigned lds) {
+      HIP_CHECK(hipFuncSetAttribute((const void *)k_accumulate<CV>, hipFuncAttributeMaxDynamicSharedMemorySize, (int)lds));
+      if constexpr (CV::WINDOW_SUMS) HIP_CHECK(hipFuncSetAttribute((const void *)k_accumulate<CV, true>, hipFuncAttributeMaxDynamicSharedMemorySize, (int)lds));
+    };
+    blocks = resident(0);
     if (blocks < 1) blocks = 1;
     if (hipDeviceGetAttribute(&lds_cu, hipDeviceAttributeMaxSharedMemoryPerMultiprocessor, dev) != hipSuccess || lds_cu <= 0) { (void)hipGetLastError(); lds_cu = 0; }
     if (hipDeviceGetAttribute(&lds_blk, hipDeviceAttributeMaxSharedMemoryPerBlock, dev) != hipSuccess || lds_blk <= 0) { (void)hipGetLastError(); lds_blk = 64 * 1024; }
@@ -559,15 +660,14 @@
       const unsigned slice = (unsigned)(lds_cu / (cap + 1) + 1024);
       if ((size_t)slice * cap <= (size_t)lds_cu && slice <= (unsigned)lds_blk) {
         blocks = cap; lds = slice;
-        if (lds > 48 * 1024) HIP_CHECK(hipFuncSetAttribute((const void *)k_accumulate<CV>, hipFuncAttributeMaxDynamicSharedMemorySize, (int)lds));
+        if (lds > 48 * 1024) allow_lds(lds);
       }
     }
     {
       const unsigned need = 4u * 2u * CV::BASE_WORDS * 64u * 4u;
       if (lds < need) lds = need;
-      if (lds > 48 * 1024) HIP_CHECK(hipFuncSetAttribute((const void *)k_accumulate<CV>, hipFuncAttributeMaxDynamicSharedMemorySize, (int)lds));
-      int blk2 = 0;
-      HIP_CHECK(hipOccupancyMaxActiveBlocksPerMultiprocessor(&blk2, k_accumulate<CV>, 256, lds));
+      if (lds > 48 * 1024) allow_lds(lds);
+      const int blk2 = resident(lds);
       if (blk2 >= 1 && blk2 < blocks) blocks = blk2;
     }
     cache[dev] = AccShape{(size_t)cus * blocks * 256, lds};
@@ -600,7 +700,7 @@
   plan_dev.ensure(64);
   ws_buf(buckets, nbk * acc_bytes, 9); ws_buf(rc, nbk * acc_bytes, 10);
   ws_buf(part, (lanes_max + nbk + 64) * (part_bytes ? part_bytes : acc_bytes) + 64, 11);
-  ws_buf(bits, nbits * acc_bytes, 12); own.ensure(nbits * acc_bytes);
+  ws_buf(bits, nbits * acc_bytes + 64, 12); own.ensure(nbits * acc_bytes + 64);
 }
 
 void MsmChain::ensure(size_t bytes) {
@@ -612,7 +712,7 @@
 static void msm_collect(MsmWorkspace &ws, MsmChain &rec, hipStream_t stream) {
   if (ws.owns(rec)) { HIP_CHECK(hipStreamSynchronize(stream)); HIP_CHECK(hipGetLastError()); }
   HIP_CHECK(hipEventElapsedTime(&ws.accum_ms_last, rec.ev0, rec.ev1));
-  rec.plan.lpb = (int)rec.plan_host.as()[0];
+  rec.plan.lpb = (int)(rec.lpb_word ? rec.bits_host.as()[rec.lpb_word] : rec.plan_host.as()[0]);
   ws.accum_ms_total += ws.accum_ms_last; ws.accum_launches++; ws.last_plan = rec.plan;
 }
 
@@ -662,6 +762,7 @@
   const int table_c = o.table_c, scalars_mont = o.scalars_mont;
   const uint32_t *const d_base_idx = o.d_base_idx;
   MsmPlan p = msm_plan(n_in, scalar_bits);
+  rec.lpb_word = 0;
   auto finish = [&]() { if (!o.defer) msm_collect(ws, rec, stream); };
   if (n_in <= MSM_TINY_TERMS && batch <= (CV::FIXED_TABLE ? (size_t)7 : MSM_TINY_VECTORS) && !table_c && !d_base_idx && !scalars_mont && msm_env().tiny) {
     p.c = 1; p.nwin = scalar_bits; p.nb = 1; p.lpb = 0;
@@ -698,20 +799,26 @@
   const uint32_t nbk = vwin * p.nb;
   const uint32_t tile_len = tile_len_for(n, vwin), ntiles = (uint32_t)((n + tile_len - 1) / tile_len);
   const size_t lds_bytes = (size_t)p.nb * 4;
+  bool wave_planned = false;
+  if constexpr (CV::WINDOW_SUMS) wave_planned = batch == 1 && msm_env().window_sums && vwin <= PLAN_WAVE_WINDOWS;
+  const uint32_t lanes_u = (uint32_t)lanes_target, per_min_u = (uint32_t)msm_env().per_min;
   hipLaunchKernelGGL(k_digits, dim3((unsigned)((n_in + 255) / 256), (unsigned)batch), b256, 0, stream, d_scalars, (uint32_t)n_in, (uint32_t)scalar_stride,
                      p.c, dig_nwin, ws.keys.as<uint16_t>(), scalars_mont);
   hipLaunchKernelGGL(k_hist, dim3(ntiles, vwin), b256, lds_bytes, stream, ws.keys.as<uint16_t>(), (uint32_t)n, tile_len, p.c, ws.hist.as());
   hipLaunchKernelGGL(k_scan_tiles, dim3((unsigned)((p.nb + 255) / 256), vwin), b256, 0, stream, ws.hist.as(), ntiles, p.c, ws.cnts.as());
   hipLaunchKernelGGL(k_scan_offs, dim3(vwin), dim3(1024), 0, stream, ws.cnts.as(), (uint32_t)n, p.c, ws.offsets.as(), ws.win_tot.as());
-  hipLaunchKernelGGL(k_plan, dim3(1), dim3(1024), 0, stream, ws.win_tot.as(), vwin, (uint32_t)lanes_target, (uint32_t)msm_env().per_min,
-                     ws.lane_base.as(), ws.plan_dev.as());
+  if (!wave_planned) hipLaunchKernelGGL(k_plan, dim3(1), dim3(1024), 0, stream, ws.win_tot.as(), vwin, lanes_u, per_min_u, ws.lane_base.as(), ws.plan_dev.as());
   hipLaunchKernelGGL(k_scatter, dim3(8u * ((vwin + 7u) / 8u) * ntiles), b256, lds_bytes, stream, ws.keys.as<uint16_t>(), (uint32_t)n, tile_len, p.c, ws.hist.as(),
                      ws.offsets.as(), ws.sorted.as(), remap_n, remap_stride, d_base_idx, ntiles, vwin);
-  rec.ensure((size_t)vwin * 3 * acc_bytes);
+  rec.ensure((size_t)vwin * 3 * acc_bytes + 64);
   if (CV::ZERO_IS_IDENTITY) HIP_CHECK(hipMemsetAsync(ws.buckets.p, 0, (size_t)nbk * acc_bytes, stream));
   HIP_CHECK(hipEventRecord(rec.ev0, stream));
-  hipLaunchKernelGGL(k_accumulate<CV>, dim3((unsigned)((lanes_max + 255) / 256)), b256, accumulate_shape<CV>().lds, stream, d_bases, ws.sorted.as(),
-                     ws.offsets.as(), ws.win_tot.as(), ws.lane_base.as(), ws.plan_dev.as(), vwin, (uint32_t)p.nb, (uint32_t)n, ws.part.as());
+  auto accumulate = [&](auto kernel) {
+    hipLaunchKernelGGL(kernel, dim3((unsigned)((lanes_max + 255) / 256)), b256, accumulate_shape<CV>().lds, stream, d_bases, ws.sorted.as(),
+                       ws.offsets.as(), ws.win_tot.as(), ws.lane_base.as(), ws.plan_dev.as(), vwin, (uint32_t)p.nb, (uint32_t)n, ws.part.as(), lanes_u, per_min_u);
+  };
+  if constexpr (CV::WINDOW_SUMS) { if (wave_planned) accumulate(k_accumulate<CV, true>); else accumulate(k_accumulate<CV, false>); }
+  else accumulate(k_accumulate<CV, false>);
   HIP_CHECK(hipEventRecord(rec.ev1, stream));
   auto bucket_sums = [&](auto tag) {
     using BV = typename decltype(tag)::type;
@@ -720,16 +827,24 @@
     hipLaunchKernelGGL(k_heavy_sum<BV>, dim3(nbk < 1024 ? nbk : 1024), b256, 4 * acc_bytes, stream, ws.offsets.as(), ws.cnts.as(), ws.lane_base.as(),
                        ws.plan_dev.as(), (uint32_t)p.nb, (uint32_t)n, ws.part.as(), ws.buckets.as(), ws.heavy.as());
   };
-  if (red) bucket_sums(type_tag<RV>{}); else bucket_sums(type_tag<CV>{});
-  HIP_CHECK(hipMemcpyAsync(rec.plan_host.p, ws.plan_dev.p, 8, hipMemcpyDeviceToHost, stream));
+  if constexpr (CV::WINDOW_SUMS) if (wave_planned) {
+    const uint32_t nblk = (nbk + 255) / 256;
+    hipLaunchKernelGGL(k_bucket_heavy_sum<CV>, dim3(nblk + HEAVY_BLOCKS), b256, 0, stream, ws.offsets.as(), ws.cnts.as(), ws.win_tot.as(), vwin, lanes_u, per_min_u,
+                       nbk, nblk, (uint32_t)p.nb, (uint32_t)n, ws.part.as(), ws.buckets.as());
+  }
+  if (!wave_planned) { if (red) bucket_sums(type_tag<RV>{}); else bucket_sums(type_tag<CV>{}); }
+  const bool window_sums = CV::WINDOW_SUMS && batch == 1 && msm_env().window_sums;
+  if (!window_sums) HIP_CHECK(hipMemcpyAsync(rec.plan_host.p, ws.plan_dev.p, 8, hipMemcpyDeviceToHost, stream));
   rec.plan = p;
-  if constexpr (CV::WINDOW_SUMS) if (batch == 1 && msm_env().window_sums) {
+  if constexpr (CV::WINDOW_SUMS) if (window_sums) {
     const uint32_t nb = (uint32_t)p.nb;
     const uint32_t wpw = nb >= 256 ? 16u : 1u, m = nb >= 256 ? nb / 256 : (nb >= 16 ? nb / 16 : 1u);
     const uint32_t nwaves = vwin * wpw;
     hipLaunchKernelGGL(k_wsum_q1<typename CV::suite>, dim3((nwaves + 3) / 4), b256, 0, stream, ws.buckets.as(), nb, m, wpw, nwaves, ws.rc.as());
-    hipLaunchKernelGGL(k_wsum_q2<typename CV::suite>, dim3(vwin), dim3(64), 0, stream, ws.rc.as(), wpw, ws.bits.as());
-    HIP_CHECK(hipMemcpyAsync(rec.bits_host.p, ws.bits.p, (size_t)vwin * 3 * acc_bytes, hipMemcpyDeviceToHost, stream));
+    hipLaunchKernelGGL(k_wsum_q2<typename CV::suite>, dim3(vwin), dim3(64), 0, stream, ws.rc.as(), wpw, ws.bits.as(),
+                       wave_planned ? (const uint32_t *)nullptr : ws.plan_dev.as(), ws.win_tot.as(), vwin, lanes_u, per_min_u);
+    rec.lpb_word = (size_t)vwin * 3 * (acc_bytes / 4);
+    HIP_CHECK(hipMemcpyAsync(rec.bits_host.p, ws.bits.p, (size_t)vwin * 3 * acc_bytes + 4, hipMemcpyDeviceToHost, stream));
     rec.wsum_lg = 4; while ((1u << rec.wsum_lg) < 16 * m) rec.wsum_lg++;
     finish();
     return -(int)vwin;
@@ -1311,7 +1426,7 @@
   HIP_CHECK(hipEventRecord(rec.ev1, stream));
   hipLaunchKernelGGL(k_direct_reduce<RV>, dim3((unsigned)batch), dim3(64), 0, stream, ws.part.as(), (uint32_t)lpv, ws.rc.as());
   HIP_CHECK(hipMemcpyAsync(rec.bits_host.p, ws.rc.p, batch * (size_t)RV::OUT_WORDS * 4, hipMemcpyDeviceToHost, stream));
-  rec.plan_host.as()[0] = (uint32_t)per;
+  rec.plan_host.as()[0] = (uint32_t)per; rec.lpb_word = 0;
   rec.plan = p;
   msm_collect(ws, rec, stream);
   std::vector<typename HG::Pt> res(batch);
diff --git a/ark_vrf_amd/csrc/proto_dev.h b/ark_vrf_amd/csrc/proto_dev.h
--- a/ark_vrf_amd/csrc/proto_dev.h
+++ b/ark_vrf_amd/csrc/proto_dev.h
@@ -39,6 +39,7 @@
   const uint8_t *weights;
   te_ext *tabs;
   uint32_t first;
+  uint32_t *flag_blk;
 };
 struct Seed64 { uint64_t w[8]; };
 template <class S> using suite_tr = std::conditional_t<S::XOF_SHAKE, Shake128, std::conditional_t<S::TR_SHA256, Sha256, Sha512>>;
diff --git a/ark_vrf_amd/csrc/te_quad.h b/ark_vrf_amd/csrc/te_quad.h
--- a/ark_vrf_amd/csrc/te_quad.h
+++ b/ark_vrf_amd/csrc/te_quad.h
@@ -231,9 +231,7 @@
   if (q == 8) Q::store(o + 32, V);
 }
 
-template <class S>
-__global__ void __launch_bounds__(64)
-k_wsum_q2(const uint32_t *__restrict__ trip, uint32_t wpw, uint32_t *__restrict__ out) {
+template <class S> AVRF_DI void q_wsum_level2(const uint32_t *__restrict__ trip, uint32_t wpw, uint32_t *__restrict__ out) {
   const uint32_t v = blockIdx.x, lane = threadIdx.x & 63, q = lane >> 2, j = lane & 3;
   using Q = Quad<S>; using el = typename Q::el;
   el v1 = Q::identity(j), v2 = v1, y = v1;
diff --git a/ark_vrf_amd/csrc/vrf_batch.hip b/ark_vrf_amd/csrc/vrf_batch.hip
--- a/ark_vrf_amd/csrc/vrf_batch.hip
+++ b/ark_vrf_amd/csrc/vrf_batch.hip
@@ -7,12 +7,19 @@
 #endif
 namespace avrf {
 
-template <class S>
-__global__ void __launch_bounds__(128)
-k_thin_prepare(BatchDev b, uint32_t *__restrict__ c_out, uint32_t *__restrict__ z_out, uint32_t *__restrict__ flags) {
-  using Fr = typename S::Fr;
-  uint32_t j = blockIdx.x * blockDim.x + threadIdx.x;
-  if (j >= b.n) return;
+AVRF_DI void publish_flags(uint32_t f, uint32_t *__restrict__ flags, uint32_t *__restrict__ flag_blk) {
+  if (!flag_blk) { if (f) atomicOr(flags, f); return; }
+  __shared__ uint32_t blk_flags;
+  if (threadIdx.x == 0) blk_flags = 0;
+  __syncthreads();
+  if (f) atomicOr(&blk_flags, f);
+  __syncthreads();
+  if (threadIdx.x == 0) flag_blk[blockIdx.x] = blk_flags;
+}
+
+template <class S>
+AVRF_DI uint32_t thin_prepare_item(const BatchDev &b, uint32_t j, uint32_t *__restrict__ c_out, uint32_t *__restrict__ z_out) {
+  using Fr = typename S::Fr;
   uint32_t io0 = b.io_off[j], io1 = b.io_off[j + 1], m = io1 - io0;
   uint32_t ad0 = b.ad_off[j], adl = b.ad_off[j + 1] - ad0;
   uint32_t f = 0;
@@ -67,7 +74,13 @@
       r[0] = make_uint4(w[0], w[1], w[2], w[3]); r[1] = make_uint4(0, 0, 0, 0); r[2] = sp[0]; r[3] = sp[1];
     }
   }
-  if (f) atomicOr(flags, f);
+  return f;
+}
+template <class S>
+__global__ void __launch_bounds__(128)
+k_thin_prepare(BatchDev b, uint32_t *__restrict__ c_out, uint32_t *__restrict__ z_out, uint32_t *__restrict__ flags) {
+  const uint32_t j = blockIdx.x * blockDim.x + threadIdx.x;
+  publish_flags(j < b.n ? thin_prepare_item<S>(b, j, c_out, z_out) : 0u, flags, b.flag_blk);
 }
 
 AVRF_DI fp fp_from_u128(const uint32_t *w) {
@@ -147,11 +160,8 @@
 
 
 template <class S>
-__global__ void __launch_bounds__(128)
-k_ped_prepare(BatchDev b, uint32_t *__restrict__ c_out, uint8_t *__restrict__ merged_xy, uint32_t *__restrict__ flags) {
-  using Fr = typename S::Fr;
-  uint32_t j = blockIdx.x * blockDim.x + threadIdx.x;
-  if (j >= b.n) return;
+AVRF_DI uint32_t ped_prepare_item(const BatchDev &b, uint32_t j, uint32_t *__restrict__ c_out, uint8_t *__restrict__ merged_xy) {
+  using Fr = typename S::Fr;
   uint32_t io0 = b.io_off[j], m = b.io_off[j + 1] - io0, ad0 = b.ad_off[j], adl = b.ad_off[j + 1] - ad0;
   const uint8_t *ios = b.ios_xy + 128 * (size_t)io0, *pr = b.proofs + 256 * (size_t)j;
   suite_tr<S> t; uint32_t f = 0;
@@ -195,7 +205,13 @@
     const uint4 *sp = reinterpret_cast<const uint4 *>(pr + 192);
     r[0] = make_uint4(c.v[0], c.v[1], c.v[2], c.v[3]); r[1] = make_uint4(0, 0, 0, 0); r[2] = sp[0]; r[3] = sp[1]; r[4] = sp[2]; r[5] = sp[3];
   }
-  if (f) atomicOr(flags, f);
+  return f;
+}
+template <class S>
+__global__ void __launch_bounds__(128)
+k_ped_prepare(BatchDev b, uint32_t *__restrict__ c_out, uint8_t *__restrict__ merged_xy, uint32_t *__restrict__ flags) {
+  const uint32_t j = blockIdx.x * blockDim.x + threadIdx.x;
+  publish_flags(j < b.n ? ped_prepare_item<S>(b, j, c_out, merged_xy) : 0u, flags, b.flag_blk);
 }
 
 template <class S>
```
